# ma921/SOBER

Measured on AMD Instinct MI355X. Metric: recombination-step candidates/sec (N_rec=100000, N_nys=500, d=10, batch=100), higher is better.
Workload: dtype f64

## Files before the change

### include/sober_hip.h

```cpp
#ifndef SOBER_HIP_H
#define SOBER_HIP_H

#include <stdint.h>

#ifdef __cplusplus
extern "C" {
#endif

#define SOBER_ABI_VERSION 7

#define SOBER_KIND_RBF       0
#define SOBER_KIND_MATERN52  1
#define SOBER_KIND_TANIMOTO  2

#define SOBER_E_ARG      -1
#define SOBER_E_DIM      -2
#define SOBER_E_WS       -3
#define SOBER_E_EXCHANGE -5

int sober_abi_version(void);
int sober_diag_build(void);
int sober_reload_switches(void);
int sober_level_job_size(void);
int sober_nystrom_job_size(void);

int sober_padded_dim(int d);
int sober_bit_words(int d);

int sober_mt19937_uniform53(uint8_t* state, int64_t state_bytes, int64_t numel, double* out);
int sober_box_muller(const double* u, int64_t numel, double* out, void* stream);

int sober_scale_points(const double* X, int64_t n, int d, int64_t ldx,
                       const double* lengthscale, int ls_len,
                       double* out, int dt, void* stream);

int sober_scale_points_idx(const double* X, const int32_t* idx, int64_t n, int d, int64_t ldx, const double* lengthscale,
                           int ls_len, double* out, int dt, const double* gather_src, double* gather_out, void* stream);
int sober_pack_bits(const double* X, int64_t n, int d, int64_t ldx,
                    uint64_t* words, int nwords, double* norms, int32_t* bad_flag, void* stream);

int sober_pairwise(int kind, const void* a, const double* a_norm, int64_t m,
                   const void* b, const double* b_norm, const int32_t* idx, int64_t n,
                   int dt, double outputscale, double* out, int64_t ldo, void* stream);

int sober_kernel_matvec(int kind, const void* a, const double* a_norm, const double* v, int64_t m,
                        const void* b, const double* b_norm, int64_t n,
                        int dt, double outputscale, double c0, double* out, void* stream);

int sober_level_reduce(int kind, const void* rows, const double* rows_norm, int n_rows,
                       const void* cand, const double* cand_norm, int dt,
                       const int32_t* idx, int64_t pos0, int64_t count, int S,
                       const double* mu, const double* wmul, double outputscale,
                       int n_chunks, double* partG, int ldg, int col0,
                       double* partTot, int64_t tot_limit, void* stream);
int sober_aug_dim(int d);
int sober_augment_plan(const double* X_nys, int64_t M, int64_t ld_nys, const double* X_obs, int64_t n_obs, int64_t ld_obs,
                       const double* X_cand, int64_t N, int64_t ld_cand, int d, const double* lengthscale, int ls_len,
                       double* center, double* rows_aug, double* cand_aug, int da, void* stream);
int sober_augment_points(const double* X, int64_t n, int d, int64_t ldx, const double* lengthscale,
                         int ls_len, const double* center, int side, double* out, int da, void* stream);
int sober_level_reduce_mfma(int kind, const double* rows, int n_rows, const double* cand, int da,
                            const int32_t* idx, int64_t pos0, int64_t count, int S,
                            const double* mu, const double* wmul, double outputscale,
                            int n_chunks, double* partG, int ldg, int col0,
                            double* partTot, int64_t tot_limit, void* stream);

int64_t sober_nonzero_ws_bytes(int64_t N);
int sober_nonzero_i32(const double* mu, int64_t N, int32_t* idx_out, int64_t* count_out, void* ws, int64_t ws_bytes,
                      void* stream);

int sober_level_chunks(int n_rows, int64_t pos0, int64_t count, int S);
int sober_level_parts_mfma(int n_rows, int64_t pos0, int64_t count, int S);
int sober_level_parts_mfma_cap(int n_rows, int64_t e_total_ub, int S);

int sober_sum_partials(const double* partG, const double* partTot, int n_chunks, int n_rows,
                       int ldg, int S, const double* extraG, const double* extraTot,
                       int n_xchunks, int n_xcols, double* G, int ldo, double* tot, void* stream);

int sober_dgemm(int transa, int transb, int m, int n, int k, double alpha,
                const double* A, int lda, const double* B, int ldb,
                double beta, double* C, int ldc, void* stream);

int sober_barycentres(const double* Xtr, int ldx, int n, int S, const double* tot,
                      double* X_tmp, void* stream);
int sober_dgemm_coldiv_t(int m, int n, int k, const double* A, int lda, const double* B, int ldb, const double* coldiv,
                         double* Ct, int ldct, void* stream);

int sober_level_update(const int32_t* idx_cur, int64_t pos0, int64_t count, int S, int64_t E,
                       const int32_t* keep_rank, const double* w_star, const double* tot,
                       int n_keep, double* mu, int32_t* idx_new, int64_t new_pos0, void* stream);

int sober_scatter_weights(const int32_t* idx_cur, const int32_t* sel, const double* w, int n_sel,
                          double* mu, int64_t* out_idx, void* stream);

int sober_gather_f64(const double* src, const int32_t* idx, int64_t n, double* out, void* stream);
int sober_final_scatter(const int32_t* idx, int n, const int32_t* keep_rank, const double* w_star,
                        int64_t row_offset, double* mu, int64_t* out_idx, double* out_w, void* stream);
int sober_final_commit(const int32_t* idx, int n, const int32_t* keep_rank, const double* w_star, const int32_t* n_keep,
                       int64_t row_offset, double* mu, int64_t N, int64_t* out_idx, double* out_w, void* stream);

int sober_i64_to_i32(const int64_t* in, int64_t n, int32_t* out, void* stream);

int sober_car_pivot_host(double* h_Phi, int N, int m, double* h_mu);
int sober_car_pivot_host_fast(double* h_Phi, int N, int m, double* h_mu);

int sober_car_supported(int N, int m);
int64_t sober_car_ws_bytes(int N, int m);
int sober_car_device(const double* X, int ldx, int N, int m, const double* mu_in,
                     int32_t* keep_rank, double* w_star, int32_t* n_keep, double* mu_out,
                     double* phi_out, void* ws, int64_t ws_bytes, void* stream);
int sober_probe_rcp(const double* x, double* out, int64_t n, void* stream);

#define SOBER_CAR_DEFAULT 0
#define SOBER_CAR_SAFE 1
int sober_car_safe_supported(int N, int m);
int sober_car_giveup_forced(void);
int sober_car_device_ex(const double* X, int ldx, int N, int m, const double* mu_in,
                        int32_t* keep_rank, double* w_star, int32_t* n_keep, double* mu_out,
                        double* phi_out, void* ws, int64_t ws_bytes, int mode, void* stream);
int sober_obj_set_sums(const double* obj, const double* mu, const int32_t* idx, int64_t pos0, int64_t count, int S, int64_t E,
                       double* out, void* stream);
int sober_second_elimination(const double* phi, const double* objp, const double* w1, const int32_t* rank1, int n1,
                             int Nsets, int32_t* keep_rank, double* w_star, int32_t* n_keep, void* stream);
int sober_null_vector_supported(int nfun);
int sober_null_vector(const double* X, int ldx, int Nsets, int nfun, const int32_t* rank1, const int32_t* n_keep1, int n1,
                      double* null_row, int32_t* status, void* stream);
int sober_second_elimination_rows(const double* null_row, const double* obj_row, const double* w1, const int32_t* rank1,
                                  const int32_t* n_keep1, const int32_t* status, int n1, int Nsets, int32_t* keep_rank,
                                  double* w_star, int32_t* n_keep, void* stream);
int sober_obj_set_sums_queued(const double* obj, const double* mu, const int32_t* idx, int S, const int64_t* dR, int64_t R_known,
                              const double* tot, double* xcol, int ldx, double* ocol, void* stream);

int sober_car_mc_supported(int N, int m);
int64_t sober_car_mc_ws_bytes(int N, int m);
int sober_car_mc_device(const double* X, int ldx, int N, int m, const double* mu_in,
                        int32_t* keep_rank, double* w_star, int32_t* n_keep, double* mu_out,
                        double* phi_out, void* ws, int64_t ws_bytes, void* stream);
int sober_car_big_supported(int N, int m);
int64_t sober_car_big_ws_bytes(int N, int m);
int sober_car_big_device(const double* X, int ldx, int N, int m, const double* mu_in,
                         int32_t* keep_rank, double* w_star, int32_t* n_keep, double* mu_out,
                         double* phi_out, void* ws, int64_t ws_bytes, void* stream);
int sober_mc_selftest(const double* in, double* out, void* stream);

int sober_chol_max_n(void);
int sober_nystrom_max_n(void);
int sober_cholesky_probe_batched(const double* src, int n, int ld_src, const double* shifts, int n_shifts,
                                 double* work, int32_t* info, double* min_pivot, void* xinv_ws, int64_t ws_bytes,
                                 void* stream);
int sober_cholesky(double* A, int n, int ld, double shift, int32_t* info, double* min_pivot, void* stream);
int sober_cholesky_inv(double* A, int n, int ld, double shift, int32_t* info, double* min_pivot, double* xinv,
                       void* stream);
int sober_cholesky_inv_ratio(double* A, int n, int ld, double shift, int32_t* info, double* min_pivot, double* xinv,
                             double* ratio_out, void* stream);
int sober_trsm_blocks(const double* Y, int64_t m, int q, int ldy, const double* L, int ldl, const double* Xinv,
                      double* Q, int ldq, void* stream);
int sober_cholesky_probe(const double* src, int n, int ld_src, const double* shifts, int n_shifts,
                         double* work, int32_t* info, void* stream);
int sober_cholesky_probe_piv(const double* src, int n, int ld_src, const double* shifts, int n_shifts,
                             double* work, int32_t* info, double* min_pivot, void* stream);

int64_t sober_cholesky_probe_mc_ws_bytes(int n, int n_shifts);
int sober_cholesky_probe_mc(const double* src, int n, int ld_src, const double* shifts, int n_shifts,
                            double* work, int32_t* info, double* min_pivot, void* ws, int64_t ws_bytes,
                            void* stream);
int sober_abs_sym(const double* C, int n, int ld, double* out, int ldo, int32_t* flag, void* stream);
int sober_abs_sym_dmax(const double* C, int n, int ld, double* out, int ldo, int32_t* flag, double* dmax,
                       void* stream);

int sober_jitter_ladder(double* A, int n, int ld, int k, void* stream);
int sober_jitter_ladder_auto(double* A, int n, int ld, const int32_t* info, int n_rungs, int32_t* k_out,
                             void* stream);

int sober_level_reduce_tani_supported(int dt);
int sober_level_reduce_tani(const void* rows, const double* rows_norm, int n_rows, const void* cand,
                            const double* cand_norm, int dt, const int32_t* idx, int64_t pos0, int64_t count, int S,
                            const double* mu, const double* wmul, double outputscale, int n_chunks, double* partG,
                            int ldg, int col0, double* partTot, int64_t tot_limit, void* stream);

int sober_rank_scatter(const double* X, int ldx, int N, int n, const double* ocol, const int32_t* rank, int n1,
                       double* Xp, double* objp, void* stream);
int sober_set_i64(int64_t* dst, int64_t v, void* stream);

int sober_level_reduce_mfma_queued(int kind, const double* rows, int n_rows, const double* cand, int da,
                                   const int32_t* idx, int64_t count_ub, int S, int S_main, int leftover,
                                   const double* mu, const double* wmul, double outputscale, int n_chunks_ub,
                                   double* partG, int ldg, double* partTot, const int64_t* dR, void* stream);
int sober_level_reduce_mfma_queued_pair(int kind, const double* rows, int n_rows, const double* cand, int da,
                                        const int32_t* idx, int64_t count_ub, int S, int n_xcols, const double* mu,
                                        const double* wmul, double outputscale, int n_chunks_ub, double* partG,
                                        int ldg, double* partTot, int n_xchunks_ub, double* extraG, double* extraTot,
                                        const int64_t* dR, void* stream);
int sober_sum_partials_queued(const double* partG, const double* partTot, int n_rows, int ldg, int S,
                              const double* extraG, const double* extraTot, int n_xcols, double* G, int ldo,
                              double* tot, const int64_t* dR, int chunked, void* stream);
int sober_level_reduce_tani_queued(const void* rows, const double* rows_norm, int n_rows, const void* cand,
                                   const double* cand_norm, int dt, const int32_t* idx, int64_t count_ub, int S,
                                   int S_main, int leftover, const double* mu, const double* wmul, double outputscale,
                                   int n_chunks_ub, double* partG, int ldg, double* partTot, const int64_t* dR,
                                   void* stream);
int sober_level_reduce_tani_queued_pair(const void* rows, const double* rows_norm, int n_rows, const void* cand,
                                        const double* cand_norm, int dt, const int32_t* idx, int64_t count_ub, int S,
                                        int n_xcols, const double* mu, const double* wmul, double outputscale,
                                        int n_chunks_ub, double* partG, int ldg, double* partTot, int n_xchunks_ub,
                                        double* extraG, double* extraTot, const int64_t* dR, void* stream);
int sober_level_chunks_cap(int n_rows, int64_t e_total_ub, int S);
int sober_level_chunks_tani(int n_rows, int64_t pos0, int64_t count, int S);
int sober_level_chunks_tani_cap(int n_rows, int64_t e_total_ub, int S);
int sober_level_update_queued(const int32_t* idx_cur, int64_t R_ub, int S, const int32_t* keep_rank,
                              const double* w_star, const double* tot, double* mu, int32_t* idx_new,
                              const int64_t* dR_cur, int64_t* dR_next, int64_t R_ub_next, void* stream);

int sober_level_class_wpt(int n_rows, int64_t e_total, int S);
int sober_level_class_slots(int wpt);
int sober_level_reduce_mfma_wpt(int kind, const double* rows, int n_rows, const double* cand, int da,
                                const int32_t* idx, int64_t count, int S, const double* mu, const double* wmul,
                                double outputscale, int wpt, int n_chunks, double* partG, int ldg, double* partTot,
                                void* stream);
int sober_class_sum(const double* partG, const double* partTot, int n_chunks, int n_rows, int S, int CL,
                    double* Gc, double* totc, double* G, double* tot, void* stream);
int sober_class_derive_queued(const double* Gc, const double* totc, int n_rows, int S, int CL, const double* scale,
                              const int32_t* sof, double* Gn, double* totn, double* G, double* tot, const int64_t* dR,
                              void* stream);
int sober_level_update_queued_ex(const int32_t* idx_cur, int64_t R_ub, int S, const int32_t* keep_rank,
                                 const double* w_star, const double* tot, double* mu, int32_t* idx_new,
                                 const int64_t* dR_cur, int64_t* dR_next, int64_t R_ub_next, int need_keep,
                                 double* cls_scale, int32_t* cls_sof, int64_t R_known, void* stream);
int sober_level_update_queued_cls(const int32_t* idx_cur, int64_t R_ub, int S, const int32_t* keep_rank,
                                  const double* w_star, const double* tot, double* mu, int32_t* idx_new,
                                  const int64_t* dR_cur, int64_t* dR_next, int64_t R_ub_next, int need_keep,
                                  double* cls_scale, int32_t* cls_sof, void* stream);
#define SOBER_CLASS_MAX_DEPTH 4
int sober_level_class_depth(int variant, int n_rows, int64_t R, int S);

int64_t sober_kmeans_ws_bytes(int64_t N, int d, int K);
int64_t sober_kmeans_stat_offset(int64_t N, int d, int K);
int64_t sober_kmeans_ws_bytes_screened(int64_t N, int d, int K);
int sober_kmeans_lloyd(const double* X, int64_t N, int d, int K, int iters,
                       double* centroids, int32_t* labels, void* ws, int64_t ws_bytes, void* stream);

int sober_predict_fused_supported(int kind, int n_obs, int dt);
int sober_predict_fused(int kind, const void* obs, const double* obs_norm, int n_obs, const void* cand,
                        const double* cand_norm, int64_t N, int dt, double outputscale, const double* W, int ldw,
                        const double* alpha, double c0, double kxx_const, double noise, double* mean_out, double* var_out,
                        double eta, const double* eta_ptr, double* lfi_out, int log_flag, void* stream);
int sober_predict_fused_root(int kind, const void* obs, const double* obs_norm, int n_obs, const void* cand,
                             const double* cand_norm, int64_t N, int dt, double outputscale, const double* St, int ldst,
                             const int32_t* tri_flag, const double* alpha, double c0, double kxx_const, double noise,
                             double* mean_out, double* var_out, double eta, const double* eta_ptr, double* lfi_out, int log_flag,
                             void* stream);
int sober_predict_finish(const double* KX, const double* V, int n_obs, int64_t N, int64_t ld,
                         const double* mean, double kxx_const, const double* norms, double outputscale,
                         double noise, double* var_out, double eta, double* lfi_out, int log_flag,
                         void* stream);

int64_t sober_reduce_ws_bytes(int64_t n);
int sober_cleansing_weights(double* w, int64_t n, double eps, void* ws, int64_t ws_bytes, void* stream);

int sober_wkde_draw(const double* eps, int64_t n, int d, const int32_t* comp, const double* Xobs, int ldx,
                    const double* L, const double* lo, const double* hi, double* x, int32_t* inside,
                    void* stream);

int sober_level_gather(const double* Kmat, int n_rows, int64_t ldk, const int32_t* idx, int64_t pos0,
                       int64_t count, int S, const double* mu, const double* wmul, int n_chunks,
                       double* partG, int ldg, int col0, double* partTot, int64_t tot_limit, void* stream);

int sober_gspace_finish(double* K, const double* corr, int64_t n, int m, int64_t ldk, int64_t ldc,
                        const double* mug_cand, const double* mug_rows, void* stream);

#define SOBER_LEVEL_VALU        0
#define SOBER_LEVEL_MFMA        1
#define SOBER_LEVEL_GATHER      2
#define SOBER_LEVEL_TANI        3
#define SOBER_LEVEL_MAX_CHUNKS  64
#define SOBER_LEVEL_XS          16
typedef struct sober_level_job {
    int32_t variant, kind;
    const void* rows;   const double* rows_norm;
    const void* cand;   const double* cand_norm;
    int32_t n_rows, dim;
    int64_t kmat_ld;
    const double* wmul; double outputscale;
    int32_t S, n;
    const double* P;
    double *partG, *partTot, *extraG, *extraTot;
    double *G, *Xtr, *tot;
    double *X_tmp;
    int32_t* keep_rank;
    double *w_star, *mu_out;
    void* car_ws; int64_t car_ws_bytes;
    int32_t* h_flags;
    void* ev[4];
    const int32_t* idx; int64_t pos0, count, E;
    double* mu;
    int32_t phase;
    int64_t* dR; int64_t* h_dR;
    int32_t car_mode;
    uint64_t ev_used[2];
    int32_t class_depth;
    double* Gc[2]; double* totc[2];
    double* cls_scale; int32_t* cls_sof;
} sober_level_job;
#define SOBER_LEVEL_QUEUE 24
int sober_level_moments(const sober_level_job* job, void* stream);
int sober_level_car(const sober_level_job* job, void* stream);
int sober_level_car_retry(sober_level_job* job, void* stream);
#define SOBER_E_NOPROGRESS -4
int sober_level_loop(sober_level_job* job, int64_t R, int32_t* idx_a, int32_t* idx_b, int first_sums_ready,
                     void** events, int max_levels, int64_t* level_R, int32_t* n_levels, int64_t* R_final,
                     int32_t* in_b, void* stream);
typedef struct sober_obj_job {
    const double* obj;
    double* X_tmp;
    double* ocol;
    int32_t* kr1; double* w1; int32_t* nk1;
    double* null_row;
    int32_t* status;
} sober_obj_job;
int sober_obj_job_size(void);
int sober_level_loop_obj(sober_level_job* job, const sober_obj_job* obj_job, int64_t R, int32_t* idx_a, int32_t* idx_b,
                         int first_sums_ready, int max_levels, int64_t* level_R, int32_t* n_levels, int64_t* R_final,
                         int32_t* in_b, void* stream);
typedef int (*sober_allreduce_fn)(void* comm, double* buf, int64_t n, void* stream);
int sober_level_loop_sharded(sober_level_job* job, int rank, int world, int64_t* bounds, int32_t* idx_a,
                             int32_t* idx_b, int first_sums_ready, sober_allreduce_fn allreduce, void* comm,
                             int64_t R_stop, int max_levels, int64_t* level_R, int32_t* n_levels, int32_t* in_b,
                             void* stream);
int sober_rccl_load(const char* path);
int sober_rccl_unique_id(char* out128);
int sober_rccl_comm_init(const char* id128, int rank, int world, void** comm);
int sober_rccl_comm_destroy(void* comm);
int sober_rccl_allreduce_f64(void* comm, double* buf, int64_t n, void* stream);
int64_t sober_rccl_allreduce_ptr(void);

int64_t sober_peer_region_bytes(int64_t n_max);
int sober_peer_create(int rank, int world, int64_t n_max, void** comm, char* handle64);
int sober_peer_connect(void* comm, const char* handles);
int sober_peer_connect_ptrs(void* comm, void* const* regions);
int64_t sober_peer_region(void* comm);
int sober_peer_set_spin_limit(void* comm, unsigned spin_limit);
int sober_peer_allreduce_f64(void* comm, double* buf, int64_t n, void* stream);
int64_t sober_peer_allreduce_ptr(void);
int sober_peer_status(void* comm, double* restore, int64_t n, void* stream);
int sober_peer_destroy(void* comm);

int sober_level_final(const sober_level_job* job, const void* rows_sc, const double* rows_norm, const void* cand_sc,
                      const double* cand_norm, int dt, const int32_t* idx, int R, int64_t N, int64_t row_offset,
                      double* K, double* mu_live, int64_t* out_idx, double* out_w, void* stream);
int sober_plan_rows(int kind, const double* X_nys, int M, int64_t ld_nys, const double* X_obs, int n_obs,
                    int64_t ld_obs, int d, const double* lengthscale, int ls_len, double outputscale,
                    const double* S_cache, int ld_s, double* rows, int dt, double* Kall, double* W, double* T,
                    double* G, void* stream);

typedef struct sober_final_job {
    const void* rows_sc; const double* rows_norm;
    const void* cand_sc; const double* cand_norm;
    int32_t dt, done;
    int64_t N, row_offset;
    double *K, *mu_live;
    int64_t* out_idx; double* out_w;
    const double* cand_raw; int64_t ld_raw; int32_t d_raw, ls_len; const double* ls; double* sc_buf;
} sober_final_job;
int sober_level_final_job(const sober_level_job* job, const sober_final_job* final, const int32_t* idx, int R, void* stream);
int sober_final_job_size(void);
int sober_level_loop_final(sober_level_job* job, sober_final_job* final, int64_t R, int32_t* idx_a, int32_t* idx_b,
                           int first_sums_ready, void** events, int max_levels, int64_t* level_R, int32_t* n_levels,
                           int64_t* R_final, int32_t* in_b, void* stream);
int sober_projection(const double* Ut, int s, int M, const double* mean, const double* T, int n_obs, double* P,
                     void* stream);

typedef struct sober_nystrom_job {
    int32_t M, s, n_rungs, niter, probe_mc;
    int32_t reserved0;
    const double* G;
    const double* shifts;
    const double* R;
    double* C;
    double* chol_work;
    void* probe_ws; int64_t probe_ws_bytes;
    double* Y[2];
    double* Gm;
    double* xinv;
    void* flags_block; int64_t flags_bytes;
    void* h_flags_block;
    double* Ut;
    const double* T; int32_t n_obs;
    const double* mean_nys; double* P;
} sober_nystrom_job;
int64_t sober_nystrom_flags_bytes(int n_rungs, int niter);
int sober_nystrom_basis(const sober_nystrom_job* job, int phase, void* stream);

int sober_set_launch_events(void* start, void* stop);
int sober_record_event_pair(void* ev0, void* ev1, void* stream);

#ifdef __cplusplus
}
#endif
#endif
```

### sober_amd/_engine.py

```python
from __future__ import annotations

import os
import time
import warnings
from typing import Optional

import numpy as np
import torch

from . import _native as nat
from ._utils import SafeTensorOperator


class SoloComm:
    rank, world = 0, 1

    def allreduce_sum(self, *tensors):
        return

    def allgather_counts(self, n: int):
        return [n]

    def allgather_rows(self, t: torch.Tensor, counts):
        return t
# ... 152 lines not shown
    lm = len(w_star)
    plis = w_null > 0
    alpha = torch.zeros(lm, dtype=dt)
    alpha[plis] = w_star[plis] / w_null[plis]
    idx_sp = torch.arange(lm)[plis]
    idx_sp = idx_sp[torch.argmin(alpha[plis])]
    w_star = w_star - alpha[idx_sp] * w_null
    w_star[idx_sp] = 0.0
    keep = w_star > 0
    return w_star[keep], idx_star[keep]


def survivors_before(p: int, S: int, E: int, kept_prefix, n_keep: int, last_kept: bool) -> int:
    ES = E * S
    if p <= ES:
        return (p // S) * n_keep + kept_prefix[p % S]
    return E * n_keep + ((p - ES) if last_kept else 0)


class RecombinationEngine:
    def __init__(self, ops, comm=None, row_offset: int = 0):
        self.ops = ops
        self.comm = comm or SoloComm()
        self.row_offset = int(row_offset)
        self.tm = SafeTensorOperator()
        self.trace = None
        self.timers = {}
        self.force_host_car = False
        self.force_host_nystrom = False
        self.basis_override = None
        self.cutover_R = int(os.environ.get("SOBER_CUTOVER_R", "32768"))
        self.force_sharded = bool(os.environ.get("SOBER_FORCE_SHARDED"))

    def _tick(self, name, t0):
        t1 = time.perf_counter()
        self.timers[name] = self.timers.get(name, 0.0) + (t1 - t0)
        return t1

    def nystrom_basis(self, plan, s: int, overlap=None, literal=False, early=None):
        if self.basis_override is not None:
            return self.basis_override
        t0 = time.perf_counter()
        dev_route = getattr(self.ops, "nystrom_basis_device", None)
        if dev_route is not None and not self.force_host_nystrom and not literal:
            res = dev_route(plan, s, self.tm.max_iter, overlap, early) if (overlap is not None or early is not None) \
                else dev_route(plan, s, self.tm.max_iter)
            if res is not None:
                U, gram = res
                self._tick("nystrom_device", t0)
                if self.trace is not None:
                    (gram_h, U_h) = self.ops.to_host(gram, U)
                    self.trace.update(gram=gram_h, U=U_h)
                return U
        gram = self.ops.gram(plan)
        (gram_h,) = self.ops.to_host(gram)
        t0 = self._tick("gram_device", t0)
        _, U = ker_svd_sparsify_host(gram_h, s, self.tm)
        self._tick("nystrom_host", t0)
        if self.trace is not None:
            self.trace.update(gram=gram_h.clone(), U=U.clone())
        return U

    def run(self, plan, mu: torch.Tensor, num_pts: int, obj: Optional[torch.Tensor] = None, live=None):
        ops, comm = self.ops, self.comm
        self.obj = obj
        self.obj_head = None
        if obj is not None:
            head = obj[:2 * num_pts].clone()
            if comm.world > 1:
                cnt = comm.allgather_counts(int(head.numel()))
                head = comm.allgather_rows(head, cnt)[:2 * num_pts]
            self.obj_head = head
        n = num_pts - 1
        S = 2 * (n + 1)
        state = {}
        can_start = getattr(ops, "nonzero_start", None) is not None and live is None
        pend = {}

        def start_list():
            if can_start and "p" not in pend:
                pend["p"] = ops.nonzero_start(mu)
        sharded = comm.world > 1 or (self.force_sharded and getattr(comm, "native_allreduce", None) is not None)

        def first_sums():
            if live is not None:
                idx_cur, count = live, int(live.numel())
            else:
                start_list()
                idx_cur, count = ops.nonzero_finish(pend["p"]) if "p" in pend else ops.nonzero_i32(mu)
            counts = comm.allgather_counts(count)
            bounds = [0]
            for c in counts:
                bounds.append(bounds[-1] + c)
            state.update(idx_cur=idx_cur, count=count, pos0=bounds[comm.rank], R=bounds[-1], bounds=bounds)
            cut = sharded and obj is None and self.cutover_R > 0 and state["R"] <= self.cutover_R
            if state["R"] > S and getattr(ops, "level_car", None) is not None and count > 0 and not cut:
                ops.level_moments(plan, idx_cur, state["pos0"], count, S, state["R"] // S, mu, phase=1, n=n)
                state["sums_ready"] = True

        def head_once():
            if not state:
                first_sums()

        n_fun = n + 1 + (1 if obj is not None else 0)
        car_on_host = self.force_host_car or getattr(ops, "car_supported", None) is None \
            or not ops.car_supported(S, n_fun) or (obj is not None and getattr(ops, "car_obj_device", None) is None)
        if car_on_host and not self.force_host_car and getattr(ops, "size_cliff", None) is not None \
                and getattr(ops, "car_supported", None) is not None and not ops.car_supported(S, n_fun):
            ops.size_cliff("car", f"batch = {n + 1}: a Caratheodory step on 2 x batch = {S} points with {n_fun} test functions is beyond "
                                  "the device kernels (registers of one compute unit: batch <= 100, of nine: batch <= 224, memory-resident: "
                                  "2 x batch <= 2048); every level's step runs on host LAPACK + the C++ pivots instead -- seconds per level")
        if comm.world > 1:
            start_list()
        U = self.nystrom_basis(plan, n, overlap=head_once if comm.world == 1 else None, literal=car_on_host,
                               early=start_list if comm.world == 1 else None)
        if comm.world > 1:
            U = comm.broadcast0(ops.from_host(U.contiguous()) if U.device != ops.device else U.contiguous())
            if hasattr(plan, "_proj_src"):
                plan._proj_src = None
        ops.set_projection(plan, U)
        head_once()
        idx_cur, count, pos0, R = state["idx_cur"], state["count"], state["pos0"], state["R"]
        bounds = state["bounds"]
        sums_ready = state.get("sums_ready", False)
        idx_new = ops.empty_i32(count)
        levels = [] if self.trace is not None else None

        if self.trace is not None:
            self.trace["levels"] = levels
        if not sharded and obj is None and levels is None and not self.force_host_car and R > S \
                and getattr(ops, "level_loop", None) is not None and ops.car_supported(S, n + 1):
            t0 = time.perf_counter()
            idx_cur, idx_new, R = ops.level_loop(plan, idx_cur, idx_new, R, S, mu, sums_ready, self.row_offset)
            pos0, count, bounds, sums_ready = 0, R, [0, R], False
            self._tick("levels_device", t0)
        elif not sharded and obj is not None and levels is None and not self.force_host_car and R > S \
                and getattr(ops, "level_loop_obj", None) is not None:
            t0 = time.perf_counter()
            res = ops.level_loop_obj(plan, idx_cur, idx_new, R, S, mu, obj, sums_ready)
            if res is not None and res[3] > 0:
                idx_cur, idx_new, R = res[:3]
                pos0, count, bounds, sums_ready = 0, R, [0, R], False
            self._tick("levels_device", t0)
        elif sharded and obj is None and levels is None and not self.force_host_car and R > S \
                and getattr(ops, "level_loop_sharded", None) is not None and ops.car_supported(S, n + 1) \
                and getattr(comm, "native_allreduce", None) is not None:
            t0 = time.perf_counter()
            idx_cur, idx_new, bounds = ops.level_loop_sharded(plan, idx_cur, idx_new, bounds, S, mu, sums_ready, comm,
                                                              self.cutover_R)
            R, pos0, count, sums_ready = bounds[-1], bounds[comm.rank], bounds[comm.rank + 1] - bounds[comm.rank], False
            self._tick("levels_device", t0)
            if R > S:
                return self._finish_replicated(plan, idx_cur, bounds, mu, num_pts, U)
        while True:
            if R <= n + 1:
                return self._finish_small(mu)
            if R <= S:
                return self._finish_direct(plan, idx_cur, bounds, R, mu, levels)

            E = R // S
            r = R - E * S
            t0 = time.perf_counter()
            if sums_ready:
                Xtr, tot = ops.level_moments(plan, idx_cur, pos0, count, S, E, mu, phase=2)
                sums_ready = False
            else:
                Xtr, tot = ops.level_moments(plan, idx_cur, pos0, count, S, E, mu)
            if obj is None:
                flat = getattr(ops, "level_flat", None)
                if flat is not None:
                    comm.allreduce_sum(flat(plan))
                else:
                    comm.allreduce_sum(Xtr, tot)
            else:
                orow = self._obj_set_sums(obj, mu, idx_cur, pos0, count, S, E)
                comm.allreduce_sum(Xtr, tot, orow)
                Xtr = torch.cat([Xtr, orow.unsqueeze(0)], 0)
            if obj is None and not self.force_host_car and getattr(ops, "level_car", None) is not None \
                    and ops.car_supported(S, n + 1):
                res = ops.level_car(plan, S)
                if res is None:
                    X_tmp, tot = ops.level_barycentres(plan)
                    keep_rank_d, w_star_d, keep_rank, n_keep = self._car(X_tmp, tot, R, E, r, levels, t0)
                    keep_np = keep_rank.numpy()
                else:
                    keep_rank_d, w_star_d, keep_np, n_keep = res
                    self._tick("levels_device", t0)
                    if levels is not None:
                        X_h, mu_h, w_h = ops.level_trace(plan)
                        levels.append(dict(kind="level", R=R, E=E, r=r, X_tmp=X_h, tot_weights=mu_h,
                                           idx_star=torch.from_numpy(np.flatnonzero(keep_np >= 0)),
                                           w_star=w_h[:n_keep].clone()))
            else:
                X_tmp = ops.barycentres(Xtr, tot)
                keep_rank_d, w_star_d, keep_rank, n_keep = self._car(X_tmp, tot, R, E, r, levels, t0)
                keep_np = keep_rank.numpy()
            kept = keep_np >= 0
            last_kept = bool(kept[S - 1])
            kept_prefix = [0] + np.cumsum(kept).tolist()
            R_new = E * n_keep + (r if last_kept else 0)
            if R_new >= R:
                raise RuntimeError(
                    "recombination made no progress (the Caratheodory step cancelled nothing, "
                    "SOBER/_rchq.py:241-242); the reference would loop forever here")
            bounds = [survivors_before(b_, S, E, kept_prefix, n_keep, last_kept) for b_ in bounds]
            new_pos0, new_end = bounds[comm.rank], bounds[comm.rank + 1]
            if count > 0:
                ops.level_update(idx_cur, pos0, count, S, E, keep_rank_d, w_star_d, tot, n_keep, mu,
                                 idx_new, new_pos0)
            idx_cur, idx_new = idx_new, idx_cur
            pos0, count, R = new_pos0, new_end - new_pos0, R_new

    def _obj_set_sums(self, obj, mu, idx_cur, pos0, count, S, E):
        dev = mu.device
        if count == 0:
            return torch.zeros(S, dtype=torch.float64, device=dev)
        native = getattr(self.ops, "obj_set_sums", None)
        if native is not None and obj.dtype == torch.float64 and obj.is_contiguous():
            return native(obj, mu, idx_cur, pos0, count, S, E)
        c = idx_cur[:count].long()
        v = obj[c] * mu[c]
        e_first = pos0 // S
        e_total = (pos0 + count + S - 1) // S - e_first
        dense = torch.zeros(e_total * S, dtype=torch.float64, device=dev)
        off = pos0 - e_first * S
        dense[off:off + count] = v
        out = dense.view(e_total, S).sum(0)
        n_left = pos0 + count - max(pos0, E * S)
        if n_left > 0:
            out[S - 1] += v[count - n_left:].sum()
        return out

    def _finish_replicated(self, plan, idx_cur, bounds, mu, num_pts, U):
        ops, comm = self.ops, self.comm
        counts = [bounds[r + 1] - bounds[r] for r in range(comm.world)]
        loc = idx_cur[:counts[comm.rank]].long()
        X_all = comm.allgather_rows(plan.X_cand_raw[loc].to(torch.float64).contiguous(), counts)
        w_all = comm.allgather_rows(mu[loc].contiguous(), counts)
        gid = comm.allgather_rows((loc + self.row_offset).contiguous(), counts)
        plan2 = ops.build_plan(plan.spec, plan.mode, plan.X_nys_raw, X_all)
        sub = RecombinationEngine(ops, SoloComm(), row_offset=0)
        sub.basis_override = U
        sub.force_host_nystrom, sub.force_host_car = self.force_host_nystrom, self.force_host_car
        mu2 = w_all.clone().contiguous()
        live2 = torch.arange(mu2.numel(), dtype=torch.int32, device=mu2.device)
        idx2, w2 = sub.run(plan2, mu2, num_pts, live=live2)
        for k, v in sub.timers.items():
            self.timers[k] = self.timers.get(k, 0.0) + v
        idx_glob = gid[idx2]
        mu[loc] = 0.0
        mine = (idx_glob >= self.row_offset) & (idx_glob < self.row_offset + mu.numel())
        mu[idx_glob[mine] - self.row_offset] = w2[mine]
        return idx_glob, w2

    def _car(self, X_dev, mu_dev, R, E, r, levels, t0, kind="level"):
        ops = self.ops
        Np, n1 = X_dev.shape[0], X_dev.shape[1] + 1
        use_obj = getattr(self, "obj", None) is not None
        on_device = getattr(ops, "car_supported", None) is not None and ops.car_supported(Np, n1) \
            and not self.force_host_car
        if on_device and use_obj and getattr(ops, "car_obj_device", None) is not None:
            res = ops.car_obj_device(X_dev, mu_dev, None if kind == "level" else self.obj_head)
            if res is not None:
                keep_rank_d, w_star_d, keep_rank, n_keep, (kr1_h, w1_d, n1k) = res
                self._tick("levels_device", t0)
                if levels is not None:
                    X_h, mu_h, w1_h = ops.to_host(X_dev, mu_dev, w1_d)
                    levels.append(dict(kind=kind, R=R, E=E, r=r, X_tmp=X_h, tot_weights=mu_h,
                                       idx_star=torch.nonzero(kr1_h >= 0).flatten(), w_star=w1_h[:n1k].clone()))
                return keep_rank_d, w_star_d, keep_rank, n_keep
            on_device = False
        elif use_obj:
            on_device = False
        if on_device:
            res = ops.car_device_checked(X_dev, mu_dev, also=(X_dev, mu_dev) if levels is not None else ())
            if res is not None:
                keep_rank_d, w_star_d, keep_rank, n_keep, extra = res
                self._tick("levels_device", t0)
                if levels is not None:
                    (w_h,) = ops.to_host(w_star_d)
                    levels.append(dict(kind=kind, R=R, E=E, r=r, X_tmp=extra[0], tot_weights=extra[1],
                                       idx_star=torch.nonzero(keep_rank >= 0).flatten(), w_star=w_h[:n_keep].clone()))
                return keep_rank_d, w_star_d, keep_rank, n_keep
        X_h, mu_h = ops.to_host(X_dev, mu_dev)
        t0 = self._tick("levels_device", t0)
        w_star, idx_star = car_host(X_h, mu_h.clone())
        if levels is not None:
            levels.append(dict(kind=kind, R=R, E=E, r=r, X_tmp=X_h.clone(), tot_weights=mu_h.clone(),
                               idx_star=idx_star.clone(), w_star=w_star.clone()))
        if use_obj:
            nfun = X_h.shape[1] - 1
            obj_p = X_h[idx_star, nfun] if kind == "level" else self.obj_head.cpu()[idx_star]
            w_star, idx_star = second_elimination_host(X_h[idx_star, :nfun].T.contiguous(), obj_p, w_star, idx_star)
        self._tick("car_host", t0)
        n_keep = int(idx_star.numel())
        keep_rank = torch.full((Np,), -1, dtype=torch.int32)
        keep_rank[idx_star] = torch.arange(n_keep, dtype=torch.int32)
        return ops.from_host(keep_rank), ops.from_host(w_star), keep_rank, n_keep

    def _gather_result(self, idx_local, w_local, counts=None):
        comm = self.comm
        idx_glob = idx_local.to(torch.int64) + self.row_offset
        if comm.world == 1:
            return idx_glob, w_local
        if counts is None:
            counts = comm.allgather_counts(int(idx_glob.numel()))
        return comm.allgather_rows(idx_glob, counts), comm.allgather_rows(w_local, counts)

    def _finish_small(self, mu):
        idx_star = torch.nonzero(mu > 0).flatten()
        return self._gather_result(idx_star, mu[idx_star])

    def _finish_direct(self, plan, idx_cur, bounds, R, mu, levels):
        ops, comm = self.ops, self.comm
        n = plan.n
        counts = [bounds[r + 1] - bounds[r] for r in range(comm.world)]
# ... 33 lines not shown
```

### sober_amd/_native.py

```python
from __future__ import annotations

import ctypes as C
import os
from typing import Optional

import torch

_HERE = os.path.dirname(os.path.abspath(__file__))
LIB_PATH = os.environ.get("SOBER_HIP_LIB") or os.path.join(_HERE, "libsober_hip.so")
ABI_VERSION = 7

KIND_RBF, KIND_MATERN52, KIND_TANIMOTO = 0, 1, 2
KIND_BY_NAME = {"rbf": KIND_RBF, "matern52": KIND_MATERN52, "tanimoto": KIND_TANIMOTO}

_vp, _i32, _i64, _f64 = C.c_void_p, C.c_int, C.c_int64, C.c_double

SIGNATURES = {
    "sober_abi_version": (_i32, []),
    "sober_diag_build": (_i32, []),
    "sober_reload_switches": (_i32, []),
    "sober_level_job_size": (_i32, []),
    "sober_nystrom_job_size": (_i32, []),
    "sober_final_job_size": (_i32, []),
    "sober_set_i64": (_i32, [_vp, _i64, _vp]),
    "sober_rank_scatter": (_i32, [_vp, _i32, _i32, _i32, _vp, _vp, _i32, _vp, _vp, _vp]),
    "sober_plan_rows": (_i32, [_i32, _vp, _i32, _i64, _vp, _i32, _i64, _i32, _vp, _i32, _f64, _vp, _i32, _vp, _i32, _vp,
                               _vp, _vp, _vp, _vp]),
    "sober_level_loop_final": (_i32, [_vp, _vp, _i64, _vp, _vp, _i32, _vp, _i32, _vp, _vp, _vp, _vp, _vp]),
    "sober_padded_dim": (_i32, [_i32]),
    "sober_bit_words": (_i32, [_i32]),
    "sober_scale_points": (_i32, [_vp, _i64, _i32, _i64, _vp, _i32, _vp, _i32, _vp]),
    "sober_augment_plan": (_i32, [_vp, _i64, _i64, _vp, _i64, _i64, _vp, _i64, _i64, _i32, _vp, _i32, _vp, _vp, _vp, _i32, _vp]),
    "sober_scale_points_idx": (_i32, [_vp, _vp, _i64, _i32, _i64, _vp, _i32, _vp, _i32, _vp, _vp, _vp]),
    "sober_pack_bits": (_i32, [_vp, _i64, _i32, _i64, _vp, _i32, _vp, _vp, _vp]),
    "sober_mt19937_uniform53": (_i32, [_vp, _i64, _i64, _vp]),
    "sober_box_muller": (_i32, [_vp, _i64, _vp, _vp]),
    "sober_pairwise": (_i32, [_i32, _vp, _vp, _i64, _vp, _vp, _vp, _i64, _i32, _f64, _vp, _i64, _vp]),
    "sober_kernel_matvec": (_i32, [_i32, _vp, _vp, _vp, _i64, _vp, _vp, _i64, _i32, _f64, _f64, _vp, _vp]),
    "sober_level_reduce": (_i32, [_i32, _vp, _vp, _i32, _vp, _vp, _i32, _vp, _i64, _i64, _i32, _vp, _vp,
                                  _f64, _i32, _vp, _i32, _i32, _vp, _i64, _vp]),
    "sober_nonzero_ws_bytes": (_i64, [_i64]),
    "sober_nonzero_i32": (_i32, [_vp, _i64, _vp, _vp, _vp, _i64, _vp]),
    "sober_dgemm_coldiv_t": (_i32, [_i32, _i32, _i32, _vp, _i32, _vp, _i32, _vp, _vp, _i32, _vp]),
    "sober_level_chunks": (_i32, [_i32, _i64, _i64, _i32]),
    "sober_level_parts_mfma": (_i32, [_i32, _i64, _i64, _i32]),
    "sober_level_parts_mfma_cap": (_i32, [_i32, _i64, _i32]),
    "sober_aug_dim": (_i32, [_i32]),
    "sober_augment_points": (_i32, [_vp, _i64, _i32, _i64, _vp, _i32, _vp, _i32, _vp, _i32, _vp]),
    "sober_level_reduce_mfma": (_i32, [_i32, _vp, _i32, _vp, _i32, _vp, _i64, _i64, _i32, _vp, _vp, _f64, _i32,
                                       _vp, _i32, _i32, _vp, _i64, _vp]),
    "sober_sum_partials": (_i32, [_vp, _vp, _i32, _i32, _i32, _i32, _vp, _vp, _i32, _i32, _vp, _i32, _vp, _vp]),
    "sober_dgemm": (_i32, [_i32, _i32, _i32, _i32, _i32, _f64, _vp, _i32, _vp, _i32, _f64, _vp, _i32, _vp]),
    "sober_barycentres": (_i32, [_vp, _i32, _i32, _i32, _vp, _vp, _vp]),
    "sober_level_update": (_i32, [_vp, _i64, _i64, _i32, _i64, _vp, _vp, _vp, _i32, _vp, _vp, _i64, _vp]),
    "sober_scatter_weights": (_i32, [_vp, _vp, _vp, _i32, _vp, _vp, _vp]),
    "sober_i64_to_i32": (_i32, [_vp, _i64, _vp, _vp]),
    "sober_car_pivot_host": (_i32, [_vp, _i32, _i32, _vp]),
    "sober_car_pivot_host_fast": (_i32, [_vp, _i32, _i32, _vp]),
    "sober_car_supported": (_i32, [_i32, _i32]),
    "sober_car_ws_bytes": (_i64, [_i32, _i32]),
    "sober_car_device": (_i32, [_vp, _i32, _i32, _i32, _vp, _vp, _vp, _vp, _vp, _vp, _vp, _i64, _vp]),
    "sober_probe_rcp": (_i32, [_vp, _vp, _i64, _vp]),
    "sober_second_elimination": (_i32, [_vp, _vp, _vp, _vp, _i32, _i32, _vp, _vp, _vp, _vp]),
    "sober_car_mc_supported": (_i32, [_i32, _i32]),
    "sober_car_mc_ws_bytes": (_i64, [_i32, _i32]),
    "sober_car_mc_device": (_i32, [_vp, _i32, _i32, _i32, _vp, _vp, _vp, _vp, _vp, _vp, _vp, _i64, _vp]),
    "sober_car_big_supported": (_i32, [_i32, _i32]),
    "sober_car_big_ws_bytes": (_i64, [_i32, _i32]),
    "sober_car_big_device": (_i32, [_vp, _i32, _i32, _i32, _vp, _vp, _vp, _vp, _vp, _vp, _vp, _i64, _vp]),
    "sober_car_device_ex": (_i32, [_vp, _i32, _i32, _i32, _vp, _vp, _vp, _vp, _vp, _vp, _vp, _i64, _i32, _vp]),
    "sober_obj_set_sums": (_i32, [_vp, _vp, _vp, _i64, _i64, _i32, _i64, _vp, _vp]),
    "sober_null_vector_supported": (_i32, [_i32]),
    "sober_null_vector": (_i32, [_vp, _i32, _i32, _i32, _vp, _vp, _i32, _vp, _vp, _vp]),
    "sober_second_elimination_rows": (_i32, [_vp, _vp, _vp, _vp, _vp, _vp, _i32, _i32, _vp, _vp, _vp, _vp]),
    "sober_obj_set_sums_queued": (_i32, [_vp, _vp, _vp, _i32, _vp, _i64, _vp, _vp, _i32, _vp, _vp]),
    "sober_obj_job_size": (_i32, []),
    "sober_level_loop_obj": (_i32, [_vp, _vp, _i64, _vp, _vp, _i32, _i32, _vp, _vp, _vp, _vp, _vp]),
    "sober_car_safe_supported": (_i32, [_i32, _i32]),
    "sober_car_giveup_forced": (_i32, []),
    "sober_final_commit": (_i32, [_vp, _i32, _vp, _vp, _vp, _i64, _vp, _i64, _vp, _vp, _vp]),
    "sober_level_car_retry": (_i32, [_vp, _vp]),
    "sober_mc_selftest": (_i32, [_vp, _vp, _vp]),
    "sober_chol_max_n": (_i32, []),
    "sober_nystrom_max_n": (_i32, []),
    "sober_cholesky_probe_batched": (_i32, [_vp, _i32, _i32, _vp, _i32, _vp, _vp, _vp, _vp, _i64, _vp]),
    "sober_cholesky": (_i32, [_vp, _i32, _i32, _f64, _vp, _vp, _vp]),
    "sober_cholesky_inv": (_i32, [_vp, _i32, _i32, _f64, _vp, _vp, _vp, _vp]),
    "sober_cholesky_inv_ratio": (_i32, [_vp, _i32, _i32, _f64, _vp, _vp, _vp, _vp, _vp]),
    "sober_trsm_blocks": (_i32, [_vp, _i64, _i32, _i32, _vp, _i32, _vp, _vp, _i32, _vp]),
    "sober_cholesky_probe": (_i32, [_vp, _i32, _i32, _vp, _i32, _vp, _vp, _vp]),
    "sober_cholesky_probe_piv": (_i32, [_vp, _i32, _i32, _vp, _i32, _vp, _vp, _vp, _vp]),
    "sober_cholesky_probe_mc_ws_bytes": (_i64, [_i32, _i32]),
    "sober_cholesky_probe_mc": (_i32, [_vp, _i32, _i32, _vp, _i32, _vp, _vp, _vp, _vp, _i64, _vp]),
    "sober_abs_sym": (_i32, [_vp, _i32, _i32, _vp, _i32, _vp, _vp]),
    "sober_abs_sym_dmax": (_i32, [_vp, _i32, _i32, _vp, _i32, _vp, _vp, _vp]),
    "sober_jitter_ladder": (_i32, [_vp, _i32, _i32, _i32, _vp]),
    "sober_jitter_ladder_auto": (_i32, [_vp, _i32, _i32, _vp, _i32, _vp, _vp]),
    "sober_kmeans_ws_bytes": (_i64, [_i64, _i32, _i32]),
    "sober_kmeans_stat_offset": (_i64, [_i64, _i32, _i32]),
    "sober_kmeans_ws_bytes_screened": (_i64, [_i64, _i32, _i32]),
    "sober_kmeans_lloyd": (_i32, [_vp, _i64, _i32, _i32, _i32, _vp, _vp, _vp, _i64, _vp]),
    "sober_predict_fused_supported": (_i32, [_i32, _i32, _i32]),
    "sober_predict_fused": (_i32, [_i32, _vp, _vp, _i32, _vp, _vp, _i64, _i32, _f64, _vp, _i32, _vp, _f64, _f64, _f64, _vp, _vp,
                                   _f64, _vp, _vp, _i32, _vp]),
    "sober_predict_fused_root": (_i32, [_i32, _vp, _vp, _i32, _vp, _vp, _i64, _i32, _f64, _vp, _i32, _vp, _vp, _f64, _f64, _f64, _vp,
                                        _vp, _f64, _vp, _vp, _i32, _vp]),
    "sober_predict_finish": (_i32, [_vp, _vp, _i32, _i64, _i64, _vp, _f64, _vp, _f64, _f64, _vp, _f64, _vp, _i32, _vp]),
    "sober_reduce_ws_bytes": (_i64, [_i64]),
    "sober_cleansing_weights": (_i32, [_vp, _i64, _f64, _vp, _i64, _vp]),
    "sober_level_gather": (_i32, [_vp, _i32, _i64, _vp, _i64, _i64, _i32, _vp, _vp, _i32, _vp, _i32, _i32, _vp, _i64,
                                  _vp]),
    "sober_gspace_finish": (_i32, [_vp, _vp, _i64, _i32, _i64, _i64, _vp, _vp, _vp]),
    "sober_wkde_draw": (_i32, [_vp, _i64, _i32, _vp, _vp, _i32, _vp, _vp, _vp, _vp, _vp, _vp]),
    "sober_level_moments": (_i32, [_vp, _vp]),
    "sober_level_car": (_i32, [_vp, _vp]),
    "sober_level_reduce_tani_supported": (_i32, [_i32]),
    "sober_level_reduce_tani": (_i32, [_vp, _vp, _i32, _vp, _vp, _i32, _vp, _i64, _i64, _i32, _vp, _vp, _f64, _i32, _vp,
                                       _i32, _i32, _vp, _i64, _vp]),
    "sober_level_loop_sharded": (_i32, [_vp, _i32, _i32, _vp, _vp, _vp, _i32, _vp, _vp, _i64, _i32, _vp, _vp, _vp, _vp]),
    "sober_rccl_load": (_i32, [C.c_char_p]),
    "sober_rccl_unique_id": (_i32, [_vp]),
    "sober_rccl_comm_init": (_i32, [_vp, _i32, _i32, _vp]),
    "sober_rccl_comm_destroy": (_i32, [_vp]),
    "sober_rccl_allreduce_f64": (_i32, [_vp, _vp, _i64, _vp]),
    "sober_rccl_allreduce_ptr": (_i64, []),
    "sober_peer_region_bytes": (_i64, [_i64]),
    "sober_peer_create": (_i32, [_i32, _i32, _i64, _vp, _vp]),
    "sober_peer_connect": (_i32, [_vp, C.c_char_p]),
    "sober_peer_connect_ptrs": (_i32, [_vp, _vp]),
    "sober_peer_region": (_i64, [_vp]),
    "sober_peer_set_spin_limit": (_i32, [_vp, C.c_uint]),
    "sober_peer_allreduce_f64": (_i32, [_vp, _vp, _i64, _vp]),
    "sober_peer_allreduce_ptr": (_i64, []),
    "sober_peer_status": (_i32, [_vp, _vp, _i64, _vp]),
    "sober_peer_destroy": (_i32, [_vp]),
    "sober_level_reduce_mfma_queued": (_i32, [_i32, _vp, _i32, _vp, _i32, _vp, _i64, _i32, _i32, _i32, _vp, _vp, _f64,
                                              _i32, _vp, _i32, _vp, _vp, _vp]),
    "sober_level_reduce_mfma_queued_pair": (_i32, [_i32, _vp, _i32, _vp, _i32, _vp, _i64, _i32, _i32, _vp, _vp, _f64, _i32,
                                                   _vp, _i32, _vp, _i32, _vp, _vp, _vp, _vp]),
    "sober_sum_partials_queued": (_i32, [_vp, _vp, _i32, _i32, _i32, _vp, _vp, _i32, _vp, _i32, _vp, _vp, _i32, _vp]),
    "sober_level_reduce_tani_queued": (_i32, [_vp, _vp, _i32, _vp, _vp, _i32, _vp, _i64, _i32, _i32, _i32, _vp, _vp, _f64,
                                              _i32, _vp, _i32, _vp, _vp, _vp]),
    "sober_level_reduce_tani_queued_pair": (_i32, [_vp, _vp, _i32, _vp, _vp, _i32, _vp, _i64, _i32, _i32, _vp, _vp, _f64, _i32,
                                                   _vp, _i32, _vp, _i32, _vp, _vp, _vp, _vp]),
    "sober_level_chunks_cap": (_i32, [_i32, _i64, _i32]),
    "sober_level_chunks_tani": (_i32, [_i32, _i64, _i64, _i32]),
    "sober_level_chunks_tani_cap": (_i32, [_i32, _i64, _i32]),
    "sober_level_update_queued": (_i32, [_vp, _i64, _i32, _vp, _vp, _vp, _vp, _vp, _vp, _vp, _i64, _vp]),
    "sober_level_update_queued_ex": (_i32, [_vp, _i64, _i32, _vp, _vp, _vp, _vp, _vp, _vp, _vp, _i64, _i32, _vp, _vp, _i64, _vp]),
    "sober_level_update_queued_cls": (_i32, [_vp, _i64, _i32, _vp, _vp, _vp, _vp, _vp, _vp, _vp, _i64, _i32, _vp, _vp, _vp]),
    "sober_level_class_wpt": (_i32, [_i32, _i64, _i32]),
    "sober_level_class_slots": (_i32, [_i32]),
    "sober_level_class_depth": (_i32, [_i32, _i32, _i64, _i32]),
    "sober_level_reduce_mfma_wpt": (_i32, [_i32, _vp, _i32, _vp, _i32, _vp, _i64, _i32, _vp, _vp, _f64, _i32, _i32, _vp, _i32,
                                           _vp, _vp]),
    "sober_class_sum": (_i32, [_vp, _vp, _i32, _i32, _i32, _i32, _vp, _vp, _vp, _vp, _vp]),
    "sober_class_derive_queued": (_i32, [_vp, _vp, _i32, _i32, _i32, _vp, _vp, _vp, _vp, _vp, _vp, _vp, _vp]),
    "sober_record_event_pair": (_i32, [_vp, _vp, _vp]),
    "sober_set_launch_events": (_i32, [_vp, _vp]),
    "sober_projection": (_i32, [_vp, _i32, _i32, _vp, _vp, _i32, _vp, _vp]),
    "sober_nystrom_flags_bytes": (_i64, [_i32, _i32]),
    "sober_nystrom_basis": (_i32, [_vp, _i32, _vp]),
    "sober_gather_f64": (_i32, [_vp, _vp, _i64, _vp, _vp]),
    "sober_final_scatter": (_i32, [_vp, _i32, _vp, _vp, _i64, _vp, _vp, _vp, _vp]),
    "sober_level_final": (_i32, [_vp, _vp, _vp, _vp, _vp, _i32, _vp, _i32, _i64, _i64, _vp, _vp, _vp, _vp, _vp]),
    "sober_level_final_job": (_i32, [_vp, _vp, _vp, _i32, _vp]),
    "sober_level_loop": (_i32, [_vp, _i64, _vp, _vp, _i32, _vp, _i32, _vp, _vp, _vp, _vp, _vp]),
}

LEVEL_VALU, LEVEL_MFMA, LEVEL_GATHER, LEVEL_TANI = 0, 1, 2, 3
LEVEL_MAX_CHUNKS, LEVEL_XS, LEVEL_QUEUE = 64, 16, 24


class FinalJob(C.Structure):
    _fields_ = [
        ("rows_sc", _vp), ("rows_norm", _vp), ("cand_sc", _vp), ("cand_norm", _vp),
        ("dt", _i32), ("done", _i32), ("N", _i64), ("row_offset", _i64),
        ("K", _vp), ("mu_live", _vp), ("out_idx", _vp), ("out_w", _vp),
        ("cand_raw", _vp), ("ld_raw", _i64), ("d_raw", _i32), ("ls_len", _i32), ("ls", _vp), ("sc_buf", _vp),
    ]


class ObjJob(C.Structure):
    _fields_ = [("obj", _vp), ("X_tmp", _vp), ("ocol", _vp), ("kr1", _vp), ("w1", _vp), ("nk1", _vp), ("null_row", _vp),
                ("status", _vp)]


class NystromJob(C.Structure):
    _fields_ = [
        ("M", _i32), ("s", _i32), ("n_rungs", _i32), ("niter", _i32), ("probe_mc", _i32), ("_pad0", _i32),
        ("G", _vp), ("shifts", _vp), ("R", _vp), ("C", _vp), ("chol_work", _vp),
        ("probe_ws", _vp), ("probe_ws_bytes", _i64),
        ("Y", _vp * 2), ("Gm", _vp), ("xinv", _vp),
        ("flags_block", _vp), ("flags_bytes", _i64), ("h_flags_block", _vp),
        ("Ut", _vp),
        ("T", _vp), ("n_obs", _i32), ("mean_nys", _vp), ("P", _vp),
    ]


class LevelJob(C.Structure):
    _fields_ = [
        ("variant", _i32), ("kind", _i32),
        ("rows", _vp), ("rows_norm", _vp), ("cand", _vp), ("cand_norm", _vp),
        ("n_rows", _i32), ("dim", _i32), ("kmat_ld", _i64),
        ("wmul", _vp), ("outputscale", _f64),
        ("S", _i32), ("n", _i32), ("P", _vp),
        ("partG", _vp), ("partTot", _vp), ("extraG", _vp), ("extraTot", _vp),
        ("G", _vp), ("Xtr", _vp), ("tot", _vp), ("X_tmp", _vp),
        ("keep_rank", _vp), ("w_star", _vp), ("mu_out", _vp),
        ("car_ws", _vp), ("car_ws_bytes", _i64), ("h_flags", _vp),
        ("ev", _vp * 4),
        ("idx", _vp), ("pos0", _i64), ("count", _i64), ("E", _i64), ("mu", _vp),
        ("phase", _i32),
        ("dR", _vp), ("h_dR", _vp),
        ("car_mode", _i32),
        ("ev_used", C.c_uint64 * 2),
        ("class_depth", _i32), ("Gc", _vp * 2), ("totc", _vp * 2), ("cls_scale", _vp), ("cls_sof", _vp),
    ]

E_DIM = -2
E_EXCHANGE = -5
CLASS_MAX_DEPTH = 4
CAR_DEFAULT, CAR_SAFE, CAR_HOST = 0, 1, 2

_lib: Optional[C.CDLL] = None


class SoberHipError(RuntimeError):
    pass


def load() -> C.CDLL:
    global _lib
    if _lib is not None:
        return _lib
    if not os.path.exists(LIB_PATH):
        raise SoberHipError(
            f"{LIB_PATH} not found: build it with `make -C sober_amd/csrc` "
            "(python -c 'import __graft_entry__ as g; g.build()').  sober_amd has no CPU fallback.")
    lib = C.CDLL(LIB_PATH)
    lib.sober_abi_version.restype = _i32
    got = lib.sober_abi_version()
    if got != ABI_VERSION:
        raise SoberHipError(f"libsober_hip ABI {got} != expected {ABI_VERSION}; rebuild (make -C sober_amd/csrc)")
    for name, (res, args) in SIGNATURES.items():
        fn = getattr(lib, name)
        fn.restype, fn.argtypes = res, args
    if lib.sober_diag_build() and os.environ.get("SOBER_ALLOW_DIAG_LIB") != "1":
        raise SoberHipError(f"{LIB_PATH} is a diagnostic build (in-kernel time stamps): not a library to compute with; "
                            "`make -C sober_amd/csrc` builds the product (SOBER_ALLOW_DIAG_LIB=1: the stamp scripts)")
    for name, cls in (("sober_level_job_size", LevelJob), ("sober_nystrom_job_size", NystromJob),
                      ("sober_final_job_size", FinalJob), ("sober_obj_job_size", ObjJob)):
        if getattr(lib, name)() != C.sizeof(cls):
            raise SoberHipError(f"{cls.__name__}: {C.sizeof(cls)} bytes here, {getattr(lib, name)()} in libsober_hip; "
                                "include/sober_hip.h and sober_amd/_native.py disagree")
    _lib = lib
    return lib


def reload_switches():
    load().sober_reload_switches()


def _check(rc: int, what: str):
    if rc == 0:
        return
    if rc < 0:
        msg = {-1: "bad argument", -2: "dimension not supported by the compiled tile set",
               -3: "workspace too small",
               -5: "a multi-workgroup Caratheodory kernel gave up waiting for a partner workgroup (no result)"}.get(rc, "error")
        raise SoberHipError(f"{what}: {msg} (code {rc})")
    raise SoberHipError(f"{what}: hipError_t {rc}")


def _ptr(t: Optional[torch.Tensor]) -> Optional[int]:
    return None if t is None else t.data_ptr()


_raw_stream = getattr(torch._C, "_cuda_getCurrentRawStream", None)


def _stream(t: torch.Tensor) -> Optional[int]:
    if not t.is_cuda:
        raise SoberHipError("sober_amd runs on the MI355X only: tensor is not on a HIP device")
    if _raw_stream is not None:
        return _raw_stream(t.device.index)
    return torch.cuda.current_stream(t.device).cuda_stream


def _req(t: torch.Tensor, dtype, name: str):
    if t.dtype != dtype or not t.is_contiguous():
        raise SoberHipError(f"{name}: need contiguous {dtype}, got {t.dtype} contiguous={t.is_contiguous()}")
    return t


def padded_dim(d: int, generic: bool = False) -> int:
    r = load().sober_padded_dim(d)
    if r == E_DIM and generic and d > 0:
        return (d + 3) // 4 * 4
    _check(min(r, 0), f"padded_dim({d})")
    return r


def bit_words(d: int, generic: bool = False) -> int:
    r = load().sober_bit_words(d)
    if r == E_DIM and generic and d > 0:
        return (d + 63) // 64
    _check(min(r, 0), f"bit_words({d})")
    return r


def fused_dim_supported(kind: int, d: int) -> bool:
    r = load().sober_bit_words(d) if kind == KIND_TANIMOTO else load().sober_padded_dim(d)
    return r > 0


def scale_points_idx(X, idx, n, lengthscale, out):
    _req(lengthscale, torch.float64, "lengthscale"); _req(out, torch.float64, "out"); _req(idx, torch.int32, "idx")
    if X.dtype != torch.float64 or X.stride(-1) != 1:
        raise SoberHipError("scale_points_idx: X must be float64 with unit inner stride")
    _check(load().sober_scale_points_idx(X.data_ptr(), idx.data_ptr(), int(n), X.shape[1], X.stride(0), lengthscale.data_ptr(),
                                         lengthscale.numel(), out.data_ptr(), out.shape[1], None, None, _stream(X)),
           "sober_scale_points_idx")


def scale_points(X, lengthscale, out):
    n, d = X.shape
    _req(X, torch.float64, "X"); _req(lengthscale, torch.float64, "lengthscale"); _req(out, torch.float64, "out")
    _check(load().sober_scale_points(X.data_ptr(), n, d, X.stride(0), lengthscale.data_ptr(),
                                     lengthscale.numel(), out.data_ptr(), out.shape[1], _stream(X)),
           "sober_scale_points")


def mt19937_uniform53(state, numel, out):
    _req(state, torch.uint8, "state"); _req(out, torch.float64, "out")
    if state.is_cuda or out.is_cuda or out.numel() < numel + 16:
        raise ValueError("mt19937_uniform53 takes host tensors, out of numel + 16 doubles")
    _check(load().sober_mt19937_uniform53(state.data_ptr(), state.numel(), numel, out.data_ptr()),
           "sober_mt19937_uniform53")


def box_muller(u, numel, out):
    _req(u, torch.float64, "u"); _req(out, torch.float64, "out")
    if u.numel() < numel + 16 or out.numel() < numel:
        raise ValueError("box_muller: u holds numel + 16 uniforms, out numel normals")
    _check(load().sober_box_muller(u.data_ptr(), numel, out.data_ptr(), _stream(out)), "sober_box_muller")


def pack_bits(X, words, norms, bad_flag):
    n, d = X.shape
    _req(X, torch.float64, "X"); _req(words, torch.int64, "words"); _req(norms, torch.float64, "norms")
    _req(bad_flag, torch.int32, "bad_flag")
    _check(load().sober_pack_bits(X.data_ptr(), n, d, X.stride(0), words.data_ptr(), words.shape[1],
                                  norms.data_ptr(), bad_flag.data_ptr(), _stream(X)), "sober_pack_bits")


def rank_scatter(X, n, ocol, rank, n1, Xp, objp):
    _req(X, torch.float64, "X"); _req(ocol, torch.float64, "ocol"); _req(rank, torch.int32, "rank")
    _check(load().sober_rank_scatter(X.data_ptr(), X.stride(0), X.shape[0], n, ocol.data_ptr(), rank.data_ptr(), n1,
                                     Xp.data_ptr(), objp.data_ptr(), _stream(X)), "sober_rank_scatter")


def plan_rows(kind, X_nys, X_obs, lengthscale, outputscale, S_cache, rows, Kall, W, T, G):
    M, d = X_nys.shape
    n_obs = 0 if X_obs is None else X_obs.shape[0]
    for t in (X_nys, X_obs, S_cache, rows, Kall, W, T, G):
        if t is not None and (t.dtype != torch.float64 or t.stride(-1) != 1):
            raise SoberHipError("plan_rows: float64 tensors with unit inner stride")
    _check(load().sober_plan_rows(kind, X_nys.data_ptr(), M, X_nys.stride(0), _ptr(X_obs), n_obs,
                                  X_obs.stride(0) if X_obs is not None else 0, d, lengthscale.data_ptr(),
# ... 383 lines not shown
MAX_LEVELS = 64


def level_loop(job: LevelJob, R: int, idx_a, idx_b, first_sums_ready: bool, events, stream: int, final: "FinalJob" = None):
    level_R = (_i64 * MAX_LEVELS)()
    n_levels, in_b, R_final = _i32(0), _i32(0), _i64(0)
    ev = None
    if events is not None:
        ev = (_vp * (4 * MAX_LEVELS))(*events)
    if final is not None:
        rc = load().sober_level_loop_final(C.addressof(job), C.addressof(final), R, idx_a.data_ptr(), idx_b.data_ptr(),
                                           int(bool(first_sums_ready)), ev, MAX_LEVELS, level_R, C.byref(n_levels),
                                           C.byref(R_final), C.byref(in_b), stream)
    else:
        rc = load().sober_level_loop(C.addressof(job), R, idx_a.data_ptr(), idx_b.data_ptr(), int(bool(first_sums_ready)),
                                     ev, MAX_LEVELS, level_R, C.byref(n_levels), C.byref(R_final), C.byref(in_b), stream)
    if rc == E_NOPROGRESS:
        raise RuntimeError("recombination made no progress (the Caratheodory step cancelled nothing, "
                           "SOBER/_rchq.py:241-242); the reference would loop forever here")
    if rc != E_EXCHANGE:
        _check(rc, "sober_level_loop")
    return list(level_R[:n_levels.value]), int(R_final.value), bool(in_b.value), rc == E_EXCHANGE


ALLREDUCE_FN = C.CFUNCTYPE(_i32, _vp, _vp, _i64, _vp)


def level_loop_sharded(job: LevelJob, rank: int, world: int, bounds, idx_a, idx_b, first_sums_ready: bool,
                       allreduce_ptr, comm_ptr, R_stop: int, stream: int):
    level_R = (_i64 * MAX_LEVELS)()
    n_levels, in_b = _i32(0), _i32(0)
    b = (_i64 * (world + 1))(*bounds)
    rc = load().sober_level_loop_sharded(C.addressof(job), rank, world, b, idx_a.data_ptr(), idx_b.data_ptr(),
                                         int(bool(first_sums_ready)), allreduce_ptr, comm_ptr, int(R_stop), MAX_LEVELS,
                                         level_R, C.byref(n_levels), C.byref(in_b), stream)
    if rc == E_NOPROGRESS:
        raise RuntimeError("recombination made no progress (the Caratheodory step cancelled nothing, "
                           "SOBER/_rchq.py:241-242); the reference would loop forever here")
    _check(rc, "sober_level_loop_sharded")
    return list(level_R[:n_levels.value]), list(b), bool(in_b.value)


class RcclComm:

    def __init__(self, dist, group, device):
        import torch as _t
        lib = load()
        path = os.path.join(os.path.dirname(_t.__file__), "lib", "librccl.so")
        _check(lib.sober_rccl_load(path.encode() if os.path.exists(path) else b""), "sober_rccl_load")
        rank, world = dist.get_rank(group), dist.get_world_size(group)
        buf = (C.c_char * 128)()
        if rank == 0:
            _check(lib.sober_rccl_unique_id(C.addressof(buf)), "sober_rccl_unique_id")
        on_dev = dist.get_backend(group) == "nccl"
        t = _t.frombuffer(bytearray(buf.raw), dtype=_t.uint8).clone()
        t = t.to(device) if on_dev else t
        dist.broadcast(t, src=dist.get_global_rank(group, 0) if group is not None else 0, group=group)
        ident = bytes(t.cpu().numpy().tobytes())
        self.handle = _vp()
        with _t.cuda.device(device):
            _check(lib.sober_rccl_comm_init(ident, rank, world, C.byref(self.handle)), "sober_rccl_comm_init")
        self.fn_ptr = lib.sober_rccl_allreduce_ptr()

    def close(self):
        if self.handle:
            load().sober_rccl_comm_destroy(self.handle)
            self.handle = _vp()


class PeerComm:

    def __init__(self, dist, group, device, n_max: int):
        import torch as _t
        lib = load()
        self.rank, self.world = dist.get_rank(group), dist.get_world_size(group)
        self.n_max, self.device, self.handle = int(n_max), device, _vp()
        self.fn_ptr = lib.sober_peer_allreduce_ptr()
        on_dev = dist.get_backend(group) == "nccl"
        hbuf = (C.c_char * 64)()
        with _t.cuda.device(device):
            rc = lib.sober_peer_create(self.rank, self.world, self.n_max, C.byref(self.handle), C.addressof(hbuf))
        mine = _t.frombuffer(bytearray(hbuf.raw), dtype=_t.uint8).clone()
        mine = _t.cat([mine, _t.tensor([0 if rc == 0 else 1], dtype=_t.uint8)])
        mine = mine.to(device) if on_dev else mine
        outs = [_t.empty_like(mine) for _ in range(self.world)]
        dist.all_gather(outs, mine, group=group)
        outs = [o.cpu() for o in outs]
        ok = rc == 0 and all(int(o[64]) == 0 for o in outs)
        if ok:
            allh = b"".join(bytes(o[:64].numpy().tobytes()) for o in outs)
            with _t.cuda.device(device):
                ok = lib.sober_peer_connect(self.handle, allh) == 0
        self.ok = self._agree(dist, group, on_dev, ok)
        if not self.ok:
            self.close()

    def _agree(self, dist, group, on_dev, ok: bool) -> bool:
        import torch as _t
        t = _t.tensor([1 if ok else 0], dtype=_t.int32)
        t = t.to(self.device) if on_dev else t
        dist.all_reduce(t, op=dist.ReduceOp.MIN, group=group)
        return bool(int(t.item()) == 1)

    def allreduce(self, buf, stream: int):
        _check(load().sober_peer_allreduce_f64(self.handle, buf.data_ptr(), buf.numel(), stream), "sober_peer_allreduce_f64")

    def status(self, stream: int = None) -> int:
        if stream is None:
            import torch as _t
            stream = _t.cuda.current_stream(self.device).cuda_stream
        return int(load().sober_peer_status(self.handle, None, 0, stream))

    def self_check(self, dist, group) -> bool:
        import torch as _t
        lib = load()
        on_dev = dist.get_backend(group) == "nccl"
        ok = True
        try:
            lib.sober_peer_set_spin_limit(self.handle, 1 << 21)
            dist.barrier(group=group)
            with _t.cuda.device(self.device):
                n = min(self.n_max, 4096)
                base = _t.arange(n, dtype=_t.float64, device=self.device)
                st = _t.cuda.current_stream(self.device)
                for rnd in range(4):
                    x = (base + rnd) * float(self.rank + 1)
                    self.allreduce(x, st.cuda_stream)
                    st.synchronize()
                    want = (base + rnd) * float(self.world * (self.world + 1) // 2)
                    ok = ok and self.status() == 0 and bool(_t.equal(x, want))
        except Exception:
            ok = False
        if self.handle:
            lib.sober_peer_set_spin_limit(self.handle, 1 << 27)
        self.ok = self._agree(dist, group, on_dev, ok)
        if not self.ok:
            self.close()
        return self.ok

    def close(self):
        if self.handle:
            load().sober_peer_destroy(self.handle)
            self.handle = _vp()


def level_final(job: LevelJob, rows, rows_norm, cand, cand_norm, dt, idx, R, N, row_offset, K, mu_live, out_idx,
                out_w, stream: int):
    _check(load().sober_level_final(C.addressof(job), rows.data_ptr(), _ptr(rows_norm), cand.data_ptr(),
                                    _ptr(cand_norm), dt, idx.data_ptr(), int(R), int(N), int(row_offset),
                                    K.data_ptr(), mu_live.data_ptr(), out_idx.data_ptr(), out_w.data_ptr(), stream),
           "sober_level_final")


def level_final_job(job: LevelJob, fin: "FinalJob", idx, R: int, stream: int):
    _check(load().sober_level_final_job(C.addressof(job), C.addressof(fin), idx.data_ptr(), int(R), stream), "sober_level_final_job")


def nystrom_flags_bytes(n_rungs: int, niter: int) -> int:
    return int(load().sober_nystrom_flags_bytes(n_rungs, niter))


def nystrom_basis(job: NystromJob, phase: int, stream: int):
    _check(load().sober_nystrom_basis(C.addressof(job), int(phase), stream), "sober_nystrom_basis")


def projection(Ut, mean, T, P):
    s_, M = Ut.shape
    _check(load().sober_projection(Ut.data_ptr(), s_, M, _ptr(mean), _ptr(T), 0 if T is None else T.shape[1], P.data_ptr(),
                                   _stream(P)), "sober_projection")


def record_event_pair(ev0, ev1, stream: int):
    _check(load().sober_record_event_pair(ev0.cuda_event, ev1.cuda_event, stream), "sober_record_event_pair")


def jitter_ladder_auto(A, info, k_out):
    _check(load().sober_jitter_ladder_auto(A.data_ptr(), A.shape[0], A.stride(0), info.data_ptr(), info.numel(),
                                           k_out.data_ptr(), _stream(A)), "sober_jitter_ladder_auto")


def jitter_ladder(A, k):
    _check(load().sober_jitter_ladder(A.data_ptr(), A.shape[0], A.stride(0), int(k), _stream(A)), "sober_jitter_ladder")
```

### sober_amd/_ops_hip.py

```python
from __future__ import annotations

import os
import warnings

import torch

from . import _native as nat
from ._ops_levels import _LevelOps
from ._ops_nystrom import _NystromOps
from ._ops_plan import Plan, _PlanOps


class HipOps(_PlanOps, _NystromOps, _LevelOps):
    name = "hip"

    def __init__(self, device):
        self.device = torch.device(device)
        if self.device.type != "cuda":
            raise nat.SoberHipError("sober_amd needs a HIP device (torch device 'cuda'); got "
                                    f"{self.device}.  There is no CPU fallback.")
        nat.load()
        self._pin = {}
        self.prof = None
        self.use_mfma = True
        self.queue_levels = os.environ.get("SOBER_NO_QUEUE") is None
        self.level_classes = True
        self.obj_null_kernel = True
        self.queue_obj_levels = True
        self.lazy_scaled_pool = True
        self.last_levels = None
        self._probe_mc = torch.cuda.get_device_properties(self.device).multi_processor_count >= 256
        self.car_mode = nat.CAR_DEFAULT

    def size_cliff(self, which: str, message: str):
        seen = self.__dict__.setdefault("_cliffs_seen", set())
        if which not in seen:
            seen.add(which)
            import warnings
            warnings.warn("sober_amd: " + message, RuntimeWarning, stacklevel=3)

    def prof_reserve(self, n_pairs: int):
        pool = getattr(self, "_ev_pool", None)
        if pool is None:
            pool = self._ev_pool = []
        st = torch.cuda.current_stream(self.device)
        for _ in range(n_pairs):
            e0, e1 = torch.cuda.Event(enable_timing=True), torch.cuda.Event(enable_timing=True)
            e0.record(st); e1.record(st)
            pool.append((e0, e1))

    def _prof_pair(self):
        pool = getattr(self, "_ev_pool", None)
        if not pool:
            self.prof_reserve(1)
            pool = self._ev_pool
        return pool.pop()

    def _buf(self, p, name, numel):
        t = p.ws.get(name)
        if t is None or t.numel() < numel:
            t = torch.empty(numel, dtype=torch.float64, device=self.device)
            p.ws[name] = t
        return t

    def _buf_u8(self, p, name, nbytes):
        t = p.ws.get(name)
        if t is None or t.numel() < nbytes:
            t = torch.empty(max(nbytes, 8), dtype=torch.uint8, device=self.device)
            p.ws[name] = t
        return t

    def nonzero_start(self, mu):
        N = mu.numel()
        key = ("nz", N)
        bufs = self._pin.get(key)
        if bufs is None:
            ws = torch.zeros(nat.nonzero_ws_bytes(N), dtype=torch.uint8, device=self.device)
            bufs = self._pin[key] = (ws, torch.zeros(1, dtype=torch.int64, device=self.device),
                                     torch.zeros(1, dtype=torch.int64).pin_memory())
        ws, cnt, pin = bufs
        out = torch.empty(N, dtype=torch.int32, device=self.device)
        nat.nonzero_i32(mu, out, cnt, ws)
        pin.copy_(cnt, non_blocking=True)
        ev = torch.cuda.Event()
        ev.record(torch.cuda.current_stream(self.device))
        return out, pin, ev

    def nonzero_finish(self, pending):
        out, pin, ev = pending
        ev.synchronize()
        return out, int(pin[0])

    def nonzero_i32(self, mu):
        nz = torch.nonzero(mu != 0).flatten()
        out = torch.empty(max(nz.numel(), 1), dtype=torch.int32, device=self.device)
        if nz.numel():
            nat.i64_to_i32(nz, out)
        return out, int(nz.numel())

    def empty_i32(self, n):
        return torch.empty(max(n, 1), dtype=torch.int32, device=self.device)

    def to_host(self, *tensors, before_sync=None):
        outs = []
        for i, t in enumerate(tensors):
            key = (i, t.dtype, tuple(t.shape))
            buf = self._pin.get(key)
            if buf is None:
                buf = torch.empty(t.shape, dtype=t.dtype, pin_memory=True)
                self._pin[key] = buf
            buf.copy_(t, non_blocking=True)
            outs.append(buf)
        if before_sync is None:
            torch.cuda.current_stream(self.device).synchronize()
        else:
            ev = torch.cuda.Event()
            ev.record(torch.cuda.current_stream(self.device))
            before_sync()
            ev.synchronize()
        return [o.clone() for o in outs]

    def from_host(self, t, dtype=None):
        return t.to(self.device, dtype=dtype, non_blocking=False)


class MatrixKernelOps(HipOps):

    CHUNK_ROWS = 1 << 15

    def build_plan(self, kernel_fn, mode, X_nys, X_cand, pool_owner=None) -> Plan:
        p = Plan()
        p.kernel_fn, p.mode = kernel_fn, "matrix"
        p.X_nys, p.X_cand = X_nys, X_cand
        p.M = p.Mtot = X_nys.shape[0]
        p.weighted, p.T, p.P, p.wmul, p.da = False, None, None, None, -1
        p.ws = {}
        N = X_cand.shape[0]
        if hasattr(kernel_fn, "materialise"):
            p.Kmat = kernel_fn.materialise(X_cand, X_nys)
        else:
            p.Kmat = torch.empty(N, p.M, dtype=torch.float64, device=self.device)
            for lo in range(0, N, self.CHUNK_ROWS):
                hi = min(N, lo + self.CHUNK_ROWS)
                p.Kmat[lo:hi] = kernel_fn(X_nys, X_cand[lo:hi]).to(torch.float64).T
        if tuple(p.Kmat.shape) != (N, p.M) or p.Kmat.dtype != torch.float64 or p.Kmat.stride(1) != 1:
            raise nat.SoberHipError(f"kernel matrix must be ({N}, {p.M}) float64 row-major, got "
                                    f"{tuple(p.Kmat.shape)} {p.Kmat.dtype}")
        return p

    def gram(self, p):
        if hasattr(p.kernel_fn, "materialise"):
            return p.kernel_fn.materialise(p.X_nys, p.X_nys, gram=True)
        return p.kernel_fn(p.X_nys, p.X_nys).to(torch.float64).contiguous()

    def set_projection(self, p, U):
        p.P = U.to(self.device, torch.float64).contiguous()
        p.n = p.P.shape[0]

    def direct_columns(self, p, idx, count):
        Kc = p.Kmat[idx[:count].long()].contiguous()
        Xtr = torch.empty(p.n, count, dtype=torch.float64, device=self.device)
        nat.dgemm(p.P, Kc, Xtr, transb=True)
        out = torch.empty(count, p.n, dtype=torch.float64, device=self.device)
        nat.barycentres(Xtr, p.n, count, None, out)
        return out


CallableKernelOps = MatrixKernelOps
```

### sober_amd/_ops_levels.py

```python
from __future__ import annotations

import warnings

import torch

from . import _native as nat
from ._ops_plan import Plan


class _LevelOps:

    def _job(self, p: Plan, S: int, n: int = None) -> nat.LevelJob:
        n = p.n if n is None else n
        job = p.ws.get("job")
        if job is not None and job.S == S and job.n == n:
            if p.P is not None and job.P != p.P.data_ptr():
                if p.P.stride(0) != p.Mtot or p.P.stride(1) != 1:
                    p.P = p.P.contiguous()
                job.P = p.P.data_ptr()
            job.car_mode = min(self.car_mode, nat.CAR_SAFE)
            return job
        dev, f64 = self.device, torch.float64
        job = nat.LevelJob()
        Kmat = getattr(p, "Kmat", None)
        if Kmat is not None:
            job.variant, job.kind = nat.LEVEL_GATHER, 0
            job.cand, job.kmat_ld, job.n_rows = Kmat.data_ptr(), Kmat.stride(0), Kmat.shape[1]
            job.outputscale = 1.0
        elif p.da > 0:
            job.variant, job.kind = nat.LEVEL_MFMA, p.kind
            job.rows, job.cand, job.dim, job.n_rows = p.rows_aug.data_ptr(), p.cand_aug.data_ptr(), p.da, p.Mtot
            job.outputscale = float(p.spec.outputscale)
        else:
            tani = p.kind == nat.KIND_TANIMOTO and self.use_mfma and bool(nat.load().sober_level_reduce_tani_supported(p.rows.dt))
            job.variant, job.kind = (nat.LEVEL_TANI if tani else nat.LEVEL_VALU), p.kind
            job.rows, job.rows_norm = p.rows.data.data_ptr(), nat._ptr(p.rows.norm)
            job.cand, job.cand_norm = p.cand.data.data_ptr(), nat._ptr(p.cand.norm)
            job.dim, job.n_rows = p.rows.dt, p.Mtot
            job.outputscale = float(p.spec.outputscale)
        job.wmul = nat._ptr(p.wmul)
        if p.P is not None and (p.P.stride(0) != p.Mtot or p.P.stride(1) != 1):
            p.P = p.P.contiguous()
        job.S, job.n, job.P = S, n, nat._ptr(p.P)
        nr, mc, xs = job.n_rows, nat.LEVEL_MAX_CHUNKS, nat.LEVEL_XS
        w = p.ws
        w["partG"], w["partTot"] = torch.empty(mc * nr * S, dtype=f64, device=dev), torch.empty(mc * S, dtype=f64, device=dev)
        w["extraG"], w["extraTot"] = torch.empty(mc * nr * xs, dtype=f64, device=dev), torch.empty(mc * xs, dtype=f64, device=dev)
        w["G"] = torch.empty(nr, S, dtype=f64, device=dev)
        w["XT"] = torch.empty(n * S + S, dtype=f64, device=dev)
        w["Xtr"], w["tot"] = w["XT"][:n * S].view(n, S), w["XT"][n * S:]
        w["X_tmp"] = torch.empty(S, n, dtype=f64, device=dev)
        w["keep_rank"] = torch.empty(S + 1, dtype=torch.int32, device=dev)
        w["w_star"], w["mu_out"] = torch.empty(S, dtype=f64, device=dev), torch.empty(S, dtype=f64, device=dev)
        w["h_flags"] = torch.empty(S + 1, dtype=torch.int32, pin_memory=True)
        w["h_flags_np"] = w["h_flags"].numpy()
        if job.variant in (nat.LEVEL_MFMA, nat.LEVEL_TANI) and self.queue_levels:
            w["dR"] = torch.empty(nat.LEVEL_QUEUE + 1, dtype=torch.int64, device=dev)
            w["h_dR"] = torch.zeros(nat.LEVEL_QUEUE + 1, dtype=torch.int64, pin_memory=True)
            job.dR, job.h_dR = w["dR"].data_ptr(), w["h_dR"].data_ptr()
            if S % 2 == 0:
                cl = 1 << nat.CLASS_MAX_DEPTH
                w["Gc"] = [torch.empty(nr * S * (cl >> k), dtype=f64, device=dev) for k in (0, 1)]
                w["totc"] = [torch.empty(S * (cl >> k), dtype=f64, device=dev) for k in (0, 1)]
                w["cls_scale"], w["cls_sof"] = torch.empty(S, dtype=f64, device=dev), torch.empty(S, dtype=torch.int32, device=dev)
                for k in (0, 1):
                    job.Gc[k], job.totc[k] = w["Gc"][k].data_ptr(), w["totc"][k].data_ptr()
                job.cls_scale, job.cls_sof = w["cls_scale"].data_ptr(), w["cls_sof"].data_ptr()
        for k in ("partG", "partTot", "extraG", "extraTot", "G", "Xtr", "tot", "X_tmp", "keep_rank", "w_star", "mu_out",
                  "h_flags"):
            setattr(job, k, w[k].data_ptr())
        if nat.car_supported(S, n + 1):
            nbytes = nat.car_ws_bytes(S, n + 1)
            w["car_ws"] = torch.empty(max(nbytes // 8, 1), dtype=f64, device=dev)
            job.car_ws, job.car_ws_bytes = w["car_ws"].data_ptr(), nbytes
        job.car_mode = min(self.car_mode, nat.CAR_SAFE)
        w["job"] = job
        return job

    def _car_downgrade(self, mode: int, why: str):
        if mode > self.car_mode:
            self.car_mode = mode
            warnings.warn("sober_amd: a multi-workgroup Caratheodory launch gave up waiting for its partner workgroups "
                          f"({why}); this and the following steps use "
                          + ("the kernels without such waits (one workgroup, or a launch per dependency beyond batch 100)" if mode == nat.CAR_SAFE
                             else "the host LAPACK route")
                          + " for that step -- same result, slower")

    def level_moments(self, p: Plan, idx, pos0, count, S, E, mu, phase: int = 0, n: int = None):
        job = self._job(p, S, n)
        job.phase = phase
        if count <= 0 and phase != 2:
            p.ws["XT"].zero_(); p.ws["G"].zero_()
            return p.ws["Xtr"], p.ws["tot"]
        if phase == 2:
            nat.level_moments(job, nat._stream(p.ws["G"]))
            return p.ws["Xtr"], p.ws["tot"]
        nat._req(idx, torch.int32, "idx"); nat._req(mu, torch.float64, "mu")
        job.idx, job.pos0, job.count, job.E, job.mu = idx.data_ptr(), pos0, count, E, mu.data_ptr()
        job.class_depth = 0
        if phase == 1 and pos0 == 0 and count == E * S and job.Gc[0] and job.dR and self.level_classes:
            job.class_depth = int(nat.load().sober_level_class_depth(job.variant, job.n_rows, count, S))
        pair = None
        if self.prof is not None:
            n_left = max(pos0 + count - max(pos0, E * S), 0)
            pair, pair2 = self._prof_pair(), (self._prof_pair() if n_left > 0 else None)
            job.ev[0], job.ev[1] = pair[0].cuda_event, pair[1].cuda_event
            job.ev[2], job.ev[3] = (pair2[0].cuda_event, pair2[1].cuda_event) if pair2 else (None, None)
        nat.level_moments(job, nat._stream(mu))
        if pair is not None:
            self.prof.append((pair[0], pair[1], int(count * job.n_rows), 1))
            if pair2 is not None:
                self.prof.append((pair2[0], pair2[1], int(n_left * job.n_rows), 1))
            for k in range(4):
                job.ev[k] = None
        return p.ws["Xtr"], p.ws["tot"]

    def level_loop_obj(self, p: Plan, idx_cur, idx_new, R: int, S: int, mu, obj, sums_ready: bool):
        job = self._job(p, S)
        n = job.n
        if not self.queue_obj_levels or not self.queue_levels or not job.dR or job.variant not in (nat.LEVEL_MFMA, nat.LEVEL_TANI):
            return None
        if self.car_mode == nat.CAR_HOST or not self.obj_null_kernel or not self.car_supported(S, n + 2) \
                or not bool(nat.load().sober_null_vector_supported(n)):
            return None
        nat._req(mu, torch.float64, "mu"); nat._req(idx_cur, torch.int32, "idx"); nat._req(idx_new, torch.int32, "idx")
        nat._req(obj, torch.float64, "obj")
        dev, f64, w = self.device, torch.float64, p.ws
        if "obj_job" not in w:
            oj = nat.ObjJob()
            w["obj_X"] = torch.empty(S, n + 1, dtype=f64, device=dev)
            w["obj_f"] = torch.empty(3, S, dtype=f64, device=dev)
            w["obj_i"] = torch.empty(S + 2, dtype=torch.int32, device=dev)
            nbytes = nat.car_ws_bytes(S, n + 2)
            w["obj_car_ws"] = (torch.empty(max(nbytes // 8, 1), dtype=f64, device=dev), nbytes)
            oj.X_tmp, oj.ocol, oj.w1, oj.null_row = (w["obj_X"].data_ptr(), w["obj_f"][0].data_ptr(), w["obj_f"][1].data_ptr(),
                                                       w["obj_f"][2].data_ptr())
            oj.kr1, oj.nk1, oj.status = w["obj_i"].data_ptr(), w["obj_i"][S:].data_ptr(), w["obj_i"][S + 1:].data_ptr()
            w["obj_job"] = oj
        oj = w["obj_job"]
        oj.obj = obj.data_ptr()
        job.mu = mu.data_ptr()
        saved = (job.car_ws, job.car_ws_bytes, job.class_depth)
        job.car_ws, job.car_ws_bytes, job.class_depth = w["obj_car_ws"][0].data_ptr(), w["obj_car_ws"][1], 0
        try:
            level_R, R_final, in_b = nat.level_loop_obj(job, oj, R, idx_cur, idx_new, sums_ready, nat._stream(mu))
        finally:
            job.car_ws, job.car_ws_bytes, job.class_depth = saved
        if in_b:
            idx_cur, idx_new = idx_new, idx_cur
        return idx_cur, idx_new, R_final, len(level_R)

    def level_loop(self, p: Plan, idx_cur, idx_new, R: int, S: int, mu, sums_ready: bool, row_offset: int = 0):
        import math
        job = self._job(p, S)
        nat._req(mu, torch.float64, "mu"); nat._req(idx_cur, torch.int32, "idx"); nat._req(idx_new, torch.int32, "idx")
        job.mu = mu.data_ptr()
        if not sums_ready:
            job.class_depth = 0
        events = pairs = None
        if self.prof is not None:
            n_max = min(nat.MAX_LEVELS, int(math.log2(max(R / S, 1.0))) + 3)
            pairs = [(self._prof_pair(), self._prof_pair()) for _ in range(n_max)]
            events = [None] * (4 * nat.MAX_LEVELS)
            for l, (a, b) in enumerate(pairs):
                events[4 * l:4 * l + 4] = [a[0].cuda_event, a[1].cuda_event, b[0].cuda_event, b[1].cuda_event]
        fin = None
        p.ws.pop("final_done", None)
        if not p.weighted and getattr(p, "Kmat", None) is None and self.car_mode != nat.CAR_HOST and job.car_ws:
            fin = self._final_job(p, S, mu, row_offset)
        level_R, R_final, in_b, gave_up = nat.level_loop(job, R, idx_cur, idx_new, sums_ready, events, nat._stream(mu), fin)
        self.last_levels = {"R": [int(v) for v in level_R], "derived": int(job.class_depth) if sums_ready else 0}
        if fin is not None and fin.done:
            n_keep = int(p.ws["h_flags_np"][S])
            if n_keep >= 0:
                lst = idx_new if in_b else idx_cur
                p.ws["final_done"] = (lst.data_ptr(), R_final, row_offset, p._fin_out[0][:n_keep], p._fin_out[1][:n_keep])
        if job.car_mode > min(self.car_mode, nat.CAR_SAFE):
            self._car_downgrade(nat.CAR_SAFE, "level loop")
        if gave_up:
            self._car_downgrade(nat.CAR_HOST, "level loop")
        if pairs is not None:
            for l, (a, b) in enumerate(pairs):
                Rl = level_R[l] if l < len(level_R) else 0
                both = not ((job.ev_used[1] >> l) & 1)
                for which, pr, ent in ((0, a, Rl + (Rl % S if both else 0)), (1, b, Rl % S)):
                    if (job.ev_used[which] >> l) & 1 and not (l == 0 and sums_ready):
                        self.prof.append((pr[0], pr[1], int(ent * job.n_rows), 1))
                    else:
                        self._ev_pool.append(pr)
        return (idx_new, idx_cur, R_final) if in_b else (idx_cur, idx_new, R_final)

    def level_loop_sharded(self, p: Plan, idx_cur, idx_new, bounds, S: int, mu, sums_ready: bool, comm, R_stop: int):
        job = self._job(p, S)
        nat._req(mu, torch.float64, "mu"); nat._req(idx_cur, torch.int32, "idx"); nat._req(idx_new, torch.int32, "idx")
        job.mu = mu.data_ptr()
        job.class_depth = 0
        fn_ptr, comm_ptr, keep = comm.native_allreduce(p.ws["XT"], self.device)
        _, new_bounds, in_b = nat.level_loop_sharded(job, comm.rank, comm.world, bounds, idx_cur, idx_new, sums_ready,
                                                     fn_ptr, comm_ptr, R_stop, nat._stream(mu))
        del keep
        if job.car_mode > min(self.car_mode, nat.CAR_SAFE):
            self._car_downgrade(nat.CAR_SAFE, "sharded level loop")
        return (idx_new, idx_cur, new_bounds) if in_b else (idx_cur, idx_new, new_bounds)

    def _final_job(self, p: Plan, S: int, mu, row_offset: int = 0):
        dev = self.device
        f = nat.FinalJob()
        f.rows_sc, f.rows_norm = p.rows.data.data_ptr(), nat._ptr(p.rows.norm)
        if p.cand is not None:
            f.cand_sc, f.cand_norm = p.cand.data.data_ptr(), nat._ptr(p.cand.norm)
        else:
            Xr, ls = p.cand_raw, p.spec.lengthscale
            f.cand_sc, f.cand_norm = None, None
            f.cand_raw, f.ld_raw, f.d_raw = Xr.data_ptr(), Xr.stride(0), Xr.shape[1]
            f.ls, f.ls_len = ls.data_ptr(), ls.numel()
            f.sc_buf = self._buf(p, "sc_final", S * p.rows.dt).data_ptr()
        f.dt, f.done, f.N, f.row_offset = p.rows.dt, 0, mu.numel(), row_offset
        p._fin_out = (torch.empty(S, dtype=torch.int64, device=dev), torch.empty(S, dtype=torch.float64, device=dev))
        f.K, f.mu_live = self._buf(p, "K_final", p.Mtot * S).data_ptr(), self._buf(p, "mu_live", S).data_ptr()
        f.out_idx, f.out_w = p._fin_out[0].data_ptr(), p._fin_out[1].data_ptr()
        return f

    def level_final(self, p: Plan, idx_cur, R: int, S: int, mu, row_offset: int):
        if p.weighted or getattr(p, "Kmat", None) is not None or not nat.car_supported(R, p.n + 1) \
                or self.car_mode == nat.CAR_HOST or (self.car_mode == nat.CAR_SAFE and not nat.car_safe_supported(R, p.n + 1)):
            return None
        done = p.ws.pop("final_done", None)
        if done is not None:
            if done[:3] != (idx_cur.data_ptr(), R, row_offset):
                raise nat.SoberHipError("level_final: the final level that rode in level_loop was another one")
            return done[3], done[4]
        job = self._job(p, S)
        if not job.car_ws:
            return None
        dev = self.device
        job.mu = mu.data_ptr()
        fin = self._final_job(p, S, mu, row_offset)
        out_idx, out_w = p._fin_out
        st = torch.cuda.current_stream(dev)
        nat.level_final_job(job, fin, idx_cur, R, st.cuda_stream)
        st.synchronize()
        n_keep = int(p.ws["h_flags_np"][S])
        if n_keep < 0:
            if job.car_mode == nat.CAR_DEFAULT and nat.car_safe_supported(R, p.n + 1):
                self._car_downgrade(nat.CAR_SAFE, "final level")
                return self.level_final(p, idx_cur, R, S, mu, row_offset)
            self._car_downgrade(nat.CAR_HOST, "final level")
            return None
        return out_idx[:n_keep], out_w[:n_keep]

    def level_flat(self, p: Plan):
        return p.ws["XT"]

    def level_car(self, p: Plan, S: int):
        job = self._job(p, S)
        st = torch.cuda.current_stream(self.device)
        nat.level_car(job, st.cuda_stream)
        st.synchronize()
        flags = p.ws["h_flags_np"]
        if int(flags[S]) < 0:
            if not nat.level_car_retry(job, st.cuda_stream):
                self._car_downgrade(nat.CAR_HOST, "level")
                return None
            self._car_downgrade(nat.CAR_SAFE, "level")
        return p.ws["keep_rank"][:S], p.ws["w_star"], flags[:S].copy(), int(flags[S])

    def level_barycentres(self, p: Plan):
        return p.ws["X_tmp"], p.ws["tot"]

    def level_trace(self, p: Plan):
        return self.to_host(p.ws["X_tmp"], p.ws["tot"], p.ws["w_star"])

    def direct_columns(self, p: Plan, idx, count):
        dev = self.device
        K = torch.empty(p.Mtot, count, dtype=torch.float64, device=dev)
        if p.cand is not None:
            nat.pairwise(p.kind, p.rows.data, p.rows.norm, p.cand.data, p.cand.norm, idx, count, p.rows.dt,
                         p.spec.outputscale, K)
        else:
            sc = torch.empty(count, p.rows.dt, dtype=torch.float64, device=dev)
            nat.scale_points_idx(p.cand_raw, idx, count, p.spec.lengthscale, sc)
            nat.pairwise(p.kind, p.rows.data, p.rows.norm, sc, None, None, count, p.rows.dt, p.spec.outputscale, K)
        if p.weighted:
            K = K * p.wmul[idx[:count].long()].unsqueeze(0)
        Xtr = torch.empty(p.n, count, dtype=torch.float64, device=dev)
        nat.dgemm(p.P, K, Xtr)
        out = torch.empty(count, p.n, dtype=torch.float64, device=dev)
        nat.barycentres(Xtr, p.n, count, None, out)
        return out

    def barycentres(self, Xtr, tot):
        n, S = Xtr.shape
        out = torch.empty(S, n, dtype=torch.float64, device=self.device)
        nat.barycentres(Xtr, n, S, tot, out)
        return out

    def car_supported(self, N, m):
        if not nat.car_supported(N, m) or self.car_mode == nat.CAR_HOST:
            return False
        return self.car_mode == nat.CAR_DEFAULT or nat.car_safe_supported(N, m)

    def car_device(self, X, mu_in, phi_out=None):
        N = X.shape[0]
        dev = self.device
        keep_rank = torch.empty(N, dtype=torch.int32, device=dev)
        w_star = torch.empty(N, dtype=torch.float64, device=dev)
        n_keep = torch.empty(1, dtype=torch.int32, device=dev)
        mu_out = torch.empty(N, dtype=torch.float64, device=dev)
        nat.car_device(X, mu_in, keep_rank, w_star, n_keep, mu_out, phi_out=phi_out, mode=min(self.car_mode, nat.CAR_SAFE))
        return keep_rank, w_star, n_keep, mu_out

    def car_device_checked(self, X, mu_in, phi_out=None, also=()):
        N, m = X.shape[0], X.shape[1] + 1
        for _ in range(2):
            if not self.car_supported(N, m):
                return None
            keep_rank, w_star, n_keep_d, _mu = self.car_device(X, mu_in, phi_out)
            host = self.to_host(keep_rank, n_keep_d, *also)
            n_keep = int(host[1][0])
            if n_keep >= 0:
                return keep_rank, w_star, host[0], n_keep, host[2:]
            self._car_downgrade(nat.CAR_SAFE if nat.car_safe_supported(N, m) and self.car_mode == nat.CAR_DEFAULT
                                else nat.CAR_HOST, "Caratheodory step")
        return None

    def car_obj_device(self, X, mu_in, obj_head=None):
        N, n1f = X.shape
        dev = self.device
        n1 = n1f + 1
        if self.obj_null_kernel and bool(nat.load().sober_null_vector_supported(n1f - 1)) and self.car_supported(N, n1f + 1):
            for _ in range(2):
                flags = torch.empty(2 * N + 3, dtype=torch.int32, device=dev)
                keep_rank, n_keep, nk1_d, status, kr1 = flags[:N], flags[N:N + 1], flags[N + 1:N + 2], flags[N + 2:N + 3], flags[N + 3:]
                w1 = torch.empty(N, dtype=torch.float64, device=dev)
                mu1 = torch.empty(N, dtype=torch.float64, device=dev)
                nat.car_device(X, mu_in, kr1, w1, nk1_d, mu1, mode=min(self.car_mode, nat.CAR_SAFE))
                null_row = torch.empty(N, dtype=torch.float64, device=dev)
                nat.null_vector(X, n1f - 1, kr1, nk1_d, n1, null_row, status)
                ocol = (X[:, n1f - 1] if obj_head is None else obj_head[:N]).contiguous()
                w_star = torch.empty(N, dtype=torch.float64, device=dev)
                nat.second_elimination_rows(null_row, ocol, w1, kr1, nk1_d, n1, keep_rank, w_star, n_keep, status=status)
                (fl_h,) = self.to_host(flags)
                keep_h, nk_h, nk1, st_h, kr1_h = fl_h[:N], int(fl_h[N]), int(fl_h[N + 1]), int(fl_h[N + 2]), fl_h[N + 3:]
                if nk1 == n1 and st_h == 0:
                    return keep_rank, w_star, keep_h, nk_h, (kr1_h, w1, n1)
                if nk1 >= 0:
                    return None
                self._car_downgrade(nat.CAR_SAFE if nat.car_safe_supported(N, n1f + 1) and self.car_mode == nat.CAR_DEFAULT
                                    else nat.CAR_HOST, "Caratheodory step")
                if not self.car_supported(N, n1f + 1):
                    return None
            return None
        for _ in range(2):
            if not self.car_supported(N, n1f + 1) or not self.car_supported(n1, n1f):
                return None
            kr1, w1, nk1_d, _mu = self.car_device(X, mu_in)
# ... 37 lines not shown
```

### sober_amd/csrc/level_exec.cpp

```cpp
#include <hip/hip_runtime.h>
#include <cstdio>
#include <cstdlib>

#include "../../include/sober_hip.h"
#include "switches.hpp"

extern "C" int sober_level_job_size(void) { return (int)sizeof(sober_level_job); }
extern "C" int sober_obj_job_size(void) { return (int)sizeof(sober_obj_job); }

#define LX_TRY(call)                 \
    do {                             \
        const int rc_ = (call);      \
        if (rc_ != 0) return rc_;    \
    } while (0)

static inline bool lx_timed_in_dispatch(const sober_level_job* j) {
    return j->variant == SOBER_LEVEL_MFMA || j->variant == SOBER_LEVEL_TANI;
}
#define LX_EVENTS_BEFORE(A, B)                                                                   \
    if ((A) && (B)) {                                                                            \
        if (lx_timed_in_dispatch(j)) { LX_TRY(sober_set_launch_events((A), (B))); }              \
        else { const hipError_t e_ = hipEventRecord((hipEvent_t)(A), (hipStream_t)stream); if (e_ != hipSuccess) return (int)e_; } \
    }
#define LX_EVENTS_AFTER(A, B)                                                                    \
    if ((A) && (B) && !lx_timed_in_dispatch(j)) {                                                \
        const hipError_t e_ = hipEventRecord((hipEvent_t)(B), (hipStream_t)stream);              \
        if (e_ != hipSuccess) return (int)e_;                                                    \
    }

static int lx_reduce(const sober_level_job* j, const int32_t* idx, int64_t pos0, int64_t count, int S, int n_chunks,
                     double* partG, double* partTot, int64_t tot_limit, void* stream) {
    switch (j->variant) {
        case SOBER_LEVEL_MFMA:
            return sober_level_reduce_mfma(j->kind, (const double*)j->rows, j->n_rows, (const double*)j->cand, j->dim,
                                           idx, pos0, count, S, j->mu, j->wmul, j->outputscale, n_chunks, partG, S, 0,
                                           partTot, tot_limit, stream);
        case SOBER_LEVEL_VALU:
            return sober_level_reduce(j->kind, j->rows, j->rows_norm, j->n_rows, j->cand, j->cand_norm, j->dim, idx,
                                      pos0, count, S, j->mu, j->wmul, j->outputscale, n_chunks, partG, S, 0, partTot,
                                      tot_limit, stream);
        case SOBER_LEVEL_TANI:
            return sober_level_reduce_tani(j->rows, j->rows_norm, j->n_rows, j->cand, j->cand_norm, j->dim, idx, pos0, count,
                                           S, j->mu, j->wmul, j->outputscale, n_chunks, partG, S, 0, partTot, tot_limit,
                                           stream);
        case SOBER_LEVEL_GATHER:
            return sober_level_gather((const double*)j->cand, j->n_rows, j->kmat_ld, idx, pos0, count, S, j->mu,
                                      j->wmul, n_chunks, partG, S, 0, partTot, tot_limit, stream);
        default:
            return SOBER_E_ARG;
    }
}

extern "C" int sober_level_class_depth(int variant, int n_rows, int64_t R, int S) {
    if (n_rows <= 0 || R <= 0 || S <= 0 || (S & 1) || sober::switches().level_no_classes) return 0;
    if (variant != SOBER_LEVEL_MFMA && variant != SOBER_LEVEL_TANI) return 0;
    int D = 0;
    while (D < SOBER_CLASS_MAX_DEPTH) {
        const int64_t SC = (int64_t)S << (D + 1);
        if (R % SC != 0 || R / SC < 2) break;
        int slots;
        if (variant == SOBER_LEVEL_MFMA) {
            const int wpt = sober_level_class_wpt(n_rows, R / SC, (int)SC);
            slots = wpt > 0 ? sober_level_class_slots(wpt) : 0;
        } else {
            slots = sober_level_chunks_tani(n_rows, 0, R, (int)SC);
            const int64_t rb = (n_rows + 255) / 256;
            const int64_t wg_c = (int64_t)slots * ((SC + 15) / 16 + 1) * rb;
            const int64_t wg_0 = (int64_t)sober_level_chunks_tani(n_rows, 0, R, S) * ((S + 15) / 16 + 1) * rb;
            if (slots > 0 && wg_c * 100 < wg_0 * 85) break;
        }
        if (slots <= 0 || slots * (1 << (D + 1)) > SOBER_LEVEL_MAX_CHUNKS) break;
        ++D;
    }
    return D;
}

static int lx_class_first(const sober_level_job* j, void* stream) {
    const int S = j->S, D = j->class_depth, CL = 1 << D, SC = S * CL;
    if ((j->variant != SOBER_LEVEL_MFMA && j->variant != SOBER_LEVEL_TANI) || D < 1 || D > SOBER_CLASS_MAX_DEPTH ||
        j->pos0 != 0 || j->count % SC != 0 || j->count / SC < 2 || !j->Gc[0] || !j->totc[0])
        return SOBER_E_ARG;
    int nch;
    if (j->variant == SOBER_LEVEL_MFMA) {
        const int wpt = sober_level_class_wpt(j->n_rows, j->count / SC, SC);
        if (wpt <= 0) return wpt < 0 ? wpt : SOBER_E_ARG;
        nch = sober_level_class_slots(wpt);
        if (nch <= 0 || nch * CL > SOBER_LEVEL_MAX_CHUNKS) return SOBER_E_WS;
        LX_EVENTS_BEFORE(j->ev[0], j->ev[1])
        LX_TRY(sober_level_reduce_mfma_wpt(j->kind, (const double*)j->rows, j->n_rows, (const double*)j->cand, j->dim, j->idx,
                                           j->count, SC, j->mu, j->wmul, j->outputscale, wpt, nch, j->partG, SC, j->partTot,
                                           stream));
    } else {
        nch = sober_level_chunks_tani(j->n_rows, 0, j->count, SC);
        if (nch <= 0 || nch * CL > SOBER_LEVEL_MAX_CHUNKS) return nch <= 0 ? nch : SOBER_E_WS;
        LX_EVENTS_BEFORE(j->ev[0], j->ev[1])
        LX_TRY(sober_level_reduce_tani(j->rows, j->rows_norm, j->n_rows, j->cand, j->cand_norm, j->dim, j->idx, 0, j->count, SC,
                                       j->mu, j->wmul, j->outputscale, nch, j->partG, SC, 0, j->partTot, j->count, stream));
    }
    return sober_class_sum(j->partG, j->partTot, nch, j->n_rows, S, CL, j->Gc[0], j->totc[0], j->G, j->tot, stream);
}

extern "C" int sober_level_moments(const sober_level_job* j, void* stream) {
    if (!j || !j->G || !j->tot || j->n_rows <= 0 || j->S <= 0 || j->n <= 0 || j->phase < 0 || j->phase > 2)
        return SOBER_E_ARG;
    const int S = j->S;
    if (j->phase == 2) {
        if (!j->P || !j->Xtr) return SOBER_E_ARG;
        return sober_dgemm(0, 0, j->n, S, j->n_rows, 1.0, j->P, j->n_rows, j->G, S, 0.0, j->Xtr, S, stream);
    }
    if (!j->cand || !j->idx || !j->mu || !j->partG || !j->partTot || (j->phase == 0 && (!j->P || !j->Xtr)))
        return SOBER_E_ARG;
    if (j->count <= 0 || j->pos0 < 0 || j->E < 0) return SOBER_E_ARG;
    if (j->phase == 1 && j->class_depth > 0) return lx_class_first(j, stream);
    const int64_t ES = j->E * S;
    const bool mfma = j->variant == SOBER_LEVEL_MFMA;
    const bool tani_k = j->variant == SOBER_LEVEL_TANI;
    const int n_chunks = mfma ? sober_level_parts_mfma(j->n_rows, j->pos0, j->count, S)
                              : (tani_k ? sober_level_chunks_tani(j->n_rows, j->pos0, j->count, S)
                                        : sober_level_chunks(j->n_rows, j->pos0, j->count, S));
    if (n_chunks <= 0 || n_chunks > SOBER_LEVEL_MAX_CHUNKS) return n_chunks <= 0 ? n_chunks : SOBER_E_WS;
    LX_EVENTS_BEFORE(j->ev[0], j->ev[1])
    LX_TRY(lx_reduce(j, j->idx, j->pos0, j->count, S, n_chunks, j->partG, j->partTot, ES, stream));
    LX_EVENTS_AFTER(j->ev[0], j->ev[1])
    const int64_t lo = j->pos0 > ES ? j->pos0 : ES;
    const int64_t n_left = j->pos0 + j->count - lo;
    int n_xchunks = 0;
    if (n_left > 0) {
        if (!j->extraG || !j->extraTot) return SOBER_E_ARG;
        n_xchunks = mfma ? sober_level_parts_mfma(j->n_rows, 0, n_left, SOBER_LEVEL_XS)
                         : (tani_k ? sober_level_chunks_tani(j->n_rows, 0, n_left, SOBER_LEVEL_XS)
                                   : sober_level_chunks(j->n_rows, 0, n_left, SOBER_LEVEL_XS));
        if (n_xchunks <= 0 || n_xchunks > SOBER_LEVEL_MAX_CHUNKS) return n_xchunks <= 0 ? n_xchunks : SOBER_E_WS;
        LX_EVENTS_BEFORE(j->ev[2], j->ev[3])
        LX_TRY(lx_reduce(j, j->idx + (lo - j->pos0), 0, n_left, SOBER_LEVEL_XS, n_xchunks, j->extraG, j->extraTot,
                         n_left, stream));
        LX_EVENTS_AFTER(j->ev[2], j->ev[3])
    }
    LX_TRY(sober_sum_partials(j->partG, j->partTot, n_chunks, j->n_rows, S, S, n_left > 0 ? j->extraG : nullptr,
                              n_left > 0 ? j->extraTot : nullptr, n_xchunks, SOBER_LEVEL_XS, j->G, S, j->tot, stream));
    if (j->phase == 1) return 0;
    return sober_dgemm(0, 0, j->n, S, j->n_rows, 1.0, j->P, j->n_rows, j->G, S, 0.0, j->Xtr, S, stream);
}

extern "C" int sober_level_car(const sober_level_job* j, void* stream) {
    if (!j || !j->Xtr || !j->tot || !j->X_tmp || !j->keep_rank || !j->w_star || !j->mu_out || !j->car_ws || !j->h_flags)
        return SOBER_E_ARG;
    const int S = j->S, n = j->n;
    if (!sober_car_supported(S, n + 1)) return SOBER_E_DIM;
    LX_TRY(sober_barycentres(j->Xtr, S, n, S, j->tot, j->X_tmp, stream));
    LX_TRY(sober_car_device_ex(j->X_tmp, n, S, n + 1, j->tot, j->keep_rank, j->w_star, j->keep_rank + S, j->mu_out,
                               nullptr, j->car_ws, j->car_ws_bytes, j->car_mode, stream));
    const hipError_t e = hipMemcpyAsync(j->h_flags, j->keep_rank, sizeof(int32_t) * (size_t)(S + 1),
                                        hipMemcpyDeviceToHost, (hipStream_t)stream);
    return e == hipSuccess ? 0 : (int)e;
}

extern "C" int sober_level_car_retry(sober_level_job* j, void* stream) {
    if (!j || !j->X_tmp || !j->tot || !j->keep_rank || !j->w_star || !j->mu_out || !j->car_ws || !j->h_flags) return SOBER_E_ARG;
    const int S = j->S, n = j->n;
    if (j->car_mode == SOBER_CAR_SAFE || !sober_car_safe_supported(S, n + 1)) return SOBER_E_EXCHANGE;
    j->car_mode = SOBER_CAR_SAFE;
    LX_TRY(sober_car_device_ex(j->X_tmp, n, S, n + 1, j->tot, j->keep_rank, j->w_star, j->keep_rank + S, j->mu_out,
                               nullptr, j->car_ws, j->car_ws_bytes, SOBER_CAR_SAFE, stream));
    hipError_t e = hipMemcpyAsync(j->h_flags, j->keep_rank, sizeof(int32_t) * (size_t)(S + 1), hipMemcpyDeviceToHost,
                                  (hipStream_t)stream);
    if (e == hipSuccess) e = hipStreamSynchronize((hipStream_t)stream);
    if (e != hipSuccess) return (int)e;
    return j->h_flags[S] < 0 ? SOBER_E_EXCHANGE : 0;
}

static int lx_chunks(int n_rows, int64_t e_total, int S) { return sober_level_parts_mfma_cap(n_rows, e_total, S); }

static int lx_loop_queued(sober_level_job* j, const sober_obj_job* oj, int64_t R0, int32_t* idx_a, int32_t* idx_b,
                          int first_sums_ready, void** events, int max_levels, int64_t* level_R, int* done, int64_t* R_out,
                          void* stream) {
    const int S = j->S, n = j->n, b = n + 1;
    *done = 0;
    *R_out = R0;
    int64_t Rlo[SOBER_LEVEL_QUEUE + 1], Rub[SOBER_LEVEL_QUEUE + 1];
    Rlo[0] = Rub[0] = R0;
    int L = 0;
    while (L < SOBER_LEVEL_QUEUE && L < max_levels && Rlo[L] > S) {
        Rlo[L + 1] = (Rlo[L] / S) * b;
        Rub[L + 1] = (Rub[L] / S) * b + (Rlo[L] == Rub[L] ? Rub[L] % S : S - 1);
        ++L;
    }
    if (L < 2) return 0;
    if (!sober_car_supported(S, oj ? b + 1 : b)) return SOBER_E_DIM;
    if (oj && (!sober_null_vector_supported(n) || b + 1 > 512)) return SOBER_E_DIM;
    int D = 0;
    if (first_sums_ready && j->class_depth > 0 && !oj) {
        D = j->class_depth;
        if ((j->variant != SOBER_LEVEL_MFMA && j->variant != SOBER_LEVEL_TANI) || D > SOBER_CLASS_MAX_DEPTH || D >= L ||
            R0 % ((int64_t)S << D) != 0 ||
            !j->Gc[0] || !j->Gc[1] || !j->totc[0] || !j->totc[1] || !j->cls_scale || !j->cls_sof)
            return SOBER_E_ARG;
    }
    hipStream_t st = (hipStream_t)stream;
    if (!first_sums_ready) LX_TRY(sober_set_i64(j->dR, R0, stream));
    hipError_t e = hipSuccess;
    for (int l = 0; l < L; ++l) {
        int32_t* cur = (l & 1) ? idx_b : idx_a;
        int32_t* nxt = (l & 1) ? idx_a : idx_b;
        for (int k = 0; k < 4; ++k) j->ev[k] = events ? events[4 * l + k] : nullptr;
        if (l >= 1 && l <= D) {
            LX_TRY(sober_class_derive_queued(j->Gc[(l - 1) & 1], j->totc[(l - 1) & 1], j->n_rows, S, 1 << (D - l + 1),
                                             j->cls_scale, j->cls_sof, j->Gc[l & 1], j->totc[l & 1], j->G, j->tot, j->dR + l,
                                             stream));
        } else if (!(l == 0 && first_sums_ready)) {
            const bool tani = j->variant == SOBER_LEVEL_TANI;
            const int64_t e_ub = (Rub[l] + S - 1) / S, ex_ub = (S - 1 + SOBER_LEVEL_XS - 1) / SOBER_LEVEL_XS;
            const int nch = tani ? sober_level_chunks_tani_cap(j->n_rows, e_ub, S) : lx_chunks(j->n_rows, e_ub, S);
            const int nxch = tani ? sober_level_chunks_tani_cap(j->n_rows, ex_ub, SOBER_LEVEL_XS) : lx_chunks(j->n_rows, ex_ub, SOBER_LEVEL_XS);
            if (nch <= 0 || nch > SOBER_LEVEL_MAX_CHUNKS || nxch <= 0 || nxch > SOBER_LEVEL_MAX_CHUNKS) return SOBER_E_WS;
            LX_EVENTS_BEFORE(j->ev[0], j->ev[1])
            if (j->ev[0] && j->ev[1]) j->ev_used[0] |= 1ull << l;
            const bool no_left = Rlo[l] == Rub[l] && Rub[l] % S == 0;
            if (tani && !no_left && !sober::switches().level_two_launches) {
                LX_TRY(sober_level_reduce_tani_queued_pair(j->rows, j->rows_norm, j->n_rows, j->cand, j->cand_norm, j->dim, cur,
                                                           Rub[l], S, SOBER_LEVEL_XS, j->mu, j->wmul, j->outputscale, nch,
                                                           j->partG, S, j->partTot, nxch, j->extraG, j->extraTot, j->dR + l,
                                                           stream));
            } else if (tani) {
                LX_TRY(sober_level_reduce_tani_queued(j->rows, j->rows_norm, j->n_rows, j->cand, j->cand_norm, j->dim, cur,
                                                      Rub[l], S, S, 0, j->mu, j->wmul, j->outputscale, nch, j->partG, S,
                                                      j->partTot, j->dR + l, stream));
                if (!no_left) {
                    LX_EVENTS_BEFORE(j->ev[2], j->ev[3])
                    if (j->ev[2] && j->ev[3]) j->ev_used[1] |= 1ull << l;
                    LX_TRY(sober_level_reduce_tani_queued(j->rows, j->rows_norm, j->n_rows, j->cand, j->cand_norm, j->dim, cur,
                                                          S - 1, SOBER_LEVEL_XS, S, 1, j->mu, j->wmul, j->outputscale, nxch,
                                                          j->extraG, SOBER_LEVEL_XS, j->extraTot, j->dR + l, stream));
                }
            } else if (no_left || sober::switches().level_two_launches) {
                LX_TRY(sober_level_reduce_mfma_queued(j->kind, (const double*)j->rows, j->n_rows, (const double*)j->cand,
                                                      j->dim, cur, Rub[l], S, S, 0, j->mu, j->wmul, j->outputscale, nch,
                                                      j->partG, S, j->partTot, j->dR + l, stream));
                if (!no_left) {
                    LX_EVENTS_BEFORE(j->ev[2], j->ev[3])
                    if (j->ev[2] && j->ev[3]) j->ev_used[1] |= 1ull << l;
                    LX_TRY(sober_level_reduce_mfma_queued(j->kind, (const double*)j->rows, j->n_rows, (const double*)j->cand,
                                                          j->dim, cur, S - 1, SOBER_LEVEL_XS, S, 1, j->mu, j->wmul,
                                                          j->outputscale, nxch, j->extraG, SOBER_LEVEL_XS, j->extraTot,
                                                          j->dR + l, stream));
                }
            } else {
                LX_TRY(sober_level_reduce_mfma_queued_pair(j->kind, (const double*)j->rows, j->n_rows, (const double*)j->cand,
                                                           j->dim, cur, Rub[l], S, SOBER_LEVEL_XS, j->mu, j->wmul,
                                                           j->outputscale, nch, j->partG, S, j->partTot, nxch, j->extraG,
                                                           j->extraTot, j->dR + l, stream));
            }
            LX_TRY(sober_sum_partials_queued(j->partG, j->partTot, j->n_rows, S, S, j->extraG, j->extraTot,
                                             SOBER_LEVEL_XS, j->G, S, j->tot, j->dR + l, tani ? 1 : 0, stream));
        }
        if (oj) {
            LX_TRY(sober_dgemm_coldiv_t(n, S, j->n_rows, j->P, j->n_rows, j->G, S, j->tot, oj->X_tmp, n + 1, stream));
            LX_TRY(sober_obj_set_sums_queued(oj->obj, j->mu, cur, S, j->dR + l, (l == 0 && first_sums_ready) ? R0 : (int64_t)-1,
                                             j->tot, oj->X_tmp + n, n + 1, oj->ocol, stream));
            LX_TRY(sober_car_device_ex(oj->X_tmp, n + 1, S, n + 2, j->tot, oj->kr1, oj->w1, oj->nk1, j->mu_out, nullptr,
                                       j->car_ws, j->car_ws_bytes, j->car_mode, stream));
            LX_TRY(sober_null_vector(oj->X_tmp, n + 1, S, n, oj->kr1, oj->nk1, n + 2, oj->null_row, oj->status, stream));
            LX_TRY(sober_second_elimination_rows(oj->null_row, oj->ocol, oj->w1, oj->kr1, oj->nk1, oj->status, n + 2, S,
                                                 j->keep_rank, j->w_star, j->keep_rank + S, stream));
        } else {
            LX_TRY(sober_dgemm_coldiv_t(n, S, j->n_rows, j->P, j->n_rows, j->G, S, j->tot, j->X_tmp, n, stream));
            LX_TRY(sober_car_device_ex(j->X_tmp, n, S, n + 1, j->tot, j->keep_rank, j->w_star, j->keep_rank + S, j->mu_out,
                                       nullptr, j->car_ws, j->car_ws_bytes, j->car_mode, stream));
        }
        LX_TRY(sober_level_update_queued_ex(cur, Rub[l], S, j->keep_rank, j->w_star, j->tot, j->mu, nxt, j->dR + l,
                                            j->dR + l + 1, Rub[l + 1], l < D ? b : 0, j->cls_scale, j->cls_sof,
                                            (l == 0 && first_sums_ready) ? R0 : (int64_t)-1, stream));
    }
    for (int k = 0; k < 4; ++k) j->ev[k] = nullptr;
    e = hipMemcpyAsync(j->h_dR, j->dR, sizeof(int64_t) * (size_t)(L + 1), hipMemcpyDeviceToHost, st);
    if (e != hipSuccess) return (int)e;
    e = hipStreamSynchronize(st);
    if (e != hipSuccess) return (int)e;
    j->h_dR[0] = R0;
    int d = 0;
    while (d < L && j->h_dR[d + 1] >= 0) { level_R[d] = j->h_dR[d]; ++d; }
    *done = d;
    *R_out = j->h_dR[d];
    return 0;
}

extern "C" int sober_level_loop_obj(sober_level_job* j, const sober_obj_job* oj, int64_t R, int32_t* idx_a, int32_t* idx_b,
                                    int first_sums_ready, int max_levels, int64_t* level_R, int32_t* n_levels, int64_t* R_final,
                                    int32_t* in_b, void* stream) {
    if (!j || !oj || !idx_a || !idx_b || !level_R || !n_levels || !R_final || !in_b || !j->mu || R <= 0 || !j->dR || !j->h_dR)
        return SOBER_E_ARG;
    if (!oj->obj || !oj->X_tmp || !oj->ocol || !oj->kr1 || !oj->w1 || !oj->nk1 || !oj->null_row || !oj->status) return SOBER_E_ARG;
    if (j->variant != SOBER_LEVEL_MFMA && j->variant != SOBER_LEVEL_TANI) return SOBER_E_ARG;
    int done = 0;
    int64_t R_after = R;
    j->ev_used[0] = j->ev_used[1] = 0;
    LX_TRY(lx_loop_queued(j, oj, R, idx_a, idx_b, first_sums_ready, nullptr, max_levels, level_R, &done, &R_after, stream));
    *n_levels = done;
    *R_final = R_after;
    *in_b = (done & 1) ? 1 : 0;
    return 0;
}

extern "C" int sober_level_loop(sober_level_job* j, int64_t R, int32_t* idx_a, int32_t* idx_b, int first_sums_ready,
                                void** events, int max_levels, int64_t* level_R, int32_t* n_levels, int64_t* R_final,
                                int32_t* in_b, void* stream) {
    if (!j || !idx_a || !idx_b || !level_R || !n_levels || !R_final || !in_b || !j->h_flags || !j->mu || R <= 0)
        return SOBER_E_ARG;
    const int S = j->S;
    int32_t *cur = idx_a, *nxt = idx_b;
    int levels = 0;
    j->ev_used[0] = j->ev_used[1] = 0;
    if (j->dR && j->h_dR && (j->variant == SOBER_LEVEL_MFMA || (j->variant == SOBER_LEVEL_TANI && !sober::switches().tani_no_queue))) {
        int done = 0;
        int64_t R_after = R;
        LX_TRY(lx_loop_queued(j, nullptr, R, idx_a, idx_b, first_sums_ready, events, max_levels, level_R, &done, &R_after, stream));
        if (done > 0) {
            levels = done;
            R = R_after;
            first_sums_ready = 0;
            if (done & 1) { cur = idx_b; nxt = idx_a; }
        }
    }
    while (R > S) {
        if (levels >= max_levels) return SOBER_E_WS;
        const int64_t E = R / S, r = R - E * S;
        j->idx = cur; j->pos0 = 0; j->count = R; j->E = E;
        j->phase = (levels == 0 && first_sums_ready) ? 2 : 0;
        for (int k = 0; k < 4; ++k) j->ev[k] = (events && levels < max_levels) ? events[4 * levels + k] : nullptr;
        if (j->phase != 2 && levels < 64) {
            if (j->ev[0] && j->ev[1]) j->ev_used[0] |= 1ull << levels;
            if (j->ev[2] && j->ev[3] && r > 0) j->ev_used[1] |= 1ull << levels;
        }
        LX_TRY(sober_level_moments(j, stream));
        LX_TRY(sober_level_car(j, stream));
        const hipError_t e = hipStreamSynchronize((hipStream_t)stream);
        if (e != hipSuccess) return (int)e;
        if (j->h_flags[S] < 0) {
            const int rc = sober_level_car_retry(j, stream);
            if (rc != 0) {
                *n_levels = levels; *R_final = R; *in_b = (cur == idx_b) ? 1 : 0;
                for (int k = 0; k < 4; ++k) j->ev[k] = nullptr;
                j->phase = 0;
                return rc;
            }
        }
        const int n_keep = j->h_flags[S];
        const bool last_kept = j->h_flags[S - 1] >= 0;
        const int64_t R_new = E * n_keep + (last_kept ? r : 0);
        level_R[levels++] = R;
        if (R_new >= R) { *n_levels = levels; return SOBER_E_NOPROGRESS; }
        LX_TRY(sober_level_update(cur, 0, R, S, E, j->keep_rank, j->w_star, j->tot, n_keep, j->mu, nxt, 0, stream));
        int32_t* t = cur; cur = nxt; nxt = t;
        R = R_new;
    }
    for (int k = 0; k < 4; ++k) j->ev[k] = nullptr;
    j->phase = 0;
    *n_levels = levels;
    *R_final = R;
    *in_b = (cur == idx_b) ? 1 : 0;
    return 0;
}

extern "C" int sober_level_final_job(const sober_level_job* j, const sober_final_job* f, const int32_t* idx, int R,
                                     void* stream) {
    if (!j || !f || !f->rows_sc || (!f->cand_sc && (!f->cand_raw || !f->ls || !f->sc_buf)) || !idx || !f->K || !f->mu_live ||
        !f->out_idx || !f->out_w || !j->P || !j->Xtr || !j->X_tmp || !j->keep_rank || !j->w_star || !j->mu_out || !j->car_ws ||
        !j->h_flags || !j->mu)
        return SOBER_E_ARG;
    const int S = j->S, n = j->n;
    if (R <= n + 1 || R > S || f->N <= 0) return SOBER_E_ARG;
    if (!sober_car_supported(R, n + 1)) return SOBER_E_DIM;
    if (f->cand_sc) {
        LX_TRY(sober_pairwise(j->kind, f->rows_sc, f->rows_norm, j->n_rows, f->cand_sc, f->cand_norm, idx, R, f->dt,
                              j->outputscale, f->K, R, stream));
    } else {
        LX_TRY(sober_scale_points_idx(f->cand_raw, idx, R, f->d_raw, f->ld_raw, f->ls, f->ls_len, f->sc_buf, f->dt, j->mu,
                                      f->mu_live, stream));
        LX_TRY(sober_pairwise(j->kind, f->rows_sc, f->rows_norm, j->n_rows, f->sc_buf, nullptr, nullptr, R, f->dt,
                              j->outputscale, f->K, R, stream));
    }
    LX_TRY(sober_dgemm_coldiv_t(n, R, j->n_rows, j->P, j->n_rows, f->K, R, nullptr, j->X_tmp, n, stream));
    if (f->cand_sc) LX_TRY(sober_gather_f64(j->mu, idx, R, f->mu_live, stream));
    LX_TRY(sober_car_device_ex(j->X_tmp, n, R, n + 1, f->mu_live, j->keep_rank, j->w_star, j->keep_rank + S, j->mu_out,
                               nullptr, j->car_ws, j->car_ws_bytes, j->car_mode, stream));
    LX_TRY(sober_final_commit(idx, R, j->keep_rank, j->w_star, j->keep_rank + S, f->row_offset, j->mu, f->N, f->out_idx,
                              f->out_w, stream));
    hipError_t e = hipMemcpyAsync(j->h_flags + S, j->keep_rank + S, sizeof(int32_t), hipMemcpyDeviceToHost, (hipStream_t)stream);
    return e == hipSuccess ? 0 : (int)e;
}

extern "C" int sober_level_final(const sober_level_job* j, const void* rows_sc, const double* rows_norm,
                                 const void* cand_sc, const double* cand_norm, int dt, const int32_t* idx, int R,
                                 int64_t N, int64_t row_offset, double* K, double* mu_live, int64_t* out_idx,
                                 double* out_w, void* stream) {
    if (!cand_sc) return SOBER_E_ARG;
    sober_final_job f = {};
    f.rows_sc = rows_sc; f.rows_norm = rows_norm; f.cand_sc = cand_sc; f.cand_norm = cand_norm; f.dt = dt;
    f.N = N; f.row_offset = row_offset; f.K = K; f.mu_live = mu_live; f.out_idx = out_idx; f.out_w = out_w;
    return sober_level_final_job(j, &f, idx, R, stream);
}

extern "C" int sober_final_job_size(void) { return (int)sizeof(sober_final_job); }

extern "C" int sober_level_loop_final(sober_level_job* j, sober_final_job* f, int64_t R, int32_t* idx_a, int32_t* idx_b,
                                      int first_sums_ready, void** events, int max_levels, int64_t* level_R,
                                      int32_t* n_levels, int64_t* R_final, int32_t* in_b, void* stream) {
    if (f) f->done = 0;
    const int rc = sober_level_loop(j, R, idx_a, idx_b, first_sums_ready, events, max_levels, level_R, n_levels, R_final,
                                    in_b, stream);
    if (rc != 0 || !f) return rc;
    const int S = j->S, n = j->n;
    const int64_t Rf = *R_final;
    if (Rf <= n + 1 || Rf > S) return 0;
    if (j->car_mode != SOBER_CAR_DEFAULT && j->car_mode != SOBER_CAR_SAFE) return 0;
    if (!sober_car_supported((int)Rf, n + 1)) return 0;
    if (j->car_mode == SOBER_CAR_SAFE && !sober_car_safe_supported((int)Rf, n + 1)) return 0;
    LX_TRY(sober_level_final_job(j, f, *in_b ? idx_b : idx_a, (int)Rf, stream));
    const hipError_t e = hipStreamSynchronize((hipStream_t)stream);
    if (e != hipSuccess) return (int)e;
    f->done = 1;
    return 0;
}

extern "C" int sober_record_event_pair(void* ev0, void* ev1, void* stream) {
    if (!ev0 || !ev1) return SOBER_E_ARG;
    hipError_t e = hipEventRecord((hipEvent_t)ev0, (hipStream_t)stream);
    if (e == hipSuccess) e = hipEventRecord((hipEvent_t)ev1, (hipStream_t)stream);
    return e == hipSuccess ? 0 : (int)e;
}

static int64_t lx_survivors_before(int64_t p, int S, int64_t E, const int32_t* kept_prefix, int n_keep, bool last_kept) {
    const int64_t ES = E * S;
    if (p <= ES) return (p / S) * n_keep + kept_prefix[p % S];
    return E * (int64_t)n_keep + (last_kept ? (p - ES) : 0);
}

extern "C" int sober_level_loop_sharded(sober_level_job* j, int rank, int world, int64_t* bounds, int32_t* idx_a,
                                        int32_t* idx_b, int first_sums_ready, sober_allreduce_fn allreduce,
                                        void* comm, int64_t R_stop, int max_levels, int64_t* level_R,
                                        int32_t* n_levels, int32_t* in_b, void* stream) {
    if (!j || !bounds || !idx_a || !idx_b || !allreduce || !level_R || !n_levels || !in_b || !j->h_flags || !j->mu ||
        world <= 0 || rank < 0 || rank >= world || world > 1024)
        return SOBER_E_ARG;
    const int S = j->S, n = j->n;
    if (j->Xtr + (size_t)n * S != j->tot) return SOBER_E_ARG;
    if (!sober_car_supported(S, n + 1)) return SOBER_E_DIM;
    hipStream_t st = (hipStream_t)stream;
    int32_t *cur = idx_a, *nxt = idx_b;
    int levels = 0;
    int32_t kept_prefix[1024 + 1];
    if (S > 1024) return SOBER_E_DIM;
    while (bounds[world] > S && bounds[world] > R_stop) {
        if (levels >= max_levels) return SOBER_E_WS;
        const int64_t R = bounds[world], E = R / S, r = R - E * S;
        const int64_t pos0 = bounds[rank], count = bounds[rank + 1] - bounds[rank];
        if (levels == 0 && first_sums_ready) {
            j->phase = 2;
            LX_TRY(sober_level_moments(j, stream));
        } else if (count > 0) {
            j->idx = cur; j->pos0 = pos0; j->count = count; j->E = E; j->phase = 0;
            LX_TRY(sober_level_moments(j, stream));
        } else {
            hipError_t e = hipMemsetAsync(j->Xtr, 0, sizeof(double) * ((size_t)n * S + S), st);
            if (e != hipSuccess) return (int)e;
        }
        if (world > 1 || comm) LX_TRY(allreduce(comm, j->Xtr, (int64_t)n * S + S, stream));
        LX_TRY(sober_level_car(j, stream));
        hipError_t e = hipStreamSynchronize(st);
        if (e != hipSuccess) return (int)e;
        if ((void*)allreduce == (void*)&sober_peer_allreduce_f64 && comm) {
            const int prc = sober_peer_status(comm, nullptr, 0, stream);
            if (prc != 0) { *n_levels = levels; *in_b = (cur == idx_b) ? 1 : 0; j->phase = 0; return prc; }
        }
        if (j->h_flags[S] < 0) {
            const int rc = sober_level_car_retry(j, stream);
            if (rc != 0) { *n_levels = levels; *in_b = (cur == idx_b) ? 1 : 0; j->phase = 0; return rc; }
        }
        const int n_keep = j->h_flags[S];
        const bool last_kept = j->h_flags[S - 1] >= 0;
        const int64_t R_new = E * n_keep + (last_kept ? r : 0);
        level_R[levels++] = R;
        if (R_new >= R) { *n_levels = levels; return SOBER_E_NOPROGRESS; }
        kept_prefix[0] = 0;
        for (int s = 0; s < S; ++s) kept_prefix[s + 1] = kept_prefix[s] + (j->h_flags[s] >= 0 ? 1 : 0);
        int64_t nb_lo = lx_survivors_before(bounds[rank], S, E, kept_prefix, n_keep, last_kept);
        if (count > 0)
            LX_TRY(sober_level_update(cur, pos0, count, S, E, j->keep_rank, j->w_star, j->tot, n_keep, j->mu, nxt,
                                      nb_lo, stream));
        for (int q = 0; q <= world; ++q) bounds[q] = lx_survivors_before(bounds[q], S, E, kept_prefix, n_keep, last_kept);
        int32_t* t = cur; cur = nxt; nxt = t;
    }
    j->phase = 0;
    *n_levels = levels;
    *in_b = (cur == idx_b) ? 1 : 0;
    return 0;
}
```

### sober_amd/csrc/misc.hip

```cpp
#include "common.hpp"
#include "internal.hpp"

namespace sober {

__global__ void k_scale_points(const double* __restrict__ X, int64_t n, int d, int64_t ldx,
                               const double* __restrict__ ls, int ls_len, double* __restrict__ out,
                               int dt) {
    const int64_t t = (int64_t)blockIdx.x * blockDim.x + threadIdx.x;
    if (t >= n * dt) return;
    const int64_t i = t / dt;
    const int j = (int)(t % dt);
    double v = 0.0;
    if (j < d) v = X[i * ldx + j] / ls[ls_len == 1 ? 0 : j];
    out[t] = v;
}

__global__ void k_scale_points2(const double* __restrict__ Xa, int64_t na, int64_t lda, const double* __restrict__ Xb, int64_t nb,
                                int64_t ldb, int d, const double* __restrict__ ls, int ls_len, double* __restrict__ out, int dt) {
    const int64_t t = (int64_t)blockIdx.x * blockDim.x + threadIdx.x;
    if (t >= (na + nb) * dt) return;
    const int64_t i = t / dt;
    const int j = (int)(t % dt);
    double v = 0.0;
    if (j < d) v = (i < na ? Xa[i * lda + j] : Xb[(i - na) * ldb + j]) / ls[ls_len == 1 ? 0 : j];
// ... 325 lines not shown
    for (int64_t p = s + (int64_t)tid * S; p < R; p += (int64_t)256 * S) { const int c = idx[p]; acc += obj[c] * mu[c]; }
    if (s == S - 1)
        for (int64_t q = ES + tid; q < R; q += 256) { const int c = idx[q]; acc += obj[c] * mu[c]; }
    s_p[tid] = acc;
    __syncthreads();
    for (int h = 128; h > 0; h >>= 1) {
        if (tid < h) s_p[tid] += s_p[tid + h];
        __syncthreads();
    }
    if (tid == 0) {
        const double v = s_p[0] / tot[s];
        xcol[(size_t)s * ldx] = v;
        ocol[s] = v;
    }
}

__global__ void k_projection_left(const double* __restrict__ Ut, int s, int M, const double* __restrict__ mean,
                                  double* __restrict__ P, int ldp) {
    const int t = blockIdx.x * blockDim.x + threadIdx.x;
    if (t >= s * M) return;
    const int r = t / M, c = t - r * M;
    P[(size_t)r * ldp + c] = mean ? Ut[t] * mean[c] : Ut[t];
}

__global__ void k_transpose_projection(const double* __restrict__ Q, int s, int M, const double* __restrict__ mean,
                                       double* __restrict__ Ut, double* __restrict__ P, int ldp) {
    const int t = blockIdx.x * blockDim.x + threadIdx.x;
    if (t >= s * M) return;
    const int r = t / M, c = t - r * M;
    const double v = Q[(size_t)c * s + r];
    Ut[t] = v;
    if (P != nullptr) P[(size_t)r * ldp + c] = mean ? v * mean[c] : v;
}

__global__ void k_i64_to_i32(const int64_t* __restrict__ in, int64_t n, int32_t* __restrict__ out) {
    const int64_t t = (int64_t)blockIdx.x * blockDim.x + threadIdx.x;
    if (t < n) out[t] = (int32_t)in[t];
}

__global__ void k_predict_finish(const double* __restrict__ KX, const double* __restrict__ V, int n_obs,
                                 int64_t N, int64_t ld, const double* __restrict__ mean, double kxx_const,
                                 const double* __restrict__ norms, double outputscale, double noise,
                                 double* __restrict__ var_out, double eta, double* __restrict__ lfi_out,
                                 int log_flag) {
    const int64_t j = (int64_t)blockIdx.x * blockDim.x + threadIdx.x;
    if (j >= N) return;
    double q0 = 0.0, q1 = 0.0;
    int i = 0;
    for (; i + 1 < n_obs; i += 2) {
        q0 = fma(KX[(size_t)i * ld + j], V[(size_t)i * ld + j], q0);
        q1 = fma(KX[(size_t)(i + 1) * ld + j], V[(size_t)(i + 1) * ld + j], q1);
    }
    if (i < n_obs) q0 = fma(KX[(size_t)i * ld + j], V[(size_t)i * ld + j], q0);
    double kxx = kxx_const;
    if (norms != nullptr) {
        const double n2 = norms[j];
        kxx = (n2 + 1e-6) / (1e-6 + n2) * outputscale;
    }
    const double var = kxx - (q0 + q1) + noise;
    var_out[j] = var;
    if (lfi_out != nullptr) {
        const double z = (mean[j] - eta) / sqrt(var);
        double p = 0.5 * erfc(-z * 0.70710678118654752440);
        if (log_flag) p = log(p + 1.1920928955078125e-07);
        lfi_out[j] = p;
    }
}

constexpr int CW_BLOCKS = 256, CW_THREADS = 256;

__global__ __launch_bounds__(CW_THREADS) void k_clean_partial(double* __restrict__ w, int64_t n,
                                                              double eps, double* __restrict__ part) {
    __shared__ double s[CW_THREADS];
    double acc = 0.0;
    for (int64_t i = (int64_t)blockIdx.x * CW_THREADS + threadIdx.x; i < n;
         i += (int64_t)CW_BLOCKS * CW_THREADS) {
        double v = w[i];
        if (v < eps) v = 0.0;
        if (isinf(v)) v = eps;
        if (isnan(v)) v = eps;
        w[i] = v;
        acc += v;
    }
    s[threadIdx.x] = acc;
    __syncthreads();
    for (int o = CW_THREADS / 2; o > 0; o >>= 1) {
        if (threadIdx.x < o) s[threadIdx.x] += s[threadIdx.x + o];
        __syncthreads();
    }
    if (threadIdx.x == 0) part[blockIdx.x] = s[0];
}

__global__ __launch_bounds__(CW_BLOCKS) void k_clean_scale(double* __restrict__ w, int64_t n, const double* __restrict__ part) {
    __shared__ double s[CW_BLOCKS];
    s[threadIdx.x] = part[threadIdx.x];
    __syncthreads();
    for (int o = CW_BLOCKS / 2; o > 0; o >>= 1) {
        if (threadIdx.x < o) s[threadIdx.x] += s[threadIdx.x + o];
        __syncthreads();
    }
    const double tot = s[0];
    const int64_t i = (int64_t)blockIdx.x * blockDim.x + threadIdx.x;
    if (i >= n) return;
    w[i] = (tot != 0.0) ? w[i] / tot : 1.0 / (double)n;
}

__global__ void k_wkde_draw(const double* __restrict__ eps, int64_t n, int d, const int32_t* __restrict__ comp,
                            const double* __restrict__ Xobs, int ldx, const double* __restrict__ L,
                            const double* __restrict__ lo, const double* __restrict__ hi,
                            double* __restrict__ x, int32_t* __restrict__ inside) {
    extern __shared__ double sL[];
    for (int t = threadIdx.x; t < d * d; t += blockDim.x) sL[t] = L[t];
    __syncthreads();
    const int64_t r = (int64_t)blockIdx.x * blockDim.x + threadIdx.x;
    if (r >= n) return;
    const double* e = eps + r * d;
    const double* loc = Xobs + (size_t)comp[r] * ldx;
    bool ok = true;
    for (int k = 0; k < d; ++k) {
        double acc = 0.0;
        for (int j = 0; j <= k; ++j) acc = fma(sL[k * d + j], e[j], acc);
        const double v = loc[k] + acc;
        x[r * d + k] = v;
        if (lo) ok = ok && !(v < lo[k]) && !(v > hi[k]);
    }
    if (inside) inside[r] = ok ? 1 : 0;
}

}

#include <cstdlib>
using namespace sober;

static inline unsigned nblk(int64_t n, int b) { return (unsigned)((n + b - 1) / b); }

extern "C" int sober_abi_version(void) { return SOBER_ABI_VERSION; }
extern "C" int sober_diag_build(void) {
#ifdef SOBER_DIAG_BUILD
    return 1;
#else
    return 0;
#endif
}

namespace sober {
static Switches read_switches() {
    Switches w;
    w.level_two_launches = getenv("SOBER_LEVEL_TWO_LAUNCHES") != nullptr;
    w.tani_no_queue = getenv("SOBER_TANI_NO_QUEUE") != nullptr;
    w.car_force_giveup = getenv("SOBER_CAR_FORCE_GIVEUP") != nullptr;
    w.car_unfused = getenv("SOBER_CAR_UNFUSED") != nullptr;
    w.level_no_classes = getenv("SOBER_LEVEL_NO_CLASSES") != nullptr;
    w.car_exact_ratio = getenv("SOBER_CAR_EXACT_RATIO") != nullptr;
    return w;
}
static Switches g_switches = read_switches();
const Switches& switches() { return g_switches; }
}
extern "C" int sober_reload_switches(void) { sober::g_switches = sober::read_switches(); return 0; }
namespace sober {
LaunchEvents& launch_events() {
    static thread_local LaunchEvents le;
    return le;
}
}
extern "C" int sober_set_launch_events(void* start, void* stop) {
    if ((start == nullptr) != (stop == nullptr)) return SOBER_E_ARG;
    sober::launch_events() = sober::LaunchEvents{(hipEvent_t)start, (hipEvent_t)stop};
    return 0;
}

extern "C" int sober_padded_dim(int d) {
    if (d <= 0) return SOBER_E_ARG;
    const int dts[] = {4, 8, 12, 16, 20, 24, 32};
    for (int v : dts)
        if (d <= v) return v;
    return SOBER_E_DIM;
}

extern "C" int sober_bit_words(int d) {
    if (d <= 0) return SOBER_E_ARG;
    const int w = (d + 63) / 64;
    const int ws[] = {1, 2, 4, 8, 16, 32};
    for (int v : ws)
        if (w <= v) return v;
    return SOBER_E_DIM;
}

__global__ void k_box_muller(const double* __restrict__ u, int64_t numel, double* __restrict__ out) {
    const int64_t t = (int64_t)blockIdx.x * blockDim.x + threadIdx.x;
    const int64_t full = numel / 16;
    const bool tail = (numel % 16) != 0;
    const int64_t npairs = (full + (tail ? 1 : 0)) * 8;
    if (t >= npairs) return;
    const int64_t g = t >> 3;
    const int j = (int)(t & 7);
    const bool is_tail = g == full;
    const int64_t ub = is_tail ? numel : g * 16, ob = is_tail ? numel - 16 : g * 16;
    const double u1 = 1.0 - u[ub + j], u2 = u[ub + j + 8];
    const double radius = sqrt(-2.0 * log(u1));
    const double theta = 6.283185307179586 * u2;
    double sn, cs;
    sincos(theta, &sn, &cs);
    const int64_t keep_below = tail ? numel - 16 : numel;
    if (is_tail || ob + j < keep_below) out[ob + j] = radius * cs;
    if (is_tail || ob + j + 8 < keep_below) out[ob + j + 8] = radius * sn;
}

extern "C" int sober_box_muller(const double* u, int64_t numel, double* out, void* stream) {
    if (!u || !out || numel < 16) return SOBER_E_ARG;
    const int64_t npairs = ((numel + 15) / 16) * 8;
    hipLaunchKernelGGL(k_box_muller, dim3(nblk(npairs, 256)), dim3(256), 0, (hipStream_t)stream, u, numel, out);
    LAUNCH_CHECK();
    return 0;
}

extern "C" int sober_scale_points(const double* X, int64_t n, int d, int64_t ldx,
                                  const double* lengthscale, int ls_len, double* out, int dt,
                                  void* stream) {
    if (!X || !lengthscale || !out || n <= 0 || d <= 0 || dt < d || ldx < d) return SOBER_E_ARG;
    if (ls_len != 1 && ls_len != d) return SOBER_E_ARG;
    hipLaunchKernelGGL(k_scale_points, dim3(nblk(n * dt, 256)), dim3(256), 0, (hipStream_t)stream, X,
                       n, d, ldx, lengthscale, ls_len, out, dt);
    LAUNCH_CHECK();
    return 0;
}

int sober::scale_points2(const double* Xa, int64_t na, int64_t lda, const double* Xb, int64_t nb, int64_t ldb, int d,
                         const double* lengthscale, int ls_len, double* out, int dt, void* stream) {
    if (!Xa || !Xb || !lengthscale || !out || na <= 0 || nb <= 0 || d <= 0 || dt < d || lda < d || ldb < d) return SOBER_E_ARG;
    if (ls_len != 1 && ls_len != d) return SOBER_E_ARG;
    hipLaunchKernelGGL(k_scale_points2, dim3(nblk((na + nb) * dt, 256)), dim3(256), 0, (hipStream_t)stream, Xa, na, lda, Xb, nb,
                       ldb, d, lengthscale, ls_len, out, dt);
    LAUNCH_CHECK();
    return 0;
}

int sober::transpose_projection(const double* Q, int s, int M, const double* mean, double* Ut, double* P, int ldp, void* stream) {
    if (!Q || !Ut || s <= 0 || M <= 0 || (P && ldp < M)) return SOBER_E_ARG;
    hipLaunchKernelGGL(k_transpose_projection, dim3(nblk((int64_t)s * M, 256)), dim3(256), 0, (hipStream_t)stream, Q, s, M, mean,
                       Ut, P, ldp);
    LAUNCH_CHECK();
    return 0;
}

extern "C" int sober_scale_points_idx(const double* X, const int32_t* idx, int64_t n, int d, int64_t ldx,
                                      const double* lengthscale, int ls_len, double* out, int dt, const double* gather_src,
                                      double* gather_out, void* stream) {
    if (!X || !idx || !lengthscale || !out || n <= 0 || d <= 0 || dt < d || ldx < d) return SOBER_E_ARG;
    if ((ls_len != 1 && ls_len != d) || (gather_src && !gather_out)) return SOBER_E_ARG;
    hipLaunchKernelGGL(k_scale_points_idx, dim3(nblk(n * dt, 256)), dim3(256), 0, (hipStream_t)stream, X, idx, n, d, ldx,
                       lengthscale, ls_len, out, dt, gather_src, gather_out);
    LAUNCH_CHECK();
    return 0;
}

extern "C" int sober_pack_bits(const double* X, int64_t n, int d, int64_t ldx, uint64_t* words,
                               int nwords, double* norms, int32_t* bad_flag, void* stream) {
    if (!X || !words || !norms || !bad_flag || n <= 0 || d <= 0 || nwords * 64 < d || ldx < d)
        return SOBER_E_ARG;
    hipLaunchKernelGGL(k_pack_bits, dim3(nblk(n, 4)), dim3(256), 0, (hipStream_t)stream, X, n, d, ldx,
                       words, nwords, norms, bad_flag);
    LAUNCH_CHECK();
    return 0;
}

extern "C" int sober_pairwise(int kind, const void* a, const double* a_norm, int64_t m, const void* b,
                              const double* b_norm, const int32_t* idx, int64_t n, int dt,
                              double outputscale, double* out, int64_t ldo, void* stream) {
    if (!a || !b || !out || m <= 0 || n <= 0 || dt <= 0 || ldo < n || m > 65535) return SOBER_E_ARG;
    if (kind == SOBER_KIND_TANIMOTO && (!a_norm || !b_norm)) return SOBER_E_ARG;
    dim3 grid(nblk(n, 256), (unsigned)m);
    hipStream_t st = (hipStream_t)stream;
    const double* A = (const double*)a;
    const double* B = (const double*)b;
    switch (kind) {
        case SOBER_KIND_RBF:
            hipLaunchKernelGGL(k_pairwise<SOBER_KIND_RBF>, grid, dim3(256), 0, st, A, a_norm, m, B,
                               b_norm, idx, n, dt, outputscale, out, ldo);
            break;
        case SOBER_KIND_MATERN52:
            hipLaunchKernelGGL(k_pairwise<SOBER_KIND_MATERN52>, grid, dim3(256), 0, st, A, a_norm, m, B,
                               b_norm, idx, n, dt, outputscale, out, ldo);
            break;
        case SOBER_KIND_TANIMOTO:
            hipLaunchKernelGGL(k_pairwise<SOBER_KIND_TANIMOTO>, grid, dim3(256), 0, st, A, a_norm, m, B,
                               b_norm, idx, n, dt, outputscale, out, ldo);
            break;
        default: return SOBER_E_ARG;
    }
    LAUNCH_CHECK();
    return 0;
}

template <int KIND, int DT>
static int launch_mv(const void* a, const double* an, const double* v, int64_t m, const void* b,
                     const double* bn, int64_t n, double os, double c0, double* out, hipStream_t st) {
    hipLaunchKernelGGL((k_kernel_matvec<KIND, DT>), dim3(nblk(n, 256)), dim3(256), 0, st,
                       (const double*)a, an, v, m, (const double*)b, bn, n, os, c0, out);
    LAUNCH_CHECK();
    return 0;
}

extern "C" int sober_kernel_matvec(int kind, const void* a, const double* a_norm, const double* v,
                                   int64_t m, const void* b, const double* b_norm, int64_t n, int dt,
                                   double outputscale, double c0, double* out, void* stream) {
// ... 260 lines not shown
```

### sober_amd/csrc/switches.hpp

```cpp
#pragma once
namespace sober {
struct Switches {
    bool level_two_launches;
    bool tani_no_queue;
    bool car_force_giveup;
    bool car_unfused;
    bool car_exact_ratio;
    bool level_no_classes;
};
const Switches& switches();
}
```

Baseline: 27.45 million.

## Switch late recombination levels to precomputed per-candidate Nyström feature rows

Once the surviving candidate count falls below a threshold, the level loop builds a dense feature matrix (kernel row times projection P) for the survivors in one pass. Later levels then compute the weighted barycentres by gathering and summing those cached feature rows, instead of rerunning the kernel-moment reduction and the dgemm column-divide. This trades one up-front feature build, plus extra workspace, for cheaper per-level moments at small R. It adds new kernels, a candidate-to-row map, and an ABI bump. The feature path covers only RBF and Matérn kernels with the MFMA variant and can be disabled with an environment switch.

New measurement: 27.78 million (median of 6 runs). About the same (+1.2%).

```diff
diff --git a/include/sober_hip.h b/include/sober_hip.h
--- a/include/sober_hip.h
+++ b/include/sober_hip.h
@@ -7,7 +7,7 @@
 extern "C" {
 #endif
 
-#define SOBER_ABI_VERSION 7
+#define SOBER_ABI_VERSION 8
 
 #define SOBER_KIND_RBF       0
 #define SOBER_KIND_MATERN52  1
@@ -300,8 +300,23 @@
     int32_t class_depth;
     double* Gc[2]; double* totc[2];
     double* cls_scale; int32_t* cls_sof;
+    double* feat_F; double* feat_sc; int32_t* feat_map;
+    int64_t feat_rows, feat_pool;
+    int32_t feat_level;
 } sober_level_job;
 #define SOBER_LEVEL_QUEUE 24
+#define SOBER_FEAT_MAX_R 16384
+int sober_feat_supported(int kind, int dt, int n);
+int sober_feat_first_level(int64_t R0, int S, int n, int D, int max_levels, int64_t feat_rows, int32_t* n_queued);
+int64_t sober_feat_max_r(void);
+int sober_feat_build(int kind, const double* rows_sc, int n_rows, int dt, const double* cand_sc, const double* cand_raw,
+                     int64_t ld_raw, int d_raw, const double* ls, int ls_len, double outputscale, const double* P, int n,
+                     const int32_t* cur, int64_t R_ub, int S, const int64_t* dR, int64_t pool, double* sc_buf, double* F,
+                     int ldf, int32_t* fmap, void* stream);
+int sober_feat_level_queued(const double* F, int ldf, int64_t f_rows, const int32_t* fmap, int n, int S, const int32_t* cur,
+                            const double* mu, const int64_t* dR, int64_t R_ub, double* X_tmp, double* tot, void* stream);
+int sober_feat_gather(const double* F, int ldf, int64_t f_rows, const int32_t* fmap, int n, const int32_t* idx, int R,
+                      double* X_tmp, const double* mu, double* mu_live, void* stream);
 int sober_level_moments(const sober_level_job* job, void* stream);
 int sober_level_car(const sober_level_job* job, void* stream);
 int sober_level_car_retry(sober_level_job* job, void* stream);
diff --git a/sober_amd/_engine.py b/sober_amd/_engine.py
--- a/sober_amd/_engine.py
+++ b/sober_amd/_engine.py
@@ -328,6 +328,10 @@
             self._tick("levels_device", t0)
             if R > S:
                 return self._finish_replicated(plan, idx_cur, bounds, mu, num_pts, U)
+        feat, lvl = None, -1
+        if levels is not None and not sharded and obj is None and not self.force_host_car and R > S \
+                and getattr(ops, "level_feature_plan", None) is not None and ops.car_supported(S, n + 1):
+            feat = ops.level_feature_plan(plan, R, S, mu, sums_ready)
         while True:
             if R <= n + 1:
                 return self._finish_small(mu)
@@ -336,8 +340,11 @@
 
             E = R // S
             r = R - E * S
+            lvl += 1
             t0 = time.perf_counter()
-            if sums_ready:
+            if feat is not None and feat[0] <= lvl < feat[1]:
+                Xtr, tot = ops.level_moments_features(plan, idx_cur, R, S, mu, build=lvl == feat[0])
+            elif sums_ready:
                 Xtr, tot = ops.level_moments(plan, idx_cur, pos0, count, S, E, mu, phase=2)
                 sums_ready = False
             else:
diff --git a/sober_amd/_native.py b/sober_amd/_native.py
--- a/sober_amd/_native.py
+++ b/sober_amd/_native.py
@@ -8,7 +8,7 @@
 
 _HERE = os.path.dirname(os.path.abspath(__file__))
 LIB_PATH = os.environ.get("SOBER_HIP_LIB") or os.path.join(_HERE, "libsober_hip.so")
-ABI_VERSION = 7
+ABI_VERSION = 8
 
 KIND_RBF, KIND_MATERN52, KIND_TANIMOTO = 0, 1, 2
 KIND_BY_NAME = {"rbf": KIND_RBF, "matern52": KIND_MATERN52, "tanimoto": KIND_TANIMOTO}
@@ -165,6 +165,13 @@
     "sober_final_scatter": (_i32, [_vp, _i32, _vp, _vp, _i64, _vp, _vp, _vp, _vp]),
     "sober_level_final": (_i32, [_vp, _vp, _vp, _vp, _vp, _i32, _vp, _i32, _i64, _i64, _vp, _vp, _vp, _vp, _vp]),
     "sober_level_final_job": (_i32, [_vp, _vp, _vp, _i32, _vp]),
+    "sober_feat_supported": (_i32, [_i32, _i32, _i32]),
+    "sober_feat_max_r": (_i64, []),
+    "sober_feat_first_level": (_i32, [_i64, _i32, _i32, _i32, _i32, _i64, _vp]),
+    "sober_feat_build": (_i32, [_i32, _vp, _i32, _i32, _vp, _vp, _i64, _i32, _vp, _i32, _f64, _vp, _i32, _vp, _i64, _i32, _vp,
+                                _i64, _vp, _vp, _i32, _vp, _vp]),
+    "sober_feat_level_queued": (_i32, [_vp, _i32, _i64, _vp, _i32, _i32, _vp, _vp, _vp, _i64, _vp, _vp, _vp]),
+    "sober_feat_gather": (_i32, [_vp, _i32, _i64, _vp, _i32, _vp, _i32, _vp, _vp, _vp, _vp]),
     "sober_level_loop": (_i32, [_vp, _i64, _vp, _vp, _i32, _vp, _i32, _vp, _vp, _vp, _vp, _vp]),
 }
 
@@ -216,6 +223,7 @@
         ("car_mode", _i32),
         ("ev_used", C.c_uint64 * 2),
         ("class_depth", _i32), ("Gc", _vp * 2), ("totc", _vp * 2), ("cls_scale", _vp), ("cls_sof", _vp),
+        ("feat_F", _vp), ("feat_sc", _vp), ("feat_map", _vp), ("feat_rows", _i64), ("feat_pool", _i64), ("feat_level", _i32),
     ]
 
 E_DIM = -2
@@ -905,6 +913,38 @@
            "sober_level_final")
 
 
+def feat_max_r() -> int:
+    return int(load().sober_feat_max_r())
+
+
+def feat_first_level(R0: int, S: int, n: int, D: int, feat_rows: int):
+    L = _i32(0)
+    lf = load().sober_feat_first_level(int(R0), int(S), int(n), int(D), MAX_LEVELS, int(feat_rows), C.byref(L))
+    return (int(lf), int(L.value)) if lf >= 1 else None
+
+
+def feat_build(kind, rows_sc, cand_sc, cand_raw, lengthscale, dt, outputscale, P, cur, R_ub, S, dR, sc_buf, F, fmap):
+    _req(cur, torch.int32, "cur"); _req(dR, torch.int64, "dR"); _req(fmap, torch.int32, "fmap"); _req(F, torch.float64, "F")
+    n = P.shape[0]
+    raw = cand_sc is None
+    _check(load().sober_feat_build(kind, rows_sc.data_ptr(), P.shape[1], dt, _ptr(cand_sc), _ptr(cand_raw),
+                                   cand_raw.stride(0) if raw else 0, cand_raw.shape[1] if raw else 0, _ptr(lengthscale),
+                                   lengthscale.numel() if raw else 0, float(outputscale), P.data_ptr(), n, cur.data_ptr(),
+                                   int(R_ub), int(S), dR.data_ptr(), fmap.numel(), sc_buf.data_ptr(), F.data_ptr(), F.stride(0),
+                                   fmap.data_ptr(), _stream(F)), "sober_feat_build")
+
+
+def feat_level_queued(F, fmap, n, S, cur, mu, dR, R_ub, X_tmp, tot):
+    _check(load().sober_feat_level_queued(F.data_ptr(), F.stride(0), F.shape[0], fmap.data_ptr(), n, S, cur.data_ptr(),
+                                          mu.data_ptr(), dR.data_ptr(), int(R_ub), X_tmp.data_ptr(), tot.data_ptr(),
+                                          _stream(F)), "sober_feat_level_queued")
+
+
+def feat_gather(F, fmap, n, idx, R, X_tmp, mu=None, mu_live=None):
+    _check(load().sober_feat_gather(F.data_ptr(), F.stride(0), F.shape[0], fmap.data_ptr(), n, idx.data_ptr(), int(R),
+                                    X_tmp.data_ptr(), _ptr(mu), _ptr(mu_live), _stream(F)), "sober_feat_gather")
+
+
 def level_final_job(job: LevelJob, fin: "FinalJob", idx, R: int, stream: int):
     _check(load().sober_level_final_job(C.addressof(job), C.addressof(fin), idx.data_ptr(), int(R), stream), "sober_level_final_job")
 
diff --git a/sober_amd/_ops_hip.py b/sober_amd/_ops_hip.py
--- a/sober_amd/_ops_hip.py
+++ b/sober_amd/_ops_hip.py
@@ -29,6 +29,7 @@
         self.queue_obj_levels = True
         self.lazy_scaled_pool = True
         self.last_levels = None
+        self._feat_bufs = {}
         self._probe_mc = torch.cuda.get_device_properties(self.device).multi_processor_count >= 256
         self.car_mode = nat.CAR_DEFAULT
 
diff --git a/sober_amd/_ops_levels.py b/sober_amd/_ops_levels.py
--- a/sober_amd/_ops_levels.py
+++ b/sober_amd/_ops_levels.py
@@ -168,8 +168,10 @@
         p.ws.pop("final_done", None)
         if not p.weighted and getattr(p, "Kmat", None) is None and self.car_mode != nat.CAR_HOST and job.car_ws:
             fin = self._final_job(p, S, mu, row_offset)
+            self._feat_ws(p, job, mu)
         level_R, R_final, in_b, gave_up = nat.level_loop(job, R, idx_cur, idx_new, sums_ready, events, nat._stream(mu), fin)
-        self.last_levels = {"R": [int(v) for v in level_R], "derived": int(job.class_depth) if sums_ready else 0}
+        self.last_levels = {"R": [int(v) for v in level_R], "derived": int(job.class_depth) if sums_ready else 0,
+                            "features_from": int(job.feat_level)}
         if fin is not None and fin.done:
             n_keep = int(p.ws["h_flags_np"][S])
             if n_keep >= 0:
@@ -202,6 +204,41 @@
         if job.car_mode > min(self.car_mode, nat.CAR_SAFE):
             self._car_downgrade(nat.CAR_SAFE, "sharded level loop")
         return (idx_new, idx_cur, new_bounds) if in_b else (idx_cur, idx_new, new_bounds)
+
+    def _feat_ws(self, p: Plan, job, mu):
+        if job.variant != nat.LEVEL_MFMA or not job.dR or p.kind not in (nat.KIND_RBF, nat.KIND_MATERN52):
+            job.feat_F = job.feat_sc = job.feat_map = None
+            return
+        rows, n, dt, N = nat.feat_max_r(), int(job.n), int(p.rows.dt), int(mu.numel())
+        w = self._feat_bufs
+        for name, numel, dtype in (("F", rows * n, torch.float64), ("sc", rows * dt, torch.float64), ("map", N, torch.int32)):
+            t = w.get(name)
+            if t is None or t.numel() < numel:
+                w[name] = torch.zeros(numel, dtype=dtype, device=self.device)
+        job.feat_F, job.feat_sc, job.feat_map = w["F"].data_ptr(), w["sc"].data_ptr(), w["map"].data_ptr()
+        job.feat_rows, job.feat_pool = rows, w["map"].numel()
+
+    def level_feature_plan(self, p: Plan, R: int, S: int, mu, sums_ready: bool):
+        job = self._job(p, S)
+        if p.weighted or getattr(p, "Kmat", None) is not None or self.car_mode == nat.CAR_HOST or not job.car_ws \
+                or not job.dR or job.wmul:
+            return None
+        self._feat_ws(p, job, mu)
+        if not job.feat_F or not bool(nat.load().sober_feat_supported(p.kind, p.rows.dt, job.n)):
+            return None
+        return nat.feat_first_level(R, S, job.n, int(job.class_depth) if sums_ready else 0, job.feat_rows)
+
+    def level_moments_features(self, p: Plan, idx, R: int, S: int, mu, build: bool):
+        job, w, n = self._job(p, S), self._feat_bufs, p.n
+        rows = int(job.feat_rows)
+        F, dR = w["F"][:rows * n].view(rows, n), p.ws["dR"]
+        dR[:1].fill_(R)
+        if build:
+            nat.feat_build(p.kind, p.rows.data, p.cand.data if p.cand is not None else None, p.cand_raw,
+                           p.spec.lengthscale, p.rows.dt, p.spec.outputscale, p.P, idx, R, S, dR, w["sc"], F, w["map"])
+        nat.feat_level_queued(F, w["map"], n, S, idx, mu, dR, R, p.ws["X_tmp"], p.ws["tot"])
+        job.mu, job.phase = mu.data_ptr(), 3
+        return p.ws["Xtr"], p.ws["tot"]
 
     def _final_job(self, p: Plan, S: int, mu, row_offset: int = 0):
         dev = self.device
diff --git a/sober_amd/csrc/level_exec.cpp b/sober_amd/csrc/level_exec.cpp
--- a/sober_amd/csrc/level_exec.cpp
+++ b/sober_amd/csrc/level_exec.cpp
@@ -147,7 +147,7 @@
         return SOBER_E_ARG;
     const int S = j->S, n = j->n;
     if (!sober_car_supported(S, n + 1)) return SOBER_E_DIM;
-    LX_TRY(sober_barycentres(j->Xtr, S, n, S, j->tot, j->X_tmp, stream));
+    if (j->phase != 3) LX_TRY(sober_barycentres(j->Xtr, S, n, S, j->tot, j->X_tmp, stream));
     LX_TRY(sober_car_device_ex(j->X_tmp, n, S, n + 1, j->tot, j->keep_rank, j->w_star, j->keep_rank + S, j->mu_out,
                                nullptr, j->car_ws, j->car_ws_bytes, j->car_mode, stream));
     const hipError_t e = hipMemcpyAsync(j->h_flags, j->keep_rank, sizeof(int32_t) * (size_t)(S + 1),
@@ -169,15 +169,7 @@
     return j->h_flags[S] < 0 ? SOBER_E_EXCHANGE : 0;
 }
 
-static int lx_chunks(int n_rows, int64_t e_total, int S) { return sober_level_parts_mfma_cap(n_rows, e_total, S); }
-
-static int lx_loop_queued(sober_level_job* j, const sober_obj_job* oj, int64_t R0, int32_t* idx_a, int32_t* idx_b,
-                          int first_sums_ready, void** events, int max_levels, int64_t* level_R, int* done, int64_t* R_out,
-                          void* stream) {
-    const int S = j->S, n = j->n, b = n + 1;
-    *done = 0;
-    *R_out = R0;
-    int64_t Rlo[SOBER_LEVEL_QUEUE + 1], Rub[SOBER_LEVEL_QUEUE + 1];
+static int lx_level_bounds(int64_t R0, int S, int b, int max_levels, int64_t* Rlo, int64_t* Rub) {
     Rlo[0] = Rub[0] = R0;
     int L = 0;
     while (L < SOBER_LEVEL_QUEUE && L < max_levels && Rlo[L] > S) {
@@ -185,6 +177,37 @@
         Rub[L + 1] = (Rub[L] / S) * b + (Rlo[L] == Rub[L] ? Rub[L] % S : S - 1);
         ++L;
     }
+    return L;
+}
+
+static int lx_feat_level(const int64_t* Rub, int L, int D, int n, int64_t feat_rows) {
+    if (sober::switches().level_no_features) return L;
+    const int64_t passes = ((n + 15) / 16 + 6) / 7;
+    for (int l = D + 1; l < L; ++l)
+        if (Rub[l] <= feat_rows && Rub[l] * passes <= sober::switches().feat_max_r) return l;
+    return L;
+}
+
+extern "C" int sober_feat_first_level(int64_t R0, int S, int n, int D, int max_levels, int64_t feat_rows, int32_t* n_queued) {
+    if (R0 <= 0 || S <= 0 || n <= 0 || D < 0 || !n_queued) return SOBER_E_ARG;
+    int64_t Rlo[SOBER_LEVEL_QUEUE + 1], Rub[SOBER_LEVEL_QUEUE + 1];
+    const int L = lx_level_bounds(R0, S, n + 1, max_levels, Rlo, Rub);
+    *n_queued = L;
+    if (L < 2 || D >= L) return -1;
+    const int lf = lx_feat_level(Rub, L, D, n, feat_rows);
+    return lf < L ? lf : -1;
+}
+
+static int lx_chunks(int n_rows, int64_t e_total, int S) { return sober_level_parts_mfma_cap(n_rows, e_total, S); }
+
+static int lx_loop_queued(sober_level_job* j, const sober_obj_job* oj, const sober_final_job* fj, int64_t R0, int32_t* idx_a,
+                          int32_t* idx_b, int first_sums_ready, void** events, int max_levels, int64_t* level_R, int* done,
+                          int64_t* R_out, void* stream) {
+    const int S = j->S, n = j->n, b = n + 1;
+    *done = 0;
+    *R_out = R0;
+    int64_t Rlo[SOBER_LEVEL_QUEUE + 1], Rub[SOBER_LEVEL_QUEUE + 1];
+    const int L = lx_level_bounds(R0, S, b, max_levels, Rlo, Rub);
     if (L < 2) return 0;
     if (!sober_car_supported(S, oj ? b + 1 : b)) return SOBER_E_DIM;
     if (oj && (!sober_null_vector_supported(n) || b + 1 > 512)) return SOBER_E_DIM;
@@ -196,6 +219,11 @@
             !j->Gc[0] || !j->Gc[1] || !j->totc[0] || !j->totc[1] || !j->cls_scale || !j->cls_sof)
             return SOBER_E_ARG;
     }
+    int lf = L;
+    if (fj && !oj && j->variant == SOBER_LEVEL_MFMA && !j->wmul && j->feat_F && j->feat_sc && j->feat_map && j->P &&
+        sober_feat_supported(j->kind, fj->dt, n) &&
+        (fj->cand_sc || (fj->cand_raw && fj->ls)) && fj->rows_sc && j->feat_pool >= fj->N)
+        lf = lx_feat_level(Rub, L, D, n, j->feat_rows);
     hipStream_t st = (hipStream_t)stream;
     if (!first_sums_ready) LX_TRY(sober_set_i64(j->dR, R0, stream));
     hipError_t e = hipSuccess;
@@ -207,6 +235,13 @@
             LX_TRY(sober_class_derive_queued(j->Gc[(l - 1) & 1], j->totc[(l - 1) & 1], j->n_rows, S, 1 << (D - l + 1),
                                              j->cls_scale, j->cls_sof, j->Gc[l & 1], j->totc[l & 1], j->G, j->tot, j->dR + l,
                                              stream));
+        } else if (l >= lf) {
+            if (l == lf)
+                LX_TRY(sober_feat_build(j->kind, (const double*)fj->rows_sc, j->n_rows, fj->dt, (const double*)fj->cand_sc,
+                                        fj->cand_raw, fj->ld_raw, fj->d_raw, fj->ls, fj->ls_len, j->outputscale, j->P, n, cur,
+                                        Rub[l], S, j->dR + l, j->feat_pool, j->feat_sc, j->feat_F, n, j->feat_map, stream));
+            LX_TRY(sober_feat_level_queued(j->feat_F, n, j->feat_rows, j->feat_map, n, S, cur, j->mu, j->dR + l, Rub[l], j->X_tmp,
+                                           j->tot, stream));
         } else if (!(l == 0 && first_sums_ready)) {
             const bool tani = j->variant == SOBER_LEVEL_TANI;
             const int64_t e_ub = (Rub[l] + S - 1) / S, ex_ub = (S - 1 + SOBER_LEVEL_XS - 1) / SOBER_LEVEL_XS;
@@ -263,7 +298,7 @@
             LX_TRY(sober_second_elimination_rows(oj->null_row, oj->ocol, oj->w1, oj->kr1, oj->nk1, oj->status, n + 2, S,
                                                  j->keep_rank, j->w_star, j->keep_rank + S, stream));
         } else {
-            LX_TRY(sober_dgemm_coldiv_t(n, S, j->n_rows, j->P, j->n_rows, j->G, S, j->tot, j->X_tmp, n, stream));
+            if (l < lf) LX_TRY(sober_dgemm_coldiv_t(n, S, j->n_rows, j->P, j->n_rows, j->G, S, j->tot, j->X_tmp, n, stream));
             LX_TRY(sober_car_device_ex(j->X_tmp, n, S, n + 1, j->tot, j->keep_rank, j->w_star, j->keep_rank + S, j->mu_out,
                                        nullptr, j->car_ws, j->car_ws_bytes, j->car_mode, stream));
         }
@@ -281,6 +316,7 @@
     while (d < L && j->h_dR[d + 1] >= 0) { level_R[d] = j->h_dR[d]; ++d; }
     *done = d;
     *R_out = j->h_dR[d];
+    if (lf < L && d >= lf && j->h_dR[lf] > S) j->feat_level = lf;
     return 0;
 }
 
@@ -294,16 +330,18 @@
     int done = 0;
     int64_t R_after = R;
     j->ev_used[0] = j->ev_used[1] = 0;
-    LX_TRY(lx_loop_queued(j, oj, R, idx_a, idx_b, first_sums_ready, nullptr, max_levels, level_R, &done, &R_after, stream));
+    LX_TRY(lx_loop_queued(j, oj, nullptr, R, idx_a, idx_b, first_sums_ready, nullptr, max_levels, level_R, &done, &R_after,
+                          stream));
     *n_levels = done;
     *R_final = R_after;
     *in_b = (done & 1) ? 1 : 0;
     return 0;
 }
 
-extern "C" int sober_level_loop(sober_level_job* j, int64_t R, int32_t* idx_a, int32_t* idx_b, int first_sums_ready,
-                                void** events, int max_levels, int64_t* level_R, int32_t* n_levels, int64_t* R_final,
-                                int32_t* in_b, void* stream) {
+static int lx_level_loop(sober_level_job* j, const sober_final_job* fj, int64_t R, int32_t* idx_a, int32_t* idx_b,
+                         int first_sums_ready, void** events, int max_levels, int64_t* level_R, int32_t* n_levels,
+                         int64_t* R_final, int32_t* in_b, void* stream) {
+    if (j) j->feat_level = -1;
     if (!j || !idx_a || !idx_b || !level_R || !n_levels || !R_final || !in_b || !j->h_flags || !j->mu || R <= 0)
         return SOBER_E_ARG;
     const int S = j->S;
@@ -313,7 +351,8 @@
     if (j->dR && j->h_dR && (j->variant == SOBER_LEVEL_MFMA || (j->variant == SOBER_LEVEL_TANI && !sober::switches().tani_no_queue))) {
         int done = 0;
         int64_t R_after = R;
-        LX_TRY(lx_loop_queued(j, nullptr, R, idx_a, idx_b, first_sums_ready, events, max_levels, level_R, &done, &R_after, stream));
+        LX_TRY(lx_loop_queued(j, nullptr, fj, R, idx_a, idx_b, first_sums_ready, events, max_levels, level_R, &done, &R_after,
+                              stream));
         if (done > 0) {
             levels = done;
             R = R_after;
@@ -361,8 +400,15 @@
     return 0;
 }
 
-extern "C" int sober_level_final_job(const sober_level_job* j, const sober_final_job* f, const int32_t* idx, int R,
-                                     void* stream) {
+extern "C" int sober_level_loop(sober_level_job* j, int64_t R, int32_t* idx_a, int32_t* idx_b, int first_sums_ready,
+                                void** events, int max_levels, int64_t* level_R, int32_t* n_levels, int64_t* R_final,
+                                int32_t* in_b, void* stream) {
+    return lx_level_loop(j, nullptr, R, idx_a, idx_b, first_sums_ready, events, max_levels, level_R, n_levels, R_final, in_b,
+                         stream);
+}
+
+static int lx_final(const sober_level_job* j, const sober_final_job* f, const int32_t* idx, int R, bool from_table,
+                    void* stream) {
     if (!j || !f || !f->rows_sc || (!f->cand_sc && (!f->cand_raw || !f->ls || !f->sc_buf)) || !idx || !f->K || !f->mu_live ||
         !f->out_idx || !f->out_w || !j->P || !j->Xtr || !j->X_tmp || !j->keep_rank || !j->w_star || !j->mu_out || !j->car_ws ||
         !j->h_flags || !j->mu)
@@ -370,7 +416,9 @@
     const int S = j->S, n = j->n;
     if (R <= n + 1 || R > S || f->N <= 0) return SOBER_E_ARG;
     if (!sober_car_supported(R, n + 1)) return SOBER_E_DIM;
-    if (f->cand_sc) {
+    if (from_table) {
+        LX_TRY(sober_feat_gather(j->feat_F, n, j->feat_rows, j->feat_map, n, idx, R, j->X_tmp, j->mu, f->mu_live, stream));
+    } else if (f->cand_sc) {
         LX_TRY(sober_pairwise(j->kind, f->rows_sc, f->rows_norm, j->n_rows, f->cand_sc, f->cand_norm, idx, R, f->dt,
                               j->outputscale, f->K, R, stream));
     } else {
@@ -379,14 +427,21 @@
         LX_TRY(sober_pairwise(j->kind, f->rows_sc, f->rows_norm, j->n_rows, f->sc_buf, nullptr, nullptr, R, f->dt,
                               j->outputscale, f->K, R, stream));
     }
-    LX_TRY(sober_dgemm_coldiv_t(n, R, j->n_rows, j->P, j->n_rows, f->K, R, nullptr, j->X_tmp, n, stream));
-    if (f->cand_sc) LX_TRY(sober_gather_f64(j->mu, idx, R, f->mu_live, stream));
+    if (!from_table) {
+        LX_TRY(sober_dgemm_coldiv_t(n, R, j->n_rows, j->P, j->n_rows, f->K, R, nullptr, j->X_tmp, n, stream));
+        if (f->cand_sc) LX_TRY(sober_gather_f64(j->mu, idx, R, f->mu_live, stream));
+    }
     LX_TRY(sober_car_device_ex(j->X_tmp, n, R, n + 1, f->mu_live, j->keep_rank, j->w_star, j->keep_rank + S, j->mu_out,
                                nullptr, j->car_ws, j->car_ws_bytes, j->car_mode, stream));
     LX_TRY(sober_final_commit(idx, R, j->keep_rank, j->w_star, j->keep_rank + S, f->row_offset, j->mu, f->N, f->out_idx,
                               f->out_w, stream));
     hipError_t e = hipMemcpyAsync(j->h_flags + S, j->keep_rank + S, sizeof(int32_t), hipMemcpyDeviceToHost, (hipStream_t)stream);
     return e == hipSuccess ? 0 : (int)e;
+}
+
+extern "C" int sober_level_final_job(const sober_level_job* j, const sober_final_job* f, const int32_t* idx, int R,
+                                     void* stream) {
+    return lx_final(j, f, idx, R, false, stream);
 }
 
 extern "C" int sober_level_final(const sober_level_job* j, const void* rows_sc, const double* rows_norm,
@@ -406,8 +461,8 @@
                                       int first_sums_ready, void** events, int max_levels, int64_t* level_R,
                                       int32_t* n_levels, int64_t* R_final, int32_t* in_b, void* stream) {
     if (f) f->done = 0;
-    const int rc = sober_level_loop(j, R, idx_a, idx_b, first_sums_ready, events, max_levels, level_R, n_levels, R_final,
-                                    in_b, stream);
+    const int rc = lx_level_loop(j, f, R, idx_a, idx_b, first_sums_ready, events, max_levels, level_R, n_levels, R_final,
+                                 in_b, stream);
     if (rc != 0 || !f) return rc;
     const int S = j->S, n = j->n;
     const int64_t Rf = *R_final;
@@ -415,7 +470,7 @@
     if (j->car_mode != SOBER_CAR_DEFAULT && j->car_mode != SOBER_CAR_SAFE) return 0;
     if (!sober_car_supported((int)Rf, n + 1)) return 0;
     if (j->car_mode == SOBER_CAR_SAFE && !sober_car_safe_supported((int)Rf, n + 1)) return 0;
-    LX_TRY(sober_level_final_job(j, f, *in_b ? idx_b : idx_a, (int)Rf, stream));
+    LX_TRY(lx_final(j, f, *in_b ? idx_b : idx_a, (int)Rf, j->feat_level >= 0, stream));
     const hipError_t e = hipStreamSynchronize((hipStream_t)stream);
     if (e != hipSuccess) return (int)e;
     f->done = 1;
diff --git a/sober_amd/csrc/level_feat.hip b/sober_amd/csrc/level_feat.hip
--- /dev/null
+++ b/sober_amd/csrc/level_feat.hip
@@ -0,0 +1,285 @@
+#include "common.hpp"
+
+namespace sober {
+
+typedef double double4_t __attribute__((ext_vector_type(4)));
+
+#define FEAT_NT 2
+#define FEAT_MT 8
+
+__global__ void k_feat_prep(const int32_t* __restrict__ cur, int64_t R_ub, int S, const int64_t* __restrict__ dR,
+                            const double* __restrict__ cand_sc, const double* __restrict__ cand_raw, int64_t ld_raw,
+                            int d_raw, const double* __restrict__ ls, int ls_len, int dt, int64_t pool,
+                            double* __restrict__ sc, int32_t* __restrict__ fmap) {
+    const int64_t t = (int64_t)blockIdx.x * blockDim.x + threadIdx.x;
+    if (t >= R_ub * dt) return;
+    const int64_t R = __hip_atomic_load(dR, __ATOMIC_RELAXED, __HIP_MEMORY_SCOPE_AGENT);
+    if (R <= S || R > R_ub) return;
+    const int64_t p = t / dt;
+    const int j = (int)(t % dt);
+    double v = 0.0;
+    if (p < R) {
+        const int64_t c = cur[p];
+        if (c >= 0 && c < pool) {
+            if (cand_sc != nullptr) v = cand_sc[c * dt + j];
+            else if (j < d_raw) v = cand_raw[c * ld_raw + j] / ls[ls_len == 1 ? 0 : j];
+            if (j == 0) fmap[c] = (int32_t)p;
+        }
+    }
+    sc[t] = v;
+}
+
+template <int KIND, int DT, int MT>
+__global__ __launch_bounds__(256) void k_feat_build(const double* __restrict__ rows, int n_rows, const double* __restrict__ sc,
+                                                    int64_t R_ub, int S, const int64_t* __restrict__ dR, double os,
+                                                    const double* __restrict__ P, int n, double* __restrict__ F, int ldf) {
+    constexpr int NT = FEAT_NT, LDT = 16 * MT + 1;
+    __shared__ double red[(NT * MT * 256 > NT * 16 * LDT) ? NT * MT * 256 : NT * 16 * LDT];
+    const int64_t R = __hip_atomic_load(dR, __ATOMIC_RELAXED, __HIP_MEMORY_SCOPE_AGENT);
+    if (R <= S || R > R_ub) return;
+    const int64_t j0 = (int64_t)blockIdx.x * (16 * NT);
+    if (j0 >= R) return;
+    const int wave = threadIdx.x >> 6, lane = threadIdx.x & 63, li = lane & 15, lk = lane >> 4;
+    const int i_base = blockIdx.y * (16 * MT);
+    const int kq = (((n_rows + 3) / 4) + 15) / 16 * 16;
+    const int kbeg = min(wave * kq, n_rows), kend = min(kbeg + kq, n_rows);
+
+    double y[NT][DT];
+#pragma unroll
+    for (int t = 0; t < NT; ++t) {
+        const int64_t p = min(j0 + 16 * t + li, R_ub - 1);
+#pragma unroll
+        for (int q = 0; q < DT; ++q) y[t][q] = sc[p * DT + q];
+    }
+    double4_t acc[NT][MT];
+#pragma unroll
+    for (int t = 0; t < NT; ++t)
+#pragma unroll
+        for (int r = 0; r < MT; ++r) acc[t][r] = (double4_t){0.0, 0.0, 0.0, 0.0};
+
+    for (int k0 = kbeg; k0 < kend; k0 += 16) {
+#pragma unroll
+        for (int u = 0; u < 4; ++u) {
+            const int kk = k0 + 4 * u + lk;
+            const bool ok = kk < kend;
+            const int kc = min(kk, n_rows - 1);
+            const double* x = rows + (size_t)kc * DT;
+            double kv[NT];
+#pragma unroll
+            for (int t = 0; t < NT; ++t) {
+                double sq = 0.0;
+#pragma unroll
+                for (int q = 0; q < DT; ++q) {
+                    const double df = x[q] - y[t][q];
+                    sq = fma(df, df, sq);
+                }
+                const double v = kern_from_sq<KIND>(sq, os);
+                kv[t] = ok ? v : 0.0;
+            }
+#pragma unroll
+            for (int r = 0; r < MT; ++r) {
+                const int row = i_base + 16 * r + li;
+                const double pv = P[(size_t)min(row, n - 1) * n_rows + kc];
+                const double a = (ok && row < n) ? pv : 0.0;
+#pragma unroll
+                for (int t = 0; t < NT; ++t) acc[t][r] = __builtin_amdgcn_mfma_f64_16x16x4f64(a, kv[t], acc[t][r], 0, 0, 0);
+            }
+        }
+    }
+    for (int w = 1; w < 4; ++w) {
+        if (wave == w) {
+#pragma unroll
+            for (int t = 0; t < NT; ++t)
+#pragma unroll
+                for (int r = 0; r < MT; ++r)
+#pragma unroll
+                    for (int q = 0; q < 4; ++q) red[(t * MT + r) * 256 + q * 64 + lane] = acc[t][r][q];
+        }
+        __syncthreads();
+        if (wave == 0) {
+#pragma unroll
+            for (int t = 0; t < NT; ++t)
+#pragma unroll
+                for (int r = 0; r < MT; ++r)
+#pragma unroll
+                    for (int q = 0; q < 4; ++q) acc[t][r][q] += red[(t * MT + r) * 256 + q * 64 + lane];
+        }
+        __syncthreads();
+    }
+    if (wave == 0) {
+#pragma unroll
+        for (int t = 0; t < NT; ++t)
+#pragma unroll
+            for (int r = 0; r < MT; ++r)
+#pragma unroll
+                for (int q = 0; q < 4; ++q) red[(16 * t + li) * LDT + 16 * r + lk + 4 * q] = acc[t][r][q];
+    }
+    __syncthreads();
+    const int width = min(16 * MT, n - i_base);
+    for (int e = threadIdx.x; e < NT * 16 * 16 * MT; e += 256) {
+        const int pl = e / (16 * MT), il = e % (16 * MT);
+        const int64_t p = j0 + pl;
+        if (il < width && p < R) F[(size_t)p * ldf + i_base + il] = red[pl * LDT + il];
+    }
+}
+
+template <int NI>
+__global__ __launch_bounds__(256) void k_feat_level_queued(const double* __restrict__ F, int ldf, int64_t f_rows,
+                                                           const int32_t* __restrict__ fmap, int n, int S,
+                                                           const int32_t* __restrict__ cur, const double* __restrict__ mu,
+                                                           const int64_t* __restrict__ dR, int64_t R_ub,
+                                                           double* __restrict__ X_tmp, double* __restrict__ tot) {
+    __shared__ double s_w[256], s_wt[256];
+    __shared__ int32_t s_col[256];
+    __shared__ double s_acc[3][NI][64];
+    __shared__ double s_tot[4];
+    const int64_t R = __hip_atomic_load(dR, __ATOMIC_RELAXED, __HIP_MEMORY_SCOPE_AGENT);
+    if (R <= S || R > R_ub) return;
+    const int s = blockIdx.x, tid = threadIdx.x, wave = tid >> 6, lane = tid & 63;
+    const int64_t E = R / S, ES = E * S;
+    const int r = (int)(R - ES);
+    const int64_t T = E + (s < r ? 1 : 0) + (s == S - 1 ? r : 0);
+    int off[NI];
+#pragma unroll
+    for (int q = 0; q < NI; ++q) off[q] = min(lane + 64 * q, n - 1);
+    double acc[NI];
+#pragma unroll
+    for (int q = 0; q < NI; ++q) acc[q] = 0.0;
+    double tacc = 0.0;
+    for (int64_t t0 = 0; t0 < T; t0 += 256) {
+        const int cnt = (int)min((int64_t)256, T - t0);
+        __syncthreads();
+        if (tid < cnt) {
+            const int64_t t = t0 + tid;
+            const int64_t p = t < E ? t * S + s : (s == S - 1 ? ES + (t - E) : ES + s);
+            const int c = cur[p];
+            const double w = mu[c];
+            const int64_t col = fmap[c];
+            s_w[tid] = w;
+            s_wt[tid] = (t < E || s == S - 1) ? w : 0.0;
+            s_col[tid] = (int32_t)max((int64_t)0, min(col, f_rows - 1));
+        }
+        __syncthreads();
+#pragma unroll 8
+        for (int k = wave; k < cnt; k += 4) {
+            const double w = s_w[k];
+            const double* f = F + (size_t)s_col[k] * ldf;
+            tacc += s_wt[k];
+#pragma unroll
+            for (int q = 0; q < NI; ++q) acc[q] = fma(w, f[off[q]], acc[q]);
+        }
+    }
+    if (wave > 0) {
+#pragma unroll
+        for (int q = 0; q < NI; ++q) s_acc[wave - 1][q][lane] = acc[q];
+        if (lane == 0) s_tot[wave] = tacc;
+    }
+    __syncthreads();
+    if (wave > 0) return;
+    for (int h = 1; h < 4; ++h) {
+#pragma unroll
+        for (int q = 0; q < NI; ++q) acc[q] += s_acc[h - 1][q][lane];
+        tacc += s_tot[h];
+    }
+#pragma unroll
+    for (int q = 0; q < NI; ++q) {
+        const int i = lane + 64 * q;
+        if (i < n) X_tmp[(size_t)s * n + i] = acc[q] / tacc;
+    }
+    if (tid == 0) tot[s] = tacc;
+}
+
+__global__ void k_feat_gather(const double* __restrict__ F, int ldf, int64_t f_rows, const int32_t* __restrict__ fmap, int n,
+                              const int32_t* __restrict__ idx, int R, double* __restrict__ X_tmp,
+                              const double* __restrict__ mu, double* __restrict__ mu_live) {
+    const int t = blockIdx.x * blockDim.x + threadIdx.x;
+    if (t >= R * n) return;
+    const int p = t / n, i = t % n;
+    const int c = idx[p];
+    const int64_t col = max((int64_t)0, min((int64_t)fmap[c], f_rows - 1));
+    X_tmp[t] = F[(size_t)col * ldf + i];
+    if (mu_live != nullptr && i == 0) mu_live[p] = mu[c];
+}
+
+template <int KIND, int MT>
+static int feat_build_launch(int dt, hipStream_t st, const double* rows, int n_rows, const double* sc, int64_t R_ub, int S,
+                             const int64_t* dR, double os, const double* P, int n, double* F, int ldf) {
+    dim3 grid((unsigned)((R_ub + 16 * FEAT_NT - 1) / (16 * FEAT_NT)), (unsigned)((n + 16 * MT - 1) / (16 * MT)));
+#define FEAT_CASE(DT)                                                                                                        \
+    case DT:                                                                                                                 \
+        hipLaunchKernelGGL((k_feat_build<KIND, DT, MT>), grid, dim3(256), 0, st, rows, n_rows, sc, R_ub, S, dR, os, P, n, F, \
+                           ldf);                                                                                             \
+        break;
+    switch (dt) {
+        FEAT_CASE(4) FEAT_CASE(8) FEAT_CASE(12) FEAT_CASE(16) FEAT_CASE(20) FEAT_CASE(24) FEAT_CASE(32)
+        default: return SOBER_E_DIM;
+    }
+#undef FEAT_CASE
+    LAUNCH_CHECK();
+    return 0;
+}
+template <int KIND>
+static int feat_build_kind(int dt, hipStream_t st, const double* rows, int n_rows, const double* sc, int64_t R_ub, int S,
+                           const int64_t* dR, double os, const double* P, int n, double* F, int ldf) {
+    if (n <= 32) return feat_build_launch<KIND, 2>(dt, st, rows, n_rows, sc, R_ub, S, dR, os, P, n, F, ldf);
+    const int tiles = (n + 15) / 16;
+    if ((tiles + 6) / 7 * 7 <= (tiles + 7) / 8 * 8) return feat_build_launch<KIND, 7>(dt, st, rows, n_rows, sc, R_ub, S, dR, os, P, n, F, ldf);
+    return feat_build_launch<KIND, FEAT_MT>(dt, st, rows, n_rows, sc, R_ub, S, dR, os, P, n, F, ldf);
+}
+
+}
+
+using namespace sober;
+
+extern "C" int sober_feat_supported(int kind, int dt, int n) {
+    if (kind != SOBER_KIND_RBF && kind != SOBER_KIND_MATERN52) return 0;
+    if (n <= 0 || n > 512) return 0;
+    return dt == 4 || dt == 8 || dt == 12 || dt == 16 || dt == 20 || dt == 24 || dt == 32;
+}
+
+extern "C" int64_t sober_feat_max_r(void) { return sober::switches().feat_max_r; }
+
+extern "C" int sober_feat_build(int kind, const double* rows_sc, int n_rows, int dt, const double* cand_sc,
+                                const double* cand_raw, int64_t ld_raw, int d_raw, const double* ls, int ls_len,
+                                double outputscale, const double* P, int n, const int32_t* cur, int64_t R_ub, int S,
+                                const int64_t* dR, int64_t pool, double* sc_buf, double* F, int ldf, int32_t* fmap,
+                                void* stream) {
+    if (!rows_sc || (!cand_sc && (!cand_raw || !ls)) || !P || !cur || !dR || !sc_buf || !F || !fmap || n_rows <= 0 || R_ub <= 0 ||
+        S <= 0 || pool <= 0 || ldf < n || (!cand_sc && (d_raw <= 0 || d_raw > dt || ld_raw < d_raw)))
+        return SOBER_E_ARG;
+    if (!sober_feat_supported(kind, dt, n)) return SOBER_E_DIM;
+    hipStream_t st = (hipStream_t)stream;
+    hipLaunchKernelGGL(k_feat_prep, dim3((unsigned)((R_ub * dt + 255) / 256)), dim3(256), 0, st, cur, R_ub, S, dR, cand_sc,
+                       cand_raw, ld_raw, d_raw, ls, ls_len, dt, pool, sc_buf, fmap);
+    LAUNCH_CHECK();
+    if (kind == SOBER_KIND_RBF)
+        return feat_build_kind<SOBER_KIND_RBF>(dt, st, rows_sc, n_rows, sc_buf, R_ub, S, dR, outputscale, P, n, F, ldf);
+    return feat_build_kind<SOBER_KIND_MATERN52>(dt, st, rows_sc, n_rows, sc_buf, R_ub, S, dR, outputscale, P, n, F, ldf);
+}
+
+extern "C" int sober_feat_level_queued(const double* F, int ldf, int64_t f_rows, const int32_t* fmap, int n, int S,
+                                       const int32_t* cur, const double* mu, const int64_t* dR, int64_t R_ub, double* X_tmp,
+                                       double* tot, void* stream) {
+    if (!F || !fmap || !cur || !mu || !dR || !X_tmp || !tot || n <= 0 || n > 512 || S <= 0 || ldf < n ||
+        f_rows <= 0 || R_ub <= 0)
+        return SOBER_E_ARG;
+#define FEAT_LEVEL(NI)                                                                                                    \
+    hipLaunchKernelGGL(k_feat_level_queued<NI>, dim3((unsigned)S), dim3(256), 0, (hipStream_t)stream, F, ldf, f_rows, fmap, \
+                       n, S, cur, mu, dR, R_ub, X_tmp, tot)
+    if (n <= 64) FEAT_LEVEL(1);
+    else if (n <= 128) FEAT_LEVEL(2);
+    else if (n <= 256) FEAT_LEVEL(4);
+    else FEAT_LEVEL(8);
+#undef FEAT_LEVEL
+    LAUNCH_CHECK();
+    return 0;
+}
+
+extern "C" int sober_feat_gather(const double* F, int ldf, int64_t f_rows, const int32_t* fmap, int n, const int32_t* idx,
+                                 int R, double* X_tmp, const double* mu, double* mu_live, void* stream) {
+    if (!F || !fmap || !idx || !X_tmp || n <= 0 || R <= 0 || ldf < n || f_rows <= 0 || (mu_live && !mu)) return SOBER_E_ARG;
+    hipLaunchKernelGGL(k_feat_gather, dim3((unsigned)(((int64_t)R * n + 255) / 256)), dim3(256), 0, (hipStream_t)stream, F,
+                       ldf, f_rows, fmap, n, idx, R, X_tmp, mu, mu_live);
+    LAUNCH_CHECK();
+    return 0;
+}
diff --git a/sober_amd/csrc/misc.hip b/sober_amd/csrc/misc.hip
--- a/sober_amd/csrc/misc.hip
+++ b/sober_amd/csrc/misc.hip
@@ -501,6 +501,12 @@
     w.car_unfused = getenv("SOBER_CAR_UNFUSED") != nullptr;
     w.level_no_classes = getenv("SOBER_LEVEL_NO_CLASSES") != nullptr;
     w.car_exact_ratio = getenv("SOBER_CAR_EXACT_RATIO") != nullptr;
+    w.level_no_features = getenv("SOBER_LEVEL_NO_FEATURES") != nullptr;
+    w.feat_max_r = SOBER_FEAT_MAX_R;
+    if (const char* v = getenv("SOBER_FEAT_MAX_R")) {
+        const long long r = atoll(v);
+        if (r > 0 && r <= (1ll << 22)) w.feat_max_r = r;
+    }
     return w;
 }
 static Switches g_switches = read_switches();
diff --git a/sober_amd/csrc/switches.hpp b/sober_amd/csrc/switches.hpp
--- a/sober_amd/csrc/switches.hpp
+++ b/sober_amd/csrc/switches.hpp
@@ -7,6 +7,8 @@
     bool car_unfused;
     bool car_exact_ratio;
     bool level_no_classes;
+    bool level_no_features;
+    long long feat_max_r;
 };
 const Switches& switches();
 }
```
